# fetty31/fast_LIMO

Hardware: AMD Instinct MI355X
Metric: scans/sec (64k-pt scan, 1M-pt map) + kNN HBM GB/s vs roofline; ATE vs CPU ref (higher is better)
Workload: dtype f32; 1 GPU; BASELINE.json configs[1]: 65536-pt Velodyne-like scan (64 rings x 1024 azimuths), 1000000-pt box-world map, k=5, MAX_NUM_ITERS=3, GPU deskew + iterated ESKF update per step; parallelism=replicas x1 (independent scan streams, no collective), steps_bit_reproducible=True, chains_run=0, chains_handed_back_early=0, chains_declined=2597

## Files before the change

fast_limo_amd/_abi.py:

```python
from __future__ import annotations

import ctypes as C
import numpy as np

f32p = np.ctypeslib.ndpointer(dtype=np.float32, flags="C_CONTIGUOUS")
f64p = np.ctypeslib.ndpointer(dtype=np.float64, flags="C_CONTIGUOUS")
i32p = np.ctypeslib.ndpointer(dtype=np.int32, flags="C_CONTIGUOUS")

CHAIN_MAX_PASSES = 12


class MapCfg(C.Structure):
    _fields_ = [("min_extent", C.c_float), ("bucket_size", C.c_int), ("downsample", C.c_int),
                ("cell_size", C.c_float)]


class MatchCfg(C.Structure):
    _fields_ = [("NUM_MATCH_POINTS", C.c_int), ("MAX_NUM_MATCHES", C.c_int), ("MAX_NUM_PC2MATCH", C.c_int),
                ("MAX_DIST_PLANE", C.c_double), ("PLANE_THRESHOLD", C.c_double), ("estimate_extrinsics", C.c_int)]


class Frame(C.Structure):
    _fields_ = [("p", C.c_float * 3), ("q", C.c_float * 4), ("v", C.c_float * 3), ("g", C.c_float * 3),
                ("w", C.c_float * 3), ("a", C.c_float * 3), ("bg", C.c_float * 3), ("ba", C.c_float * 3),
# ... 148 lines not shown
    ("flimo_corr_graph", "flimo_loc_corr_graph", [vp, vp, sz, P(CorrGraphCfg), vp, vp, vp, vp]),
    ("flimo_desc_ref_set", "flimo_loc_desc_ref_set", [vp, sz, i]),
    ("flimo_desc_match", "flimo_loc_desc_match", [vp, sz, i, i, vp, vp, vp]),
)
LOC_OF = {hip: loc for hip, loc, _ in PAIRED}

HIP_ONLY = (
    (i, "flimo_ctx_create", [i, P(vp)]),
    (None, "flimo_ctx_destroy", [vp]),
    (C.c_char_p, "flimo_last_error", [vp]),
    (C.c_char_p, "flimo_version", []),
    (i, "flimo_map_config", [vp, P(MapCfg)]),
    (i, "flimo_map_add", [vp, f32p, sz, sz, d]),
    (i, "flimo_map_clear", [vp]),
    (i, "flimo_map_crop_box", [vp, vp, vp, P(sz)]),
    (i, "flimo_map_crop_stats", [vp, P(u64)]),
    (i, "flimo_map_carve_stats", [vp, P(u64)]),
    (sz, "flimo_map_size", [vp]),
    (d, "flimo_map_last_time", [vp]),
    (i, "flimo_map_points", [vp, vp, sz, P(sz)]),
    (i, "flimo_map_add_scan", [vp, f64p, d]),
    (i, "flimo_knn", [vp, f32p, sz, i, i32p, f32p, i32p]),
    (i, "flimo_radius_candidates", [vp, f32p, sz, f, vp]),
    (i, "flimo_knn_k_candidates", [vp, vp, sz, i, f, vp]),
    (i, "flimo_set_outlier_chunk", [vp, sz]),
    (i, "flimo_set_fpfh_chunk", [vp, sz]),
    (i, "flimo_set_keypoints_chunk", [vp, sz]),
    (i, "flimo_set_cluster_chunk", [vp, sz]),
    (i, "flimo_set_plane_chunk", [vp, sz]),
    (i, "flimo_set_voxel_plan", [vp, i]),
    (i, "flimo_set_region_chunk", [vp, sz]),
    (i, "flimo_set_normals_chunk", [vp, sz]),
    (i, "flimo_set_fitness_chunk", [vp, sz]),
    (i, "flimo_set_linearize_chunk", [vp, sz]),
    (i, "flimo_set_corr_chunk", [vp, sz]),
    (i, "flimo_set_desc_chunk", [vp, sz, sz]),
    (sz, "flimo_desc_ref_size", [vp]),
    (i, "flimo_desc_ref_dim", [vp]),
    (f, "flimo_desc_last_ms", [vp]),
    (i, "flimo_plane_solve_host", [vp, P(PlaneCfg), vp, vp]),
    (i, "flimo_voxel_key_host", [vp, f, vp, P(u64)]),
    (i, "flimo_region_joined_host", [vp, vp, vp, vp, P(RegionCfg), P(i), P(i), P(i)]),
    (i, "flimo_corr_pose_host", [vp, vp, P(CorrCfg), vp, vp]),
    (i, "flimo_corr_compatible_host", [vp, vp, vp, vp, P(CorrGraphCfg)]),
    (i, "flimo_desc_dist_host", [vp, vp, i, vp]),
    (None, "flimo_plane_fit5_host", [f32p, f32p]),
    (i, "flimo_plane_eval5_host", [f32p, f32p, f]),
    (i, "flimo_calculate_H_host", [f64p, f32p, f32p, f32p, sz, i, f64p, f64p]),
    (i, "flimo_insert_rule_replay", [f, i, f32p, vp, sz, vp, P(sz)]),
    (i, "flimo_scan_set", [vp, f32p, sz, sz]),
    (sz, "flimo_scan_size", [vp]),
    (i, "flimo_scan_get", [vp, vp, sz, P(sz)]),
    (i, "flimo_scan_voxel_filter", [vp, f, P(sz)]),
    (i, "flimo_raw_scan_set", [vp, f32p, sz, sz, f64p]),
    (i, "flimo_raw_scan_filter_set", [vp, vp, sz, P(FilterCfg), P(sz), P(d), P(i)]),
    (i, "flimo_raw_scan_filter_order_set", [vp, vp, sz, P(FilterCfg), i, P(sz), P(d), P(i), P(i)]),
    (i, "flimo_raw_scan_order", [vp, vp, sz, P(sz)]),
    (i, "flimo_upload_stage", [vp, sz, P(vp)]),
    (i, "flimo_scan_adopt", [vp, vp]),
    (i, "flimo_deskew_resident", [vp, vp, sz, f32p, f64p]),
    (i, "flimo_deskew_resident_offset", [vp, vp, sz, f32p, f64p, d]),
    (i, "flimo_deskew", [vp, f32p, sz, sz, f64p, vp, sz, f32p, f64p]),
    (i, "flimo_scan_to_world", [vp, f64p, vp, sz]),
    (i, "flimo_scan_clouds", [vp, f64p, P(vp), P(vp), P(sz)]),
    (i, "flimo_scan_debug_clouds", [vp, f64p, P(vp), P(vp), P(sz)]),
    (i, "flimo_match_reduce", [vp, f64p, P(MatchCfg), f64p, f64p, P(i)]),
    (i, "flimo_match_reduce_overlap", [vp, f64p, P(MatchCfg), f64p, f64p, P(i), vp, vp]),
    (i, "flimo_match_fetch", [vp, vp, sz, P(sz)]),
    (i, "flimo_match_fetch_H", [vp, vp, vp, sz, P(sz)]),
    (i, "flimo_update_chain", [vp, P(MatchCfg), P(ChainIO)]),
    (i, "flimo_chain_stats", [vp, f64p, i]),
    (i, "flimo_set_update_mode", [vp, i]),
    (i, "flimo_update_mode", [vp, P(i), P(d)]),
    (i, "flimo_set_pass_pipeline", [vp, i]),
    (i, "flimo_pass_pipeline_end", [vp]),
    (i, "flimo_pass_pipeline_last", [vp]),
    (i, "flimo_pass_pipeline_stats", [vp, P(ull)]),
    (i, "flimo_device_large_bar", [i, P(i)]),
    (i, "flimo_set_timing", [vp, i]),
    (i, "flimo_set_timing_stride", [vp, i]),
    (i, "flimo_set_timing_deferred", [vp, i]),
    (i, "flimo_set_wait_timeout_ms", [vp, i]),
    (i, "flimo_set_debug_records", [vp, i]),
    (i, "flimo_set_path_switches", [vp, i, i]),
    (ull, "flimo_pass_count", [vp]),
    (ull, "flimo_fused_pass_count", [vp]),
    (i, "flimo_tie_stats", [vp, P(ull)]),
    (i, "flimo_fine_stats", [vp, P(ull)]),
    (i, "flimo_map_index_bytes", [vp, P(u64)]),
    (i, "flimo_map_index_layout", [vp, i, P(d)]),
    (i, "flimo_map_grid_selfcheck", [vp, P(u64), P(u64)]),
    (i, "flimo_last_kernel_ms", [vp, P(f), P(f), P(f)]),
    (d, "flimo_last_candidates_per_query", [vp]),
    (i, "flimo_last_widen_count", [vp]),
    (i, "flimo_last_stragglers", [vp]),
    (i, "flimo_stragglers_by_pass", [vp, P(i)]),
    (i, "flimo_timing_totals", [vp, P(d), P(d), P(d), P(C.c_longlong), P(C.c_longlong), i]),
    (i, "flimo_timing_split", [vp, f64p, i]),
    (i, "flimo_ieskf_op_shape", [i, P(i), P(i)]),
    (i, "flimo_ieskf_eval", [vp, i, f64p, sz, f64p]),
    (i, "flimo_ieskf_eval_host", [i, f64p, sz, f64p, vp]),
    (i, "flimo_ieskf_run_fixed", [vp, f64p, f64p, f64p, d, d, i, i, f64p, f64p, vp, f64p, f64p, P(i)]),
)

HOST_ONLY = (
    (i, "flimo_loc_create", [P(LocCfg), P(vp)]),
    (None, "flimo_loc_destroy", [vp]),
    (vp, "flimo_loc_ctx", [vp]),
    (None, "flimo_loc_sync", [vp]),
    (None, "flimo_loc_set_async_insert", [vp, i]),
    (None, "flimo_loc_set_lazy_time_order", [vp, i]),
    (None, "flimo_loc_set_gpu_filters", [vp, i]),
    (None, "flimo_loc_set_exact_tied_order", [vp, i]),
    (None, "flimo_loc_set_local_map", [vp, f32p, f]),
    (i, "flimo_local_map_rule", [f64p, f32p, f, f64p, P(i), f32p, f32p]),
    (None, "flimo_loc_set_map_carving", [vp, i, P(CarveCfg)]),
    (i, "flimo_carve_rule", [i, P(i)]),
    (None, "flimo_carve_sensor", [f64p, f32p]),
    (sz, "flimo_loc_last_carve_removed", [vp]),
    (i, "flimo_loc_last_sweep_tied", [vp]),
    (None, "flimo_loc_set_propagation_wait", [vp, d]),
    (d, "flimo_loc_last_insert_seconds", [vp]),
    (i, "flimo_loc_update_imu", [vp, d, f32p, f32p]),
    (i, "flimo_loc_update_imu_n", [vp, sz, f64p, f32p, f32p]),
    (i, "flimo_loc_replay", [vp, sz, P(vp), uintpp, f64p, f64p, sz, f64p, f32p, f32p, i32p, f64p]),
    (i, "flimo_loc_update_pointcloud", [vp, f32p, sz, d]),
    (i, "flimo_loc_update_pointcloud_points", [vp, vp, sz, d]),
    (i, "flimo_loc_map_add", [vp, f32p, sz, d]),
    (sz, "flimo_loc_map_size", [vp]),
    (None, "flimo_loc_get_x", [vp, f64p]),
    (None, "flimo_loc_set_x", [vp, f64p]),
    (None, "flimo_loc_get_P", [vp, f64p]),
    (None, "flimo_loc_set_P", [vp, f64p]),
    (None, "flimo_loc_set_flags", [vp, i, i, i]),
    (i, "flimo_loc_num_passes", [vp]),
    (None, "flimo_loc_get_pass", [vp, i, P(i), f64p, f64p, f64p, f64p]),
    (sz, "flimo_loc_get_pc2match", [vp, vp, sz]),
    (sz, "flimo_loc_get_final_scan", [vp, vp, sz]),
    (sz, "flimo_loc_get_debug_cloud", [vp, i, vp, sz]),
    (None, "flimo_loc_get_stage_times", [vp, f64p]),
    (None, "flimo_loc_get_pose_cov", [vp, f64p]),
    (None, "flimo_loc_host_profile", [vp, f64p, i]),
    (i, "flimo_loc_register_resident", [vp, f64p, f64p]),
    (None, "flimo_host_state_update", [f32p, d, d]),
    (i, "flimo_host_time_order", [vp, i, sz, i, i, vp]),
    (i, "flimo_host_plane", [f32p, f32p, i, i, d, d, f32p, f32p, P(f)]),
    (i, "flimo_eskf_update_fixed", [f64p, f64p, f64p, f64p, i, i, f64p, d, d, P(i)]),
    (i, "flimo_eskf_predict", [f64p, f64p, d, f64p, f64p, f64p]),
    (i, "flimo_ieskf_gj12_host", [i, f64p, sz, f64p]),
    (i, "flimo_ieskf_run_fixed_host", [f64p, f64p, f64p, d, d, i, i, f64p, f64p, P(i), f64p, f64p, P(i)]),
    (None, "flimo_host_eigen_solver6", [f64p, f64p, f64p, f64p]),
)

HIP_SYMBOLS = [hip for hip, _, _ in PAIRED] + [name for _, name, _ in HIP_ONLY]
HOST_SYMBOLS = [loc for _, loc, _ in PAIRED] + [name for _, name, _ in HOST_ONLY]


def declare(lib, side):
    for row in PAIRED:
        fn = getattr(lib, row[side])
        fn.restype, fn.argtypes = C.c_int, [vp] + row[2]
    for restype, name, args in (HIP_ONLY, HOST_ONLY)[side]:
        fn = getattr(lib, name)
        fn.restype, fn.argtypes = restype, args
```

fast_limo_amd/_lib.py:

```python
from __future__ import annotations

import ctypes as C
import os
import numpy as np

from . import _abi
from ._abi import (CHAIN_MAX_PASSES, CarveCfg, ChainIO, ChainPass, ClusterCfg, ClusterStats, CorrCfg, CorrGraphCfg, FilterCfg, FpfhCfg, Frame,
                   KeypointCfg, MapCfg, MatchCfg, OutlierCfg, OutlierStats, PlaneCfg, PlaneSel, RegionCfg, RegionStats, VoxelCfg, VoxelStats,
                   f32p, f64p, i32p)

_PKG = os.path.dirname(os.path.abspath(__file__))
ROOT = os.path.dirname(_PKG)


class FlimoError(RuntimeError):
    pass


RADIUS_SORTED = 1


def carve_cfg(res=256, win=1, margin=0.2, rel_margin=0.02, max_depth=float("inf")) -> CarveCfg:
    return CarveCfg(int(res), int(win), float(margin), float(rel_margin), float(max_depth))

# ... 663 lines not shown
    def scan_clouds(self, x26):
        b, w, n = C.c_void_p(), C.c_void_p(), C.c_size_t(0)
        self._chk(self._L.flimo_scan_clouds(self._h, np.ascontiguousarray(x26, dtype=np.float64), C.byref(b), C.byref(w), C.byref(n)))
        if n.value == 0:
            return np.zeros((0, 3), np.float32), np.zeros((0, 3), np.float32)
        rec = lambda p: np.ctypeslib.as_array(C.cast(p, C.POINTER(C.c_float)), shape=(n.value, 4))[:, :3].copy()
        return rec(b), rec(w)

    def scan_debug_clouds(self, x26):
        d, f, n = C.c_void_p(), C.c_void_p(), C.c_size_t(0)
        self._chk(self._L.flimo_scan_debug_clouds(self._h, np.ascontiguousarray(x26, dtype=np.float64), C.byref(d), C.byref(f), C.byref(n)))
        if n.value == 0:
            return np.zeros((0, 4), np.float32), np.zeros((0, 4), np.float32)
        rec = lambda p: np.ctypeslib.as_array(C.cast(p, C.POINTER(C.c_float)), shape=(n.value, 4)).copy()
        return rec(d), rec(f)

    def map_add_scan(self, x26, stamp=0.0):
        self._chk(self._L.flimo_map_add_scan(self._h, np.ascontiguousarray(x26, dtype=np.float64), float(stamp)))

    def set_timing(self, level=2):
        self._chk(self._L.flimo_set_timing(self._h, 2 if level is True else int(level)))

    def set_timing_stride(self, every=1):
        self._chk(self._L.flimo_set_timing_stride(self._h, int(every)))

    def set_timing_deferred(self, on=True):
        self._chk(self._L.flimo_set_timing_deferred(self._h, 1 if on else 0))

    def pass_count(self) -> int:
        return int(self._L.flimo_pass_count(self._h))

    def fine_stats(self):
        o = (C.c_ulonglong * 4)()
        self._chk(self._L.flimo_fine_stats(self._h, o))
        return dict(active=bool(o[0]), points=int(o[1]), builds=int(o[2]), passes=int(o[3]))

    def tie_stats(self):
        o = (C.c_ulonglong * 2)()
        self._chk(self._L.flimo_tie_stats(self._h, o))
        return dict(passes_redone=int(o[0]), queries_settled=int(o[1]))

    def map_index_bytes(self):
        o = (C.c_uint64 * 6)()
        self._chk(self._L.flimo_map_index_bytes(self._h, o))
        return dict(points=int(o[0]), index=int(o[1]), second_level=int(o[2]), tiles=int(o[3]), tile_pool_relayouts=int(o[4]),
                    sorted_array_allocated=int(o[5]))

    def map_index_layout(self, level=0):
        o = (C.c_double * 28)()
        self._chk(self._L.flimo_map_index_layout(self._h, int(level), o))
        if not o[19]:
            return dict(valid=False)
        ints = ("xs", "six", "siy", "siz", "nx", "ny", "nz", "ts", "ty", "tz", "ntx", "nty", "ntz", "escape_slots", "escape_slots_taken")
        d = dict(valid=True, ox=np.float32(o[0]), oy=np.float32(o[1]), oz=np.float32(o[2]), cell=np.float32(o[3]), points=int(o[20]))
        d.update((name, int(o[4 + i])) for i, name in enumerate(ints))
        if level == 1:
            d.update(qlo=tuple(int(o[21 + a]) for a in range(3)), qhi=tuple(int(o[24 + a]) for a in range(3)))
        return d

    def fused_pass_count(self) -> int:
        return int(self._L.flimo_fused_pass_count(self._h))

    def grid_selfcheck(self):
        mm = C.c_uint64(0)
        st = (C.c_uint64 * 2)()
        self._chk(self._L.flimo_map_grid_selfcheck(self._h, C.byref(mm), st))
        return int(mm.value), int(st[0]), int(st[1])

    def set_debug_records(self, on=True):
        self._chk(self._L.flimo_set_debug_records(self._h, int(on)))

    def last_kernel_ms(self):
        a = C.c_float(0)
        b = C.c_float(0)
        d = C.c_float(0)
        self._chk(self._L.flimo_last_kernel_ms(self._h, C.byref(a), C.byref(b), C.byref(d)))
        return a.value, b.value, d.value

    def timing_totals(self, reset=False):
        a = C.c_double(0); b = C.c_double(0); d = C.c_double(0); n = C.c_longlong(0); q = C.c_longlong(0)
        self._chk(self._L.flimo_timing_totals(self._h, C.byref(a), C.byref(b), C.byref(d), C.byref(n), C.byref(q), int(reset)))
        return dict(knn_ms=a.value, widen_ms=b.value, fit_ms=d.value, passes=n.value, queries=q.value)

    def set_path_switches(self, tail=-1, fuse=-1):
        self._chk(self._L.flimo_set_path_switches(self._h, int(tail), int(fuse)))

    def timing_split(self, reset=False):
        o = np.zeros(6)
        self._chk(self._L.flimo_timing_split(self._h, o, int(reset)))
        return dict(fused_ms=o[0], fused_n=int(o[1]), knn_ms=o[2], widen_ms=o[3], fit_ms=o[4], separate_n=int(o[5]))

    def update_chain(self, cfg: "MatchCfg", x26, P, limits, R=0.001, D=5.0, max_iter=3, want_log=True):
        io = ChainIO()
        io.x26[:] = list(np.asarray(x26, dtype=np.float64))
        io.P[:] = list(np.asarray(P, dtype=np.float64).reshape(-1))
        io.limits[:] = list(np.asarray(limits, dtype=np.float64))
        io.R, io.D, io.max_iter, io.want_log = float(R), float(D), int(max_iter), int(bool(want_log))
        self._chk(self._L.flimo_update_chain(self._h, C.byref(cfg), C.byref(io)))
        n_log = min(CHAIN_MAX_PASSES, io.passes + (1 if io.status == 2 else 0))
        log = [dict(M=io.log[i].M, stragglers=io.log[i].stragglers, ties=io.log[i].ties,
                    HTH=np.array(io.log[i].HTH).reshape(12, 12), HTh=np.array(io.log[i].HTh), dx=np.array(io.log[i].dx),
                    x_after=np.array(io.log[i].x_after)) for i in range(n_log)]
        meas = dict(M=io.meas_M, HTH=np.array(io.meas_HTH).reshape(12, 12), HTh=np.array(io.meas_HTh)) if io.meas_valid else None
        return dict(status=io.status, reason=io.reason, passes=io.passes, it_next=io.it_next, t=io.t, x=np.array(io.x26_out),
                    meas=meas, log=log)

    def set_update_mode(self, mode: int):
        self._chk(self._L.flimo_set_update_mode(self._h, int(mode)))

    def update_mode(self):
        ch = C.c_int(0); rtt = C.c_double(0)
        self._chk(self._L.flimo_update_mode(self._h, C.byref(ch), C.byref(rtt)))
        return dict(chained=bool(ch.value), launch_rtt_us=rtt.value)

    def set_pass_pipeline(self, on: bool):
        self._chk(self._L.flimo_set_pass_pipeline(self._h, int(on)))

    def pass_pipeline_end(self):
        self._chk(self._L.flimo_pass_pipeline_end(self._h))

    def pass_pipeline_last(self):
        self._chk(self._L.flimo_pass_pipeline_last(self._h))

    def pass_pipeline_stats(self):
        o = (C.c_ulonglong * 4)()
        self._chk(self._L.flimo_pass_pipeline_stats(self._h, o))
        return dict(published=int(o[0]), cancelled=int(o[1]), aged=int(o[2]), left=int(o[3]))

    def chain_stats(self, reset=False):
        o = np.zeros(5)
        self._chk(self._L.flimo_chain_stats(self._h, o, int(reset)))
        return dict(algebra_ms=o[0], algebra_n=int(o[1]), chains=int(o[2]), handed_back=int(o[3]), declined=int(o[4]))

    def ieskf_eval(self, op, items):
        a, no = ik_items(op, items)
        out = np.zeros((a.shape[0], no))
        if a.shape[0]:
            self._chk(self._L.flimo_ieskf_eval(self._h, int(op), a.reshape(-1), a.shape[0], out.reshape(-1)))
        return out

    def ieskf_run_fixed(self, x26, P, limits, partials, extras=None, tag_ok=None, R=0.001, D=5.0, max_iter=3):
        x, Pm, lim, part = ik_fixed_args(x26, P, limits, partials)
        ns = part.shape[0]
        ex = np.zeros((ns, 2)) if extras is None else np.ascontiguousarray(extras, dtype=np.float64).reshape(ns, 2)
        tg = None if tag_ok is None else np.ascontiguousarray(tag_ok, dtype=np.int32).reshape(ns)
        it_out = np.zeros((int(max_iter) + 1, IK_ITER_N))
        fin = np.zeros(IK_FINAL_N)
        n = C.c_int(0)
        self._chk(self._L.flimo_ieskf_run_fixed(self._h, x, Pm, lim, float(R), float(D), int(max_iter), ns, part.reshape(-1), ex.reshape(-1),
                                                None if tg is None else tg.ctypes.data, it_out.reshape(-1), fin, C.byref(n)))
        its = []
        for r in it_out[:n.value]:
            on = bool(r[590])
            its.append(dict(pre_dxn=r[0:23].copy(), pre_AG=r[23:299].copy(), HTH=r[299:443].reshape(12, 12).copy() if on else None,
                            HTh=r[443:455].copy() if on else None, dx=r[455:478].copy() if on else None,
                            x_after=r[478:504].copy() if on else None, pose=r[504:570].astype(np.float32), prev_RT=r[570:586].astype(np.float32),
                            status=int(r[586]), it=int(r[587]), t=int(r[588]), passes=int(r[589]), went_on=on))
        final = dict(status=int(fin[0]), reason=int(fin[1]), passes=int(fin[2]), it=int(fin[3]), t=int(fin[4]), x=fin[5:31].copy(),
                     passinfo=fin[31:67].reshape(12, 3).copy(), sums=fin[67:158].copy())
        return its, final

    def last_widen_count(self) -> int:
        return int(self._L.flimo_last_widen_count(self._h))

    def set_wait_timeout_ms(self, ms: int):
        self._chk(self._L.flimo_set_wait_timeout_ms(self._h, int(ms)))

    def last_stragglers(self) -> int:
# ... 76 lines not shown
```

fast_limo_amd/csrc/hip/flimo_capi.hip:

```cpp
#include <hip/hip_runtime.h>
#include <stdarg.h>
#include <stdio.h>
#include <string.h>
#include <math.h>
#include <string>
#include <chrono>
#include <thread>
#include <array>
#include <vector>
#include <algorithm>
#include <limits>
#include <immintrin.h>
#include "../../../include/flimo_c.h"
#include "../../../include/flimo_dev.h"
#include "flimo_types.h"
#include "flimo_kernels.h"
#include "flimo_math.h"
#include "flimo_pose.h"
#include "flimo_corr.h"
#include "flimo_plane.h"
#include "flimo_voxel.h"
#include "flimo_region.h"
#include "flimo_desc.h"
#include "flimo_chain.h"
// ... 146 lines not shown
  bool recs_valid = false, dbg_valid = false;
  PrevPass prev{};
  bool prune = true;
  unsigned probe_min = 96;
  int stragglers_hist[4] = {1 << 30, 0, 0, 0};
  int pass_in_scan = 0;
  int last_stragglers = -1;
  bool fine_on = true;
  unsigned fine_threshold = 64;
  int fine_div = 4;
  unsigned fine_min_points = 32768;
  bool fine_valid = false;
  bool crowd_box_valid = false;
  GridView fine{};
  int fine_qlo[3] = {0, 0, 0}, fine_qhi[3] = {-1, -1, -1};
  float4 *d_fine_tmp = nullptr, *d_fine_pts = nullptr;
  size_t fine_pts_cap = 0;
  IndexTables fine_idx;
  uint32_t* d_fine_count = nullptr;
  void* d_crowd_list = nullptr;
  uint32_t* d_crowd_count = nullptr;
  uint32_t* d_crowd_bits = nullptr;
  size_t crowd_bits_cap = 0;
  uint32_t crowd_listed = 0;
  std::vector<std::array<int, 3>> crowd_cells;
  float fine_center[3] = {0.f, 0.f, 0.f};
  bool have_fine_center = false;
  float fine_radius = 24.f;
  uint64_t fine_builds = 0, fine_passes = 0;
  int xslabs = 2;
  int* d_tie_list = nullptr;
  unsigned int* d_tie_count = nullptr;
  size_t tie_cap = 0;
  bool ties = true;
  unsigned long long tie_redos = 0, tie_queries = 0;
  unsigned long long* d_tie_settled = nullptr;
  void* d_nbrk = nullptr;
  size_t nbrk_cap = 0;
  int wait_timeout_ms = 2000;
  hipEvent_t adopt_ev = nullptr;
  hipEvent_t timeout_ev = nullptr;
  bool timeout_pending = false;
  ChainState* d_chain = nullptr;
  void* d_chain_gran = nullptr;
  ChainPrior* h_chain_prior = nullptr;
  ChainPrior* d_chain_prior = nullptr;
  double* h_chain_res = nullptr;
  void* d_chain_res = nullptr;
  double* h_chain_log = nullptr;
  void* d_chain_log = nullptr;
  unsigned long long chain_tag = 0x4000000000000000ull;
  struct Prelaunch {
    bool active = false;
    unsigned long long seq = 0;
    size_t nq = 0;
    int n_all = 0, pos = 0;
    flimo_match_cfg cfg{};
    uint64_t grid_version = 0;
    unsigned int end_code = 0;
    double t_launch = 0.0;
    float prev_RT[16] = {0};
  } pre;
  bool pipeline = false;
  bool pipeline_env = false;
  PipeHead* d_pipe_head = nullptr;
  unsigned int pipe_tag = 0;
  bool pipe_last_hint = false;
  unsigned long long pipe_published = 0, pipe_cancelled = 0;
  unsigned long long pipe_aged = 0, pipe_left = 0;
  bool row_slack = true;
  bool test_tight_array = false;
  int test_publish_delay_ms = 0;
  int test_publish_split_ms = 0;
  PrevPass prev_before{};
  int update_mode = 0;
  double launch_rtt_us = 0.0;
  bool host_update = false;
  hipEvent_t chain_ev[CH_MAX_PASSES][8];
  bool chain_ev_made = false;
  double chain_alg_ms = 0;
  long long chain_alg_n = 0, chains_run = 0, chains_back = 0, chains_declined = 0;
  int fov_check = 0, fov_check_bad = 0;
  bool tail = true;
};

constexpr size_t FRAMES_FG_SLOT = 8192;
static int timing_drain(flimo_ctx* c);
static inline void ctx_enter(flimo_ctx* c);
static int fail(flimo_ctx* c, int code, const char* fmt, ...) {
  char buf[512];
  va_list ap;
  va_start(ap, fmt);
  vsnprintf(buf, sizeof(buf), fmt, ap);
  va_end(ap);
  if (c) c->err = buf;
  return code;
}
#define HIPCHK(c, call)                                                                          \
  do {                                                                                           \
    hipError_t e_ = (call);                                                                      \
    if (e_ != hipSuccess) return fail(c, FLIMO_ERR_HIP, "%s failed: %s", #call, hipGetErrorString(e_)); \
  } while (0)

static int ensure_pinned(flimo_ctx* c, void*& buf, size_t& cap, size_t bytes) {
  if (bytes <= cap) return FLIMO_OK;
  if (buf) (void)hipHostFree(buf);
  buf = nullptr;
  cap = 0;
  const size_t ncap = bytes + bytes / 4 + 4096;
  HIPCHK(c, hipHostMalloc(&buf, ncap, hipHostMallocDefault));
  cap = ncap;
  return FLIMO_OK;
}
static int ensure_stage(flimo_ctx* c, size_t bytes) { return ensure_pinned(c, c->h_stage, c->stage_cap, bytes); }

template <typename T>
static int ensure_dev(flimo_ctx* c, T*& p, size_t& cap, size_t need, bool keep, size_t keep_n) {
  if (need <= cap) return FLIMO_OK;
  size_t ncap = need + need / 4 + 1024;
  T* np = nullptr;
  HIPCHK(c, hipMalloc(&np, ncap * sizeof(T)));
  if (keep && p && keep_n) {
    HIPCHK(c, hipMemcpyAsync(np, p, keep_n * sizeof(T), hipMemcpyDeviceToDevice, c->stream));
    HIPCHK(c, hipStreamSynchronize(c->stream));
  }
  if (p) (void)hipFree(p);
  p = np;
  cap = ncap;
  return FLIMO_OK;
}

struct DevScratch {
  std::vector<void*> got;
  hipError_t err = hipSuccess;
  DevScratch() = default;
  DevScratch(const DevScratch&) = delete;
  DevScratch& operator=(const DevScratch&) = delete;
  ~DevScratch() { for (void* p : got) (void)hipFree(p); }
  template <typename T>
  T* get(size_t count) {
    void* p = nullptr;
    if (err == hipSuccess) err = hipMalloc(&p, count * sizeof(T));
    if (err != hipSuccess) return nullptr;
    got.push_back(p);
    return static_cast<T*>(p);
  }
  void drop(void* p) {
    got.erase(std::remove(got.begin(), got.end(), p), got.end());
    (void)hipFree(p);
  }
  int ok(flimo_ctx* c) const { return err == hipSuccess ? FLIMO_OK : fail(c, FLIMO_ERR_HIP, "hipMalloc failed: %s", hipGetErrorString(err)); }
};


static void load_dev_switches(flimo_ctx* c) {
  auto env_int = [](const char* name, int& out) { const char* e = getenv(name); if (!e) return false; out = atoi(e); return true; };
  int v = 0;
  if (env_int("FLIMO_FUSE", v)) c->fuse = v != 0;
  if (env_int("FLIMO_TAIL", v)) c->tail = v != 0;
  if (env_int("FLIMO_PRUNE", v)) c->prune = v != 0;
  if (env_int("FLIMO_PROBE", v) && v >= 0) c->probe_min = (unsigned)v;
  if (env_int("FLIMO_TIES", v)) c->ties = v != 0;
  if (env_int("FLIMO_FINE", v)) c->fine_on = v != 0;
  if (env_int("FLIMO_FINE_THRESHOLD", v) && v > 0) c->fine_threshold = (unsigned)v;
  if (env_int("FLIMO_FINE_MIN_POINTS", v) && v >= 0) c->fine_min_points = (unsigned)v;
  if (env_int("FLIMO_FULL_REBUILD", v)) c->full_rebuild = v != 0;
  if (env_int("FLIMO_HOST_UPDATE", v)) c->update_mode = v != 0 ? 1 : 2;
  if (env_int("FLIMO_PIPELINE", v)) { c->pipeline = v != 0; c->pipeline_env = true; }
  if (env_int("FLIMO_TEST_PUBLISH_DELAY_MS", v) && v > 0) c->test_publish_delay_ms = v;
  if (env_int("FLIMO_TEST_PUBLISH_SPLIT_MS", v) && v > 0) c->test_publish_split_ms = v;
  if (env_int("FLIMO_TEST_TIGHT_ARRAY", v)) c->test_tight_array = v != 0;
  if (env_int("FLIMO_ROW_SLACK", v)) c->row_slack = v != 0;
  if (env_int("FLIMO_TAIL_MAX", v) && v > 0) c->tail_max_env = v;
}

static bool host_store_probe(flimo_ctx* c, PipeHead* head) {
  volatile unsigned long long* tagp = reinterpret_cast<volatile unsigned long long*>(c->h_chain_res) + 1;
  for (unsigned int round = 0; round < 2; round++) {
    const unsigned int pattern = 0x5a17c0deu ^ (round * 0x01010101u);
    volatile unsigned long long* g = &head->gran[round == 0 ? 0 : PH_GRANULES - 1];
    *g = ((unsigned long long)pattern << 32) | (unsigned long long)round;
    _mm_sfence();
    const unsigned long long tag = 0x7200000000000000ull + round;
    launch_word_probe(c->stream, reinterpret_cast<unsigned int*>(const_cast<unsigned long long*>(g)) + 1, c->d_chain_res, tag);
    if (hipStreamSynchronize(c->stream) != hipSuccess) { (void)hipGetLastError(); return false; }
    if (*tagp != tag) return false;
    const double seen = c->h_chain_res[0];
    if ((unsigned int)llround(seen) != pattern) return false;
    *g = 0ull;
  }
  _mm_sfence();
  memset(c->h_chain_res, 0, 2 * sizeof(double));
  return true;
}

extern "C" const char* flimo_version(void) { return "fast_limo_amd 0.1.0 (gfx950)"; }

extern "C" const char* flimo_last_error(const flimo_ctx* ctx) { return ctx ? ctx->err.c_str() : "null context"; }

extern "C" int flimo_ctx_create(int device, flimo_ctx** out) {
  if (!out) return FLIMO_ERR_INVALID;
  *out = nullptr;
  int ndev = 0;
  if (hipGetDeviceCount(&ndev) != hipSuccess || ndev <= 0) return FLIMO_ERR_NO_DEVICE;
  if (device < 0 || device >= ndev) return FLIMO_ERR_INVALID;
  if (hipSetDevice(device) != hipSuccess) return FLIMO_ERR_NO_DEVICE;
  hipDeviceProp_t prop;
  if (hipGetDeviceProperties(&prop, device) != hipSuccess) return FLIMO_ERR_NO_DEVICE;
  if (strncmp(prop.gcnArchName, "gfx950", 6) != 0) return FLIMO_ERR_NO_DEVICE;
  flimo_ctx* c = new flimo_ctx();
  c->device = device;
  if (hipStreamCreateWithFlags(&c->stream, hipStreamNonBlocking) != hipSuccess) { delete c; return FLIMO_ERR_HIP; }
  for (int i = 0; i < 6; i++) (void)hipEventCreate(&c->ev[i]);
  bool ok = hipMalloc(&c->d_partials, (size_t)c->reduce_waves * 256 * sizeof(double)) == hipSuccess &&
            hipMalloc(&c->d_out256, FIT_GROUPS * FIT_SLOT * sizeof(double)) == hipSuccess &&
            hipHostMalloc((void**)&c->h_out256, FIT_GROUPS * FIT_SLOT * sizeof(double), hipHostMallocMapped) == hipSuccess &&
            hipHostGetDevicePointer((void**)&c->d_out256_host, c->h_out256, 0) == hipSuccess &&
            hipHostMalloc((void**)&c->h_granules, FIT_GROUPS * FIT_LIVE_PAD * 2 * sizeof(double), hipHostMallocMapped) == hipSuccess &&
            hipHostGetDevicePointer((void**)&c->d_granules_host, c->h_granules, 0) == hipSuccess &&
            hipMalloc(&c->d_ticket, (FIT_GROUPS + 2) * sizeof(unsigned int)) == hipSuccess &&
            hipMemset(c->d_ticket, 0, (FIT_GROUPS + 2) * sizeof(unsigned int)) == hipSuccess &&
            hipMalloc(&c->d_cand, sizeof(unsigned long long)) == hipSuccess &&
            hipMalloc(&c->d_tie_count, 2 * sizeof(unsigned int)) == hipSuccess &&
            hipMemset(c->d_tie_count, 0, 2 * sizeof(unsigned int)) == hipSuccess &&
            hipMalloc((void**)&c->d_chain, chain_state_size()) == hipSuccess &&
            hipMemset(c->d_chain, 0, chain_state_size()) == hipSuccess &&
            hipMalloc(&c->d_chain_gran, FIT_GROUPS * FIT_LIVE_PAD * 2 * sizeof(double)) == hipSuccess &&
            hipMemset(c->d_chain_gran, 0, FIT_GROUPS * FIT_LIVE_PAD * 2 * sizeof(double)) == hipSuccess &&
            hipHostMalloc((void**)&c->h_chain_prior, sizeof(ChainPrior), hipHostMallocMapped) == hipSuccess &&
            hipHostGetDevicePointer((void**)&c->d_chain_prior, c->h_chain_prior, 0) == hipSuccess &&
            hipHostMalloc((void**)&c->h_chain_res, (size_t)CH_RES * 2 * sizeof(double), hipHostMallocMapped) == hipSuccess &&
            hipHostGetDevicePointer(&c->d_chain_res, c->h_chain_res, 0) == hipSuccess &&
            hipHostMalloc((void**)&c->h_chain_log, (size_t)CH_MAX_PASSES * CH_LOGN * 2 * sizeof(double), hipHostMallocMapped) == hipSuccess &&
            hipHostGetDevicePointer(&c->d_chain_log, c->h_chain_log, 0) == hipSuccess &&
            hipMalloc((void**)&c->d_tie_settled, sizeof(unsigned long long)) == hipSuccess &&
            hipMemset(c->d_tie_settled, 0, sizeof(unsigned long long)) == hipSuccess &&
            hipMalloc(&c->d_wl_count, sizeof(int)) == hipSuccess &&
            hipMemset(c->d_wl_count, 0, sizeof(int)) == hipSuccess &&
            hipHostMalloc((void**)&c->h_wl_count, sizeof(int), hipHostMallocDefault) == hipSuccess &&
            hipHostMalloc((void**)&c->h_cand, sizeof(unsigned long long), hipHostMallocDefault) == hipSuccess;
  if (!ok) { flimo_ctx_destroy(c); return FLIMO_ERR_HIP; }
  memset(c->h_chain_res, 0, (size_t)CH_RES * 2 * sizeof(double));
  memset(c->h_chain_log, 0, (size_t)CH_MAX_PASSES * CH_LOGN * 2 * sizeof(double));
  memset(c->h_out256, 0, FIT_GROUPS * FIT_SLOT * sizeof(double));
  memset(c->h_granules, 0, FIT_GROUPS * FIT_LIVE_PAD * 2 * sizeof(double));
  launch_mfma_layout(c->stream, c->d_out256);
  if (hipMemcpyAsync(c->h_out256, c->d_out256, 256 * sizeof(double), hipMemcpyDeviceToHost, c->stream) != hipSuccess ||
      hipStreamSynchronize(c->stream) != hipSuccess) { flimo_ctx_destroy(c); return FLIMO_ERR_HIP; }
  bool seen[256] = {false};
  for (int r = 0; r < 256; r++) {
    const double v = c->h_out256[r];
    const int code = (int)llround(v);
    if (code < 0 || code > 255 || fabs(v - code) > 1e-9 || seen[code]) { flimo_ctx_destroy(c); return FLIMO_ERR_HIP; }
    seen[code] = true;
    c->mfma_idx[code / 16][code % 16] = r;
  }
  {
    int k = 0;
    for (int i = 0; i < 12; i++) for (int j = i; j < 12; j++) c->live_idx[k++] = (unsigned char)c->mfma_idx[i][j];
    for (int i = 0; i < 12; i++) c->live_idx[k++] = (unsigned char)c->mfma_idx[i][12];
    c->live_idx[k++] = (unsigned char)c->mfma_idx[13][13];
    for (; k < FIT_LIVE_PAD; k++) c->live_idx[k] = 0;
  }
  c->book = insert_book_create();
  load_dev_switches(c);
  {
    void* p = nullptr;
    int large_bar = 0;
    (void)hipDeviceGetAttribute(&large_bar, hipDeviceAttributeIsLargeBar, device);
    if (getenv("FLIMO_NO_BAR") != nullptr) large_bar = 0;
    if (large_bar && hipExtMallocWithFlags(&p, sizeof(PipeHead), hipDeviceMallocFinegrained) == hipSuccess && p &&
        hipMemset(p, 0, sizeof(PipeHead)) == hipSuccess && hipDeviceSynchronize() == hipSuccess && host_store_probe(c, static_cast<PipeHead*>(p))) {
      c->d_pipe_head = static_cast<PipeHead*>(p);
      void* q = nullptr;
      if (hipExtMallocWithFlags(&q, 2 * FRAMES_FG_SLOT, hipDeviceMallocFinegrained) == hipSuccess && q)
        c->d_frames_fg = static_cast<char*>(q);
      else (void)hipGetLastError();
    } else {
      if (p) (void)hipFree(p);
      (void)hipGetLastError();
      c->d_pipe_head = nullptr;
    }
  }
  {
    std::vector<double> rt;
    volatile unsigned long long* tagp = reinterpret_cast<volatile unsigned long long*>(c->h_chain_res) + 1;
    for (int i = 0; i < 40; i++) {
      const unsigned long long tag = 0x7100000000000000ull + (unsigned long long)i;
      const auto t0 = std::chrono::steady_clock::now();
      launch_rtt_probe(c->stream, c->d_chain_res, tag);
      unsigned long long spins = 0;
      while (*tagp != tag && ++spins < 200000000ull) _mm_pause();
      const double us = std::chrono::duration<double, std::micro>(std::chrono::steady_clock::now() - t0).count();
      if (i >= 8) rt.push_back(us);
    }
    (void)hipStreamSynchronize(c->stream);
    std::sort(rt.begin(), rt.end());
    c->launch_rtt_us = rt[rt.size() / 4];
    memset(c->h_chain_res, 0, 2 * sizeof(double));
    c->host_update = c->update_mode != 2;
  }
  *out = c;
  return FLIMO_OK;
}

extern "C" void flimo_ctx_destroy(flimo_ctx* c) {
  if (!c) return;
  ctx_enter(c);
  if (c->stream) (void)hipStreamSynchronize(c->stream);
  (void)hipFree(c->d_map_raw); (void)hipFree(c->d_map_sorted); index_free(c->idx); index_free(c->fine_idx);
  (void)hipFree(c->d_scan_sorted); (void)hipFree(c->d_nbr); (void)hipFree(c->d_wl); (void)hipFree(c->d_wl_count);
  (void)hipFree(c->d_fit_partials); (void)hipFree(c->d_raw_sorted); (void)hipFree(c->d_t_sorted);
  (void)hipFree(c->d_scan); (void)hipFree(c->d_scan_raw); (void)hipFree(c->d_scan_world); (void)hipFree(c->d_scan_t);
  (void)hipFree(c->d_frames); (void)hipFree(c->d_recs); (void)hipFree(c->d_dbg); (void)hipFree(c->d_dbg_clouds);
  (void)hipFree(c->d_fine_tmp); (void)hipFree(c->d_fine_pts); 
  (void)hipFree(c->d_fine_count); (void)hipFree(c->d_crowd_list); (void)hipFree(c->d_crowd_count); (void)hipFree(c->d_crowd_bits);
  (void)hipFree(c->d_tkey[0]); (void)hipFree(c->d_tkey[1]); (void)hipFree(c->d_tperm); (void)hipFree(c->d_t_tmp);
  (void)hipFree(c->d_raw32); (void)hipFree(c->d_filt_ext); (void)hipFree(c->d_nbrk); (void)hipFree(c->d_tie_list); (void)hipFree(c->d_tie_count);
  if (c->h_filt_ext) (void)hipHostFree(c->h_filt_ext);
  (void)hipFree(c->d_partials); (void)hipFree(c->d_out256); (void)hipFree(c->d_cand); (void)hipFree(c->d_ticket);
  if (c->h_out256) (void)hipHostFree(c->h_out256);
  if (c->h_granules) (void)hipHostFree(c->h_granules);
  (void)hipFree(c->d_fit2_partials);
  if (c->h_cand) (void)hipHostFree(c->h_cand);
  (void)hipFree(c->d_chain); (void)hipFree(c->d_chain_gran); (void)hipFree(c->d_tie_settled);
  if (c->h_chain_prior) (void)hipHostFree(c->h_chain_prior);
  if (c->h_chain_res) (void)hipHostFree(c->h_chain_res);
  if (c->h_chain_log) (void)hipHostFree(c->h_chain_log);
  if (c->chain_ev_made) for (int i = 0; i < CH_MAX_PASSES; i++) for (int k = 0; k < 8; k++) (void)hipEventDestroy(c->chain_ev[i][k]);
  if (c->h_stage) (void)hipHostFree(c->h_stage);
  if (c->h_dbg_clouds) (void)hipHostFree(c->h_dbg_clouds);
  if (c->h_clouds) (void)hipHostFree(c->h_clouds);
  for (int k = 0; k < 2; k++) if (c->h_frames[k]) (void)hipHostFree(c->h_frames[k]);
  map_scratch_free(c->scratch);
  for (int i = 0; i < 6; i++) if (c->ev[i]) (void)hipEventDestroy(c->ev[i]);
  if (c->ev_ring_made) for (int r = 0; r < flimo_ctx::EV_RING; r++) for (int i = 0; i < 6; i++) (void)hipEventDestroy(c->ev_ring[r][i]);
  if (c->timeout_ev) (void)hipEventDestroy(c->timeout_ev);
  if (c->adopt_ev) (void)hipEventDestroy(c->adopt_ev);
  if (c->h_wl_count) (void)hipHostFree(c->h_wl_count);
  if (c->d_pipe_head) (void)hipFree(c->d_pipe_head);
  if (c->d_frames_fg) (void)hipFree(c->d_frames_fg);
  if (c->stream) (void)hipStreamDestroy(c->stream);
  if (c->book) insert_book_destroy(c->book);
  c->gbook.release();
  (void)hipFree(c->d_batch);
  (void)hipFree(c->d_desc_rt); (void)hipFree(c->d_desc_norm);
  delete c;
}

extern "C" int flimo_map_config(flimo_ctx* c, const flimo_map_cfg* cfg) {
  if (!c || !cfg) return FLIMO_ERR_INVALID;
  if (!(cfg->min_extent > 0.f)) return fail(c, FLIMO_ERR_INVALID, "min_extent must be > 0");
  const float cell_before = c->map_cfg.cell_size;
  c->map_cfg = *cfg;
  if (!(c->map_cfg.cell_size > 0.f)) c->map_cfg.cell_size = 0.5f;
  if (c->map_cfg.cell_size != cell_before) { c->force_full = true; c->have_gbox = false; c->have_origin = false; }
  insert_book_config(c->book, cfg->min_extent, cfg->downsample != 0);
  return FLIMO_OK;
}

extern "C" int flimo_map_clear(flimo_ctx* c) {
  if (!c) return FLIMO_ERR_INVALID;
  c->map_n = 0;
  c->grid_valid = false;
  c->fine_valid = false;
  c->have_gbox = false;
  c->have_origin = false;
  c->map_last_time = -1.0;
  c->bb[0] = c->bb[1] = c->bb[2] = 3.4e38f; c->bb[3] = c->bb[4] = c->bb[5] = -3.4e38f;
  c->crowd_box_valid = false;
  c->have_fine_center = false;
  insert_book_clear(c->book);
  c->gbook.active = false;
  c->prev.valid = 0;
  return FLIMO_OK;
}

extern "C" size_t flimo_map_size(const flimo_ctx* c) { return c ? c->map_n : 0; }
extern "C" double flimo_map_last_time(const flimo_ctx* c) { return c ? c->map_last_time : -1.0; }

static inline int grid_low_x_cells(int xs) { return (8 + xs - 1) / xs; }
static bool grid_side_low_ok(const GridView& g, const float* bb, int a) {
  const float o[3] = {g.ox, g.oy, g.oz};
  const int si[3] = {g.six, g.siy, g.siz};
  const int low = a == 0 ? grid_low_x_cells(g.xs) : 0;
  if ((int)floorf((bb[a] - 0.5f * g.cell - o[a]) * g.inv_cell) - si[a] < low) return false;
  if ((int)floorf((bb[a] - o[a]) * g.inv_cell) - si[a] < low) return false;
  return true;
}
static bool grid_covers(const GridView& g, const float* bb) {
  const float o[3] = {g.ox, g.oy, g.oz};
  const int n[3] = {g.nx, g.ny, g.nz}, si[3] = {g.six, g.siy, g.siz};
  for (int a = 0; a < 3; a++) {
    if (!grid_side_low_ok(g, bb, a)) return false;
    if ((int)floorf((bb[3 + a] - o[a]) * g.inv_cell) - si[a] > n[a] - 2) return false;
  }
  return true;
}
static int update_fine_grid(flimo_ctx* c, bool relayout, const float4* new_pts = nullptr, size_t n_new = 0) {
  c->fine_valid = false;
  if (!c->fine_on || !c->grid_valid || c->map_n == 0) return FLIMO_OK;
  const GridView& g = c->grid;
  if ((double)g.nx * (double)g.ny * (double)g.nz > 2.0e9) return FLIMO_OK;
  constexpr uint32_t CROWD_CAP = 1u << 20;
  if (!c->d_crowd_list) {
    HIPCHK(c, hipMalloc(&c->d_crowd_list, (size_t)CROWD_CAP * sizeof(int4)));
    HIPCHK(c, hipMalloc(&c->d_crowd_count, sizeof(uint32_t)));
    HIPCHK(c, hipMalloc(&c->d_fine_count, sizeof(uint32_t)));
  }
  static const bool prof = getenv("FLIMO_PROF_INSERT") != nullptr;
  auto now = [] { return std::chrono::duration<double>(std::chrono::steady_clock::now().time_since_epoch()).count(); };
  const double tp0 = prof ? now() : 0.0;
  uint32_t listed = 0;
  const size_t ncells_main = (size_t)g.nx * g.ny * g.nz;
  if (relayout || !c->crowd_box_valid || !new_pts) {
    const size_t words = (ncells_main + 31) / 32;
    if (words > c->crowd_bits_cap) {
      (void)hipFree(c->d_crowd_bits);
      c->d_crowd_bits = nullptr; c->crowd_bits_cap = 0;
      HIPCHK(c, hipMalloc(&c->d_crowd_bits, (words + words / 4 + 64) * sizeof(uint32_t)));
      c->crowd_bits_cap = words + words / 4 + 64;
    }
// ... 1542 lines not shown
    struct Part { void* dst; const void* src; size_t bytes; char* at; } parts[5] = {
        {centroid, d_centroid, 24 * m, nullptr}, {cov, d_cov, 48 * m, nullptr}, {label, d_label, 4 * m, nullptr},
        {count, d_cnt, 4 * m, nullptr},          {first, d_first, 4 * m, nullptr}};
    for (Part& p : parts) {
      if (!p.dst) continue;
      p.at = h;
      h += p.bytes;
      HIPCHK(c, hipMemcpyAsync(p.at, p.src, p.bytes, hipMemcpyDeviceToHost, c->stream));
    }
    HIPCHK(c, hipStreamSynchronize(c->stream));
    for (const Part& p : parts)
      if (p.dst) memcpy(p.dst, p.at, p.bytes);
  }
  if (stats) *stats = st;
  return FLIMO_OK;
}
extern "C" int flimo_map_remove_regions(flimo_ctx* c, size_t first, size_t n, const flimo_region_cfg* cfg, size_t* removed,
                                        flimo_region_stats* stats) {
  if (!c) return FLIMO_ERR_INVALID;
  { const int rc = region_check(c, first, n, cfg, "remove regions"); if (rc) return rc; }
  if (c->map_n == 0) { if (removed) *removed = 0; region_stats_none(stats); return FLIMO_OK; }
  if (n == 0 && !stats) { if (removed) *removed = 0; return FLIMO_OK; }
  RegionDev d;
  flimo_region_stats st;
  { const int rc = regions_device(c, first, n, *cfg, false, false, true, false, d, &st); if (rc) return rc; }
  if (removed) *removed = 0;
  if (stats) *stats = st;
  if (st.sel_points == 0) return FLIMO_OK;
  return map_remove_masked(c, d.mask, first, n, (size_t)st.sel_points, &c->region_removals, &c->region_removed, removed, "remove regions");
}
extern "C" int flimo_set_region_chunk(flimo_ctx* c, size_t n) { return set_chunk(c, &flimo_ctx::region_chunk, n, (size_t)1 << 20); }
extern "C" int flimo_region_joined_host(const float pi[3], const float ni[4], const float pj[3], const float nj[4], const flimo_region_cfg* cfg,
                                        int* smooth_i, int* smooth_j, int* joined) {
  if (!pi || !ni || !pj || !nj || !cfg || !region_cfg_ok(cfg)) return FLIMO_ERR_INVALID;
  const float r2 = cfg->tol * cfg->tol;
  if (smooth_i) *smooth_i = region_smooth(ni[0], ni[1], ni[2], ni[3], cfg->max_curv) ? 1 : 0;
  if (smooth_j) *smooth_j = region_smooth(nj[0], nj[1], nj[2], nj[3], cfg->max_curv) ? 1 : 0;
  if (joined)
    *joined = region_has_normal(ni[0], ni[1], ni[2], ni[3]) && region_has_normal(nj[0], nj[1], nj[2], nj[3]) &&
                      region_joined(pi, ni, pj, nj, r2, cfg->min_cos) ? 1 : 0;
  return FLIMO_OK;
}
extern "C" int flimo_set_voxel_plan(flimo_ctx* c, int plan) {
  if (!c) return FLIMO_ERR_INVALID;
  if (plan < 0 || (plan & ~VOXEL_PLAN_SORTED) > VOXEL_PLAN_RUNS) return fail(c, FLIMO_ERR_INVALID, "voxel plan: %d is none of 0..4, + 8", plan);
  c->voxel_plan = plan;
  return FLIMO_OK;
}

static int ensure_raw_sorted(flimo_ctx* c, size_t n) {
  if (n <= c->raw_sorted_cap) return FLIMO_OK;
  const size_t cap = n + n / 4 + 1024;
  float4* rs = nullptr;
  double* ts = nullptr;
  HIPCHK(c, hipMalloc(&rs, cap * sizeof(float4)));
  HIPCHK(c, hipMalloc(&ts, cap * sizeof(double)));
  (void)hipFree(c->d_raw_sorted); (void)hipFree(c->d_t_sorted);
  c->d_raw_sorted = rs; c->d_t_sorted = ts; c->raw_sorted_cap = cap;
  return FLIMO_OK;
}
static int ensure_scan(flimo_ctx* c, size_t n) {
  { const int rc = ensure_raw_sorted(c, n); if (rc) return rc; }
  if (n <= c->scan_cap) return FLIMO_OK;
  const size_t cap = n + n / 4 + 1024;
  float4 *a = nullptr, *b = nullptr, *w = nullptr, *so = nullptr;
  double* t = nullptr;
  void* nb = nullptr;
  int* wl = nullptr;
  double* fp = nullptr;
  const size_t fpn = (size_t)fit_blocks((int)cap) * 256;
  {
    int* tlst = nullptr;
    HIPCHK(c, hipMalloc(&tlst, cap * sizeof(int)));
    (void)hipFree(c->d_tie_list);
    c->d_tie_list = tlst; c->tie_cap = cap;
  }
  {
    const size_t f2n = (size_t)std::max(std::max(fit2_blocks((int)cap), fused_blocks((int)cap)), FUSED_SPREAD_SLOTS / 128 + 8) * FIT_LIVE_PAD;
    double* f2 = nullptr;
    HIPCHK(c, hipMalloc(&f2, f2n * sizeof(double)));
    (void)hipFree(c->d_fit2_partials);
    c->d_fit2_partials = f2; c->fit2_partials_cap = f2n;
  }
  HIPCHK(c, hipMalloc(&so, cap * sizeof(float4)));
  HIPCHK(c, hipMalloc(&nb, cap * nbr_rec_size()));
  HIPCHK(c, hipMemsetAsync(nb, 0, cap * nbr_rec_size(), c->stream));
  HIPCHK(c, hipMalloc(&wl, (cap + 8192) * wl_entry_size()));
  HIPCHK(c, hipMalloc(&fp, fpn * sizeof(double)));
  (void)hipFree(c->d_scan_sorted); (void)hipFree(c->d_nbr); (void)hipFree(c->d_wl); (void)hipFree(c->d_fit_partials);
  c->d_scan_sorted = so; c->d_nbr = nb; c->d_wl = wl; c->d_fit_partials = fp; c->fit_partials_cap = fpn;
  HIPCHK(c, hipMalloc(&a, cap * sizeof(float4)));
  HIPCHK(c, hipMalloc(&b, cap * sizeof(float4)));
  HIPCHK(c, hipMalloc(&w, cap * sizeof(float4)));
  HIPCHK(c, hipMalloc(&t, cap * sizeof(double)));
  (void)hipFree(c->d_scan); (void)hipFree(c->d_scan_raw); (void)hipFree(c->d_scan_world); (void)hipFree(c->d_scan_t);
  c->d_scan = a; c->d_scan_raw = b; c->d_scan_world = w; c->d_scan_t = t;
  c->scan_cap = cap;
  c->scan_n = 0; c->sorted_n = 0; c->raw_n = 0; c->prev.valid = 0;
  c->deskew_kept = false;
  return FLIMO_OK;
}

static int ensure_recs(flimo_ctx* c, size_t n) {
  if (n <= c->rec_cap) return FLIMO_OK;
  const size_t cap = n + n / 4 + 1024;
  (void)hipFree(c->d_recs); (void)hipFree(c->d_dbg);
  c->d_recs = nullptr; c->d_dbg = nullptr; c->rec_cap = 0;
  HIPCHK(c, hipMalloc(&c->d_recs, cap * sizeof(Rec16)));
  HIPCHK(c, hipMalloc(&c->d_dbg, cap * sizeof(RecDbg)));
  c->rec_cap = cap;
  return FLIMO_OK;
}

static int upload_points(flimo_ctx* c, const float* xyz, size_t n, size_t stride_bytes, float4* dst) {
  int rc = ensure_stage(c, n * sizeof(float4));
  if (rc) return rc;
  float4* st = (float4*)c->h_stage;
  const unsigned char* b = (const unsigned char*)xyz;
  for (size_t i = 0; i < n; i++) {
    const float* p = (const float*)(b + i * stride_bytes);
    st[i].x = p[0]; st[i].y = p[1]; st[i].z = p[2]; st[i].w = (stride_bytes >= 16) ? p[3] : 0.f;
  }
  HIPCHK(c, hipMemcpyAsync(dst, st, n * sizeof(float4), hipMemcpyHostToDevice, c->stream));
  HIPCHK(c, hipStreamSynchronize(c->stream));
  return FLIMO_OK;
}

static int flush_deskew(flimo_ctx* c) {
  if (!c->deskew_pending) return FLIMO_OK;
  c->deskew_pending = false;
  const DeskewArgs& a = c->deskew_args;
  launch_deskew(c->stream, a.raw, a.t, (int)c->deskew_n, a.frames, a.nf, a.mats, a.out_sorted, a.out_orig, a.t_offset);
  HIPCHK(c, hipGetLastError());
  return FLIMO_OK;
}

extern "C" int flimo_scan_set(flimo_ctx* c, const float* xyz, size_t n, size_t stride_bytes) {
  if (!c) return FLIMO_ERR_INVALID;
  if (n > 0 && (!xyz || stride_bytes < 12)) return fail(c, FLIMO_ERR_INVALID, "bad xyz/stride");
  if (n > 0x7fff0000ull) return fail(c, FLIMO_ERR_TOO_LARGE, "scan too large");
  ctx_enter(c);
  c->deskew_pending = false;
  c->deskew_kept = false;
  int rc = ensure_scan(c, n);
  if (rc) return rc;
  if (n) {
    rc = upload_points(c, xyz, n, stride_bytes, c->d_scan);
    if (rc) return rc;
    HIPCHK(c, sort_scan(c->stream, c->d_scan, n, c->d_scan_sorted, c->scratch));
    HIPCHK(c, hipStreamSynchronize(c->stream));
  }
  c->scan_n = n; c->sorted_n = n; c->prev.valid = 0;
  return FLIMO_OK;
}

extern "C" size_t flimo_scan_size(const flimo_ctx* c) { return c ? c->scan_n : 0; }

static int download_xyz(flimo_ctx* c, const float4* src, size_t m, float* out) {
  int rc = ensure_stage(c, m * sizeof(float4));
  if (rc) return rc;
  HIPCHK(c, hipMemcpyAsync(c->h_stage, src, m * sizeof(float4), hipMemcpyDeviceToHost, c->stream));
  HIPCHK(c, hipStreamSynchronize(c->stream));
  const float4* s = (const float4*)c->h_stage;
  for (size_t i = 0; i < m; i++) { out[3 * i] = s[i].x; out[3 * i + 1] = s[i].y; out[3 * i + 2] = s[i].z; }
  return FLIMO_OK;
}
// ... 340 lines not shown
  if (!on && c->ev_pending) { const int rc = timing_drain(c); if (rc) return rc; }
  c->timing_deferred = on != 0;
  return FLIMO_OK;
}
extern "C" unsigned long long flimo_pass_count(const flimo_ctx* c) { return c ? c->pass_seq : 0ull; }
extern "C" unsigned long long flimo_fused_pass_count(const flimo_ctx* c) { return c ? c->fused_passes : 0ull; }
extern "C" int flimo_fine_stats(const flimo_ctx* c, unsigned long long out[4]) {
  if (!c || !out) return FLIMO_ERR_INVALID;
  out[0] = c->fine_valid ? 1 : 0; out[1] = c->fine_valid ? c->fine.n_pts : 0; out[2] = c->fine_builds; out[3] = c->fine_passes;
  return FLIMO_OK;
}
extern "C" int flimo_map_index_bytes(const flimo_ctx* c, uint64_t out[6]) {
  if (!c || !out) return FLIMO_ERR_INVALID;
  out[0] = (uint64_t)c->map_n * sizeof(float4);
  auto tables = [](const GridView& g, const IndexTables& T) {
    const uint64_t rows = ((uint64_t)g.ny + 2 * GRID_PAD) * ((uint64_t)g.nz + 2 * GRID_PAD);
    return (uint64_t)T.tiles_used * grid_tile_entries(g.ts, g.ty, g.tz) * 8ull + (uint64_t)GRID_DIR_MAX * 2ull +
           (uint64_t)(grid_xstart_size(g.ny, g.nz, g.ntx) + T.ovf_cap) * 4ull + rows * 4ull + (uint64_t)g.ny * g.nz * 4ull;
  };
  out[5] = c->d_map_sorted ? (uint64_t)c->sorted_cap * sizeof(float4) : 0ull;
  out[1] = c->grid_valid ? tables(c->grid, c->idx) : 0ull;
  out[2] = c->fine_valid ? (uint64_t)c->fine.n_pts * sizeof(float4) + tables(c->fine, c->fine_idx) : 0ull;
  out[3] = c->grid_valid ? c->idx.tiles_used : 0ull;
  out[4] = c->index_overflows;
  return FLIMO_OK;
}
extern "C" int flimo_map_index_layout(flimo_ctx* c, int level, double out[28]) {
  if (!c || !out || level < 0 || level > 1) return FLIMO_ERR_INVALID;
  for (int i = 0; i < 28; i++) out[i] = 0.0;
  const bool valid = level == 0 ? c->grid_valid : c->fine_valid;
  out[19] = valid ? 1.0 : 0.0;
  if (!valid) return FLIMO_OK;
  const GridView& g = level == 0 ? c->grid : c->fine;
  const IndexTables& T = level == 0 ? c->idx : c->fine_idx;
  out[0] = g.ox; out[1] = g.oy; out[2] = g.oz; out[3] = g.cell; out[4] = g.xs;
  out[5] = g.six; out[6] = g.siy; out[7] = g.siz; out[8] = g.nx; out[9] = g.ny; out[10] = g.nz;
  out[11] = g.ts; out[12] = g.ty; out[13] = g.tz; out[14] = g.ntx; out[15] = g.nty; out[16] = g.ntz;
  out[17] = (double)(T.ovf_cap / 8);
  uint32_t taken = 0;
  ctx_enter(c);
  HIPCHK(c, hipStreamSynchronize(c->stream));
  if (T.counters) HIPCHK(c, hipMemcpy(&taken, T.counters + 2, sizeof(taken), hipMemcpyDeviceToHost));
  out[18] = taken;
  out[20] = g.n_pts;
  if (level == 1) for (int a = 0; a < 3; a++) { out[21 + a] = c->fine_qlo[a]; out[24 + a] = c->fine_qhi[a]; }
  return FLIMO_OK;
}
extern "C" int flimo_tie_stats(flimo_ctx* c, unsigned long long out[2]) {
  if (!c || !out) return FLIMO_ERR_INVALID;
  out[0] = c->tie_redos; out[1] = c->tie_queries;
  unsigned long long dev = 0;
  ctx_enter(c);
  if (c->d_tie_settled && hipMemcpy(&dev, c->d_tie_settled, sizeof(dev), hipMemcpyDeviceToHost) == hipSuccess) out[1] += dev;
  return FLIMO_OK;
}
extern "C" int flimo_set_timing_stride(flimo_ctx* c, int every) { if (!c || every < 1) return FLIMO_ERR_INVALID; c->timing_stride = every; return FLIMO_OK; }
extern "C" int flimo_set_debug_records(flimo_ctx* c, int on) { if (!c) return FLIMO_ERR_INVALID; c->debug_recs = on != 0; return FLIMO_OK; }
extern "C" int flimo_last_kernel_ms(const flimo_ctx* c, float* knn_ms, float* widen_ms, float* fit_ms) {
  if (!c) return FLIMO_ERR_INVALID;
  if (knn_ms) *knn_ms = c->last_knn_ms;
  if (widen_ms) *widen_ms = c->last_widen_ms;
  if (fit_ms) *fit_ms = c->last_fit_ms;
  return FLIMO_OK;
}
extern "C" int flimo_last_widen_count(const flimo_ctx* c) { return c ? c->last_widen_count : 0; }
extern "C" int flimo_last_stragglers(const flimo_ctx* c) { return c ? c->last_stragglers : -1; }
extern "C" int flimo_stragglers_by_pass(const flimo_ctx* c, int out[4]) {
  if (!c || !out) return FLIMO_ERR_INVALID;
  for (int i = 0; i < 4; i++) out[i] = c->stragglers_hist[i];
  return FLIMO_OK;
}
extern "C" int flimo_timing_totals(flimo_ctx* c, double* knn_ms, double* widen_ms, double* fit_ms, long long* passes,
                                   long long* queries, int reset) {
  if (!c) return FLIMO_ERR_INVALID;
  if (c->ev_pending) { ctx_enter(c); const int rc = timing_drain(c); if (rc) return rc; }
  if (knn_ms) *knn_ms = c->tot_knn_ms;
  if (widen_ms) *widen_ms = c->tot_widen_ms;
  if (fit_ms) *fit_ms = c->tot_fit_ms;
  if (passes) *passes = c->tot_passes;
  if (queries) *queries = c->tot_queries;
  if (reset) { c->tot_knn_ms = c->tot_widen_ms = c->tot_fit_ms = 0.0; c->tot_passes = 0; c->tot_queries = 0; }
  return FLIMO_OK;
}
extern "C" int flimo_set_path_switches(flimo_ctx* c, int tail, int fuse) {
  if (!c) return FLIMO_ERR_INVALID;
  if (tail >= 0) c->tail = tail != 0;
  if (fuse >= 0) c->fuse = fuse != 0;
  return FLIMO_OK;
}
extern "C" int flimo_timing_split(flimo_ctx* c, double out[6], int reset) {
  if (!c || !out) return FLIMO_ERR_INVALID;
  if (c->ev_pending) { ctx_enter(c); const int rc = timing_drain(c); if (rc) return rc; }
  out[0] = c->split_fused_ms; out[1] = (double)c->split_fused_n;
  out[2] = c->split_knn_ms; out[3] = c->split_widen_ms; out[4] = c->split_fit_ms; out[5] = (double)c->split_sep_n;
  if (reset) { c->split_fused_ms = c->split_knn_ms = c->split_widen_ms = c->split_fit_ms = 0.0; c->split_fused_n = c->split_sep_n = 0; }
  return FLIMO_OK;
}
extern "C" double flimo_last_candidates_per_query(const flimo_ctx* c) { return c ? c->last_cand_per_query : 0.0; }

static int gate_rings(const flimo_ctx* c, double max_dist_plane) {
  const double cell = c->grid.cell;
  const int maxdim = std::max(c->grid.nx, std::max(c->grid.ny, c->grid.nz));
  const double margin = 1.0e-3 + 4.0e-7 * maxdim;
  const double need = sqrt(std::max(max_dist_plane, 0.0)) * (1.0 + 1e-5) / cell + margin;
  int r = (int)ceil(need);
  return std::max(r, 1);
}

static int abandon_wait(flimo_ctx* c, const char* what, unsigned long long id) {
  if (!c->timeout_ev) (void)hipEventCreateWithFlags(&c->timeout_ev, hipEventDisableTiming);
  if (c->timeout_ev && hipEventRecord(c->timeout_ev, c->stream) == hipSuccess) c->timeout_pending = true;
  c->prev.valid = 0;
  return fail(c, FLIMO_ERR_TIMEOUT, "%s %llu did not publish its result within %d ms (kernels still running)", what, id, c->wait_timeout_ms);
}
static inline bool same_match_cfg(const flimo_match_cfg& a, const flimo_match_cfg& b) {
  return a.NUM_MATCH_POINTS == b.NUM_MATCH_POINTS && a.MAX_NUM_MATCHES == b.MAX_NUM_MATCHES && a.MAX_NUM_PC2MATCH == b.MAX_NUM_PC2MATCH &&
         a.MAX_DIST_PLANE == b.MAX_DIST_PLANE && a.PLANE_THRESHOLD == b.PLANE_THRESHOLD && a.estimate_extrinsics == b.estimate_extrinsics;
}
static inline double wall_s() { return std::chrono::duration<double>(std::chrono::steady_clock::now().time_since_epoch()).count(); }
static inline void cancel_prelaunch(flimo_ctx* c) {
  if (!c->pre.active) return;
  c->pre.active = false;
  c->pipe_cancelled++;
  *reinterpret_cast<volatile unsigned long long*>(&c->d_pipe_head->gran[0]) = (unsigned long long)c->pre.end_code << 32;
  _mm_sfence();
}
static inline void ctx_enter(flimo_ctx* c) {
  (void)hipSetDevice(c->device);
  cancel_prelaunch(c);
}
static inline void publish_prelaunch(flimo_ctx* c, const PoseMats& P, unsigned long long seq) {
  unsigned int w[PH_GRANULES] = {0u};
  const unsigned int* src = reinterpret_cast<const unsigned int*>(&P);
  for (int i = 0; i < PH_WORDS; i++) w[i] = src[i < 36 ? (i / 12) * 16 + i % 12 : i + 12];
  const unsigned long long tag = (unsigned long long)ch_epoch_of(seq) << 32;
  volatile unsigned long long* dst = c->d_pipe_head->gran;
  for (int i = 0; i < PH_GRANULES; i++) {
    if (i == PH_GRANULES / 2 && c->test_publish_split_ms > 0) {
      _mm_sfence();
      std::this_thread::sleep_for(std::chrono::milliseconds(c->test_publish_split_ms));
    }
    dst[i] = tag | (unsigned long long)w[i];
  }
  _mm_sfence();
  c->pre.active = false;
  c->pipe_published++;
}

static inline bool auto_host_update(const flimo_ctx*) { return true; }

static int check_abandoned(flimo_ctx* c) {
  if (!c->timeout_pending) return FLIMO_OK;
  hipError_t q = hipEventQuery(c->timeout_ev);
  if (q == hipErrorNotReady) return fail(c, FLIMO_ERR_TIMEOUT, "the launches of an earlier pass whose wait ran out are still running");
  c->timeout_pending = false;
  if (q != hipSuccess) return fail(c, FLIMO_ERR_HIP, "an abandoned pass failed: %s", hipGetErrorString(q));
  return FLIMO_OK;
}
static bool tags_complete(const flimo_ctx* c, unsigned long long want) {
  const volatile unsigned long long* t0 = reinterpret_cast<const volatile unsigned long long*>(c->h_granules);
  if (t0[2 * FIT_LIVE + 1] != want || t0[2 * (FIT_LIVE + 1) + 1] != want) return false;
  for (int g = 0; g < FIT_GROUPS; g++) {
    const volatile unsigned long long* tags = reinterpret_cast<const volatile unsigned long long*>(c->h_granules + (size_t)g * FIT_LIVE_PAD * 2);
    for (int k = 0; k < FIT_LIVE; k++)
      if (tags[2 * k + 1] != want) return false;
  }
  return true;
}
constexpr int FLIMO_PASS_LEFT = 1000;
static int wait_tags(flimo_ctx* c, unsigned long long want, int left_ms = -1) {
  const volatile unsigned long long* t0 = reinterpret_cast<const volatile unsigned long long*>(c->h_granules);
  unsigned long long spins = 0;
  double deadline = 0.0;
  auto now_s = [] { return std::chrono::duration<double>(std::chrono::steady_clock::now().time_since_epoch()).count(); };
  if (c->wait_timeout_ms == 0) return abandon_wait(c, "pass", want);
  const int bound_ms = left_ms >= 0 ? std::min(left_ms, c->wait_timeout_ms) : c->wait_timeout_ms;
  for (;;) {
    if (t0[2 * (FIT_LIVE + 1) + 1] == want && tags_complete(c, want)) return FLIMO_OK;
    _mm_pause();
    if ((++spins & 0x3fffull) != 0) continue;
    if (left_ms >= 0 && c->d_pipe_head &&
        __atomic_load_n(&c->d_pipe_head->decision, __ATOMIC_ACQUIRE) == ((ch_epoch_of(want) & 0x3fffffffu) | 0x80000000u)) return FLIMO_PASS_LEFT;
    const double t = now_s();
    if (deadline == 0.0) { deadline = t + 1e-3 * (double)bound_ms; continue; }
    if (t < deadline) continue;
    const hipError_t q = hipStreamQuery(c->stream);
    if (q == hipErrorNotReady && left_ms >= 0 && bound_ms < c->wait_timeout_ms) { left_ms = -1; deadline = t + 1e-3 * (double)(c->wait_timeout_ms - bound_ms); continue; }
    if (q == hipErrorNotReady) return abandon_wait(c, "pass", want);
    if (q != hipSuccess) return fail(c, FLIMO_ERR_HIP, "pass %llu failed: %s", want, hipGetErrorString(q));
    if (tags_complete(c, want)) return FLIMO_OK;
    if (left_ms >= 0) return FLIMO_PASS_LEFT;
    (void)hipMemsetAsync(c->d_ticket, 0, (FIT_GROUPS + 2) * sizeof(unsigned int), c->stream);
    (void)hipMemsetAsync(c->d_wl_count, 0, sizeof(int), c->stream);
    (void)hipMemsetAsync(c->d_tie_count, 0, 2 * sizeof(unsigned int), c->stream);
    (void)hipStreamSynchronize(c->stream);
    c->prev.valid = 0;
    return fail(c, FLIMO_ERR_HIP, "pass %llu completed without publishing its result (reduction tickets re-armed)", want);
  }
}

extern "C" int flimo_set_wait_timeout_ms(flimo_ctx* c, int ms) {
  if (!c || ms < 0) return FLIMO_ERR_INVALID;
  c->wait_timeout_ms = ms;
  return FLIMO_OK;
}

extern "C" int flimo_match_reduce(flimo_ctx* c, const double x26[26], const flimo_match_cfg* cfg, double HTH[144], double HTh[12], int* M);
extern "C" int flimo_match_reduce_overlap(flimo_ctx* c, const double x26[26], const flimo_match_cfg* cfg, double HTH[144], double HTh[12],
                                          int* M, void (*while_in_flight)(void*), void* arg) {
  if (!c) return FLIMO_ERR_INVALID;
  c->overlap_fn = while_in_flight;
  c->overlap_arg = arg;
  const int rc = flimo_match_reduce(c, x26, cfg, HTH, HTh, M);
  c->overlap_fn = nullptr;
  return rc;
}

static inline void run_overlap(flimo_ctx* c) {
  if (!c->overlap_fn) return;
  void (*fn)(void*) = c->overlap_fn;
  c->overlap_fn = nullptr;
  fn(c->overlap_arg);
}

struct PassPlan {
  const flimo_match_cfg* cfg = nullptr;
  PoseMats P;
  MatchParams mp;
  size_t nq = 0;
  int n_all = 0;
  bool general_k = false;
  bool use_pre = false, was_pre = false;
  bool last_of_update = false;
  uint64_t grid_version = 0;
  const DeskewArgs* dkp = nullptr;
  bool cap_binds = false, want_recs = false, want_count = false, fused_cap = false, use_fit2 = false;
  int tlev = 0;
  hipEvent_t* ev = nullptr;
  int tail_max = 0;
  bool tail = false, fused = false, after_fine = false, widen_timed = false;
  unsigned long long seq = 0;
  bool ties_on = false, inline_ties = false;
  TieList tl{};
  BookView book{};
  const BookView* bookp = nullptr;
  double tp0 = 0, tpa = 0, tpb = 0, tpc = 0, tp1 = 0;
};
static const bool g_prof_pass = getenv("FLIMO_PROF_PASS") != nullptr;
static inline double now_us() { return std::chrono::duration<double, std::micro>(std::chrono::steady_clock::now().time_since_epoch()).count(); }

constexpr int PASS_NOTHING = 2000;
static int pass_plan(flimo_ctx* c, const double x26[26], const flimo_match_cfg* cfg, PassPlan& pl) {
  pl.cfg = cfg;
  pl.general_k = cfg->NUM_MATCH_POINTS != 5;
  pl.last_of_update = c->pipe_last_hint;
  c->pipe_last_hint = false;
  struct PreGuard { flimo_ctx* c; bool decided = false; ~PreGuard() { if (!decided) cancel_prelaunch(c); } } pre_guard{c};
  { const int rca = check_abandoned(c); if (rca) return rca; }
  c->last_nq = 0;
  c->last_cfg = *cfg;
  c->recs_valid = c->dbg_valid = false;
  if (!c->grid_valid && c->map_n > 0) { int rc0 = rebuild_grid(c); if (rc0) return rc0; }
  if (!c->grid_valid || c->map_n == 0) return PASS_NOTHING;
  size_t nq = c->scan_n;
  if (cfg->MAX_NUM_PC2MATCH >= 0 && nq > (size_t)cfg->MAX_NUM_PC2MATCH) nq = (size_t)cfg->MAX_NUM_PC2MATCH;
  if (nq == 0) return PASS_NOTHING;
  pl.nq = nq;
  (void)hipSetDevice(c->device);
  pl.grid_version = c->grid_builds * 0x100000000ull + c->grid_merges;
  bool use_pre = c->pre.active && !pl.general_k && c->prev.valid && c->pre.nq == nq && c->pre.seq == c->pass_seq + 1 &&
                 same_match_cfg(c->pre.cfg, *cfg) && c->pre.grid_version == pl.grid_version && !c->deskew_pending &&
                 !(nq < c->sorted_n || (c->sorted_n < c->scan_n && nq > c->sorted_n)) && c->pre.n_all == (int)c->sorted_n &&
                 !c->debug_recs && !(cfg->MAX_NUM_MATCHES >= 0 && (size_t)cfg->MAX_NUM_MATCHES < nq) &&
                 memcmp(c->pre.prev_RT, c->prev.RT, sizeof(c->pre.prev_RT)) == 0;
  if (use_pre && !(wall_s() - c->pre.t_launch < 0.25e-3 * (double)CH_POLL_MS)) { use_pre = false; c->pipe_aged++; }
  if (!use_pre) cancel_prelaunch(c);
  pre_guard.decided = true;
  int rc = ensure_recs(c, nq);
  if (rc) { cancel_prelaunch(c); return rc; }

  pl.tp0 = g_prof_pass ? now_us() : 0.0;
  pose_from_x26(x26, pl.P);
  MatchParams& mp = pl.mp;
  mp.max_dist_plane_d = cfg->MAX_DIST_PLANE;
  mp.plane_threshold = (float)cfg->PLANE_THRESHOLD;
  mp.estimate_extrinsics = cfg->estimate_extrinsics ? 1 : 0;
  mp.n_queries = (int)nq;
  mp.max_ring = gate_rings(c, cfg->MAX_DIST_PLANE);

  if (nq < c->sorted_n || (c->sorted_n < c->scan_n && nq > c->sorted_n)) {
    const size_t want = nq;
    { const int rcf = flush_deskew(c); if (rcf) return rcf; }
    HIPCHK(c, sort_scan(c->stream, c->d_scan, want, c->d_scan_sorted, c->scratch));
    c->sorted_n = want;
    c->prev.valid = 0;
  }
  pl.n_all = (int)c->sorted_n;
  const bool ride = c->deskew_pending && !pl.general_k && c->deskew_n == (size_t)pl.n_all &&
                    !(c->fine_valid && mp.max_ring >= 1);
  if (!ride) { const int rcf = flush_deskew(c); if (rcf) return rcf; }
  pl.dkp = ride ? &c->deskew_args : nullptr;
  c->deskew_pending = false;
  pl.cap_binds = cfg->MAX_NUM_MATCHES >= 0 && (size_t)cfg->MAX_NUM_MATCHES < nq;
  if (pl.general_k) return FLIMO_OK;
  pl.want_recs = c->debug_recs || pl.cap_binds;
  if (c->debug_recs) HIPCHK(c, hipMemsetAsync(c->d_cand, 0, sizeof(unsigned long long), c->stream));
  pl.want_count = c->debug_recs;
  pl.tpa = g_prof_pass ? now_us() : 0.0;
  pl.tlev = (c->timing == 1 && c->timing_stride > 1 && ((c->pass_seq + 1) % (unsigned long long)c->timing_stride) != 0) ? 0 : c->timing;
  pl.ev = (c->timing_deferred && c->ev_ring_made) ? c->ev_ring[c->ev_pending] : c->ev;
  const bool first_pass = !c->prev.valid;
  c->pass_in_scan = first_pass ? 0 : std::min(c->pass_in_scan + 1, 3);
  pl.tail_max = c->tail_max_env > 0 ? c->tail_max_env : std::max(1024, pl.n_all / 64);
  const bool tail_here = first_pass ? (c->stragglers_hist[0] <= pl.tail_max)
                                    : (c->stragglers_hist[c->pass_in_scan] <= pl.tail_max);
  pl.tail = c->tail && tail_here && mp.max_ring >= 2 && mp.max_ring <= 3;
  c->prev.probe_min = c->probe_min;
  pl.fused = pl.tail && c->fuse && !pl.want_recs;
  pl.seq = ++c->pass_seq;
  pl.ties_on = c->ties && c->gbook.active;
  pl.tl = TieList{};
  pl.tl.count_next = c->d_tie_count + ((pl.seq + 1) & 1);
  pl.inline_ties = pl.ties_on && !pl.want_recs;
  if (pl.ties_on && !pl.inline_ties) { pl.tl.list = c->d_tie_list; pl.tl.count = c->d_tie_count + (pl.seq & 1); pl.tl.cap = (unsigned)c->tie_cap; }
  pl.book = BookView{c->gbook.node_c, c->gbook.node_child, c->gbook.node_cnt, c->gbook.root, c->d_tie_settled};
  pl.bookp = pl.inline_ties ? &pl.book : nullptr;
  pl.after_fine = c->fine_valid && mp.max_ring >= 1;
  if (use_pre && !(pl.fused && !pl.after_fine && pl.tlev == 0)) {
    cancel_prelaunch(c);
    use_pre = false;
  }
  if (use_pre) {
    const int test_delay_ms = c->test_publish_delay_ms;
    if (wall_s() - c->pre.t_launch >= 0.25e-3 * (double)CH_POLL_MS) { cancel_prelaunch(c); use_pre = false; c->pipe_aged++; }
    else if (test_delay_ms > 0) std::this_thread::sleep_for(std::chrono::milliseconds(test_delay_ms));
  }
  pl.use_pre = pl.was_pre = use_pre;
  pl.widen_timed = !pl.tail && pl.tlev == 1 && mp.max_ring >= 2;
  pl.fused_cap = pl.cap_binds && !c->debug_recs;
  pl.use_fit2 = !pl.want_recs;
  return FLIMO_OK;
}

static int pass_general_k(flimo_ctx* c, const PassPlan& pl, double HTH[144], double HTh[12], int* M) {
  const flimo_match_cfg* cfg = pl.cfg;
  const int n_all = pl.n_all;
  const size_t nq = pl.nq;
  if ((size_t)n_all > c->nbrk_cap) {
    (void)hipFree(c->d_nbrk);
    c->d_nbrk = nullptr; c->nbrk_cap = 0;
    const size_t cap = (size_t)n_all + (size_t)n_all / 4 + 1024;
    HIPCHK(c, hipMalloc(&c->d_nbrk, cap * nbrk_rec_size()));
    c->nbrk_cap = cap;
  }
  c->prev.valid = 0;
  const BookView bookk{c->gbook.node_c, c->gbook.node_child, c->gbook.node_cnt, c->gbook.root, nullptr};
  if (!launch_match_k(c->stream, cfg->NUM_MATCH_POINTS, c->grid, c->d_scan_sorted, n_all, pl.P, pl.mp, c->d_nbrk, c->d_recs, c->d_dbg,
                      (c->ties && c->gbook.active) ? &bookk : nullptr))
    return fail(c, FLIMO_ERR_UNSUPPORTED, "NUM_MATCH_POINTS out of range");
  if (pl.cap_binds) launch_cap(c->stream, c->d_recs, (int)nq, cfg->MAX_NUM_MATCHES);
  launch_reduce(c->stream, c->d_recs, (int)nq, c->reduce_waves, c->d_partials, c->d_out256_host);
  HIPCHK(c, hipMemsetAsync(c->d_tie_count, 0, 2 * sizeof(unsigned int), c->stream));
  HIPCHK(c, hipGetLastError());
  run_overlap(c);
  HIPCHK(c, hipStreamSynchronize(c->stream));
  ++c->pass_seq;
  for (int i = 0; i < 12; i++) {
    for (int j = 0; j < 12; j++) HTH[i * 12 + j] = c->h_out256[c->mfma_idx[i][j]];
    HTh[i] = c->h_out256[c->mfma_idx[i][12]];
  }
  *M = (int)llround(c->h_out256[c->mfma_idx[13][13]]);
  c->last_nq = (int)nq;
  c->last_P = pl.P; c->last_mp = pl.mp; c->last_n_all = n_all;
  c->recs_valid = true; c->dbg_valid = true;
  c->last_stragglers = -1;
  c->async_deskews = 0;
  return FLIMO_OK;
}

static int pass_launch(flimo_ctx* c, PassPlan& pl) {
  const flimo_match_cfg* cfg = pl.cfg;
  const PoseMats& P = pl.P;
  const MatchParams& mp = pl.mp;
  const int n_all = pl.n_all;
  const size_t nq = pl.nq;
  const unsigned long long seq = pl.seq;
  const int tlev = pl.tlev;
  if (pl.use_pre) {
    publish_prelaunch(c, P, seq);
    c->fused_passes++;
  } else if (pl.after_fine) {
    launch_knn5_fine(c->stream, c->fine, c->d_scan_sorted, n_all, P, c->d_nbr, c->prev, c->fine_qlo, c->fine_qhi, &pl.tl, seq);
    c->fine_passes++;
  }
  if (pl.use_pre) {
  } else if (pl.fused) {
    launch_match_fused(c->stream, c->grid, c->d_scan_sorted, n_all, P, mp, c->d_nbr, c->d_wl, c->d_wl_count, nullptr, c->prev,
                       c->live_idx, c->d_fit2_partials, c->d_granules_host, c->d_ticket, seq, tlev == 1 ? pl.ev[0] : nullptr,
                       tlev == 1 ? pl.ev[1] : nullptr, &pl.tl, pl.after_fine ? 1 : 0, pl.dkp, nullptr, nullptr, pl.bookp);
    c->fused_passes++;
  } else
  launch_knn5(c->stream, 2, c->grid, c->d_scan_sorted, n_all, P, mp.max_ring, c->d_nbr, c->d_wl,
              c->d_wl_count, c->debug_recs ? c->d_cand : nullptr, c->prev, pl.tail ? 1 : 0, tlev == 1 ? pl.ev[0] : nullptr,
              tlev == 1 ? pl.ev[1] : nullptr, nullptr, &pl.tl, pl.after_fine ? 1 : 0, seq, pl.dkp);
  c->prev_before = c->prev;
  if (c->prune) { memcpy(c->prev.RT, P.RT, sizeof(c->prev.RT)); c->prev.valid = 1; }
  pl.tpb = g_prof_pass ? now_us() : 0.0;
  if (!pl.tail)
    launch_widen(c->stream, c->grid, c->d_scan_sorted, P, mp.max_ring, c->d_nbr, c->d_wl, c->d_wl_count,
                 c->debug_recs ? c->d_cand : nullptr, pl.widen_timed ? pl.ev[4] : nullptr, pl.widen_timed ? pl.ev[5] : nullptr, &pl.tl);
  pl.tpc = g_prof_pass ? now_us() : 0.0;
  if (pl.want_count) HIPCHK(c, hipMemcpyAsync(c->h_wl_count, c->d_wl_count, sizeof(int), hipMemcpyDeviceToHost, c->stream));
  if (pl.fused) {
  } else if (pl.use_fit2)
    launch_fit2(c->stream, c->grid, c->d_scan_sorted, n_all, c->d_nbr, P, mp, c->live_idx, c->d_fit2_partials, c->d_granules_host,
                c->d_ticket, c->d_wl_count, seq, tlev == 1 ? pl.ev[2] : nullptr, tlev == 1 ? pl.ev[3] : nullptr, &pl.tl, nullptr, nullptr, pl.bookp);
  else {
    HIPCHK(c, hipGetLastError());
    if (pl.ties_on) { launch_tie(c->stream, c->grid, pl.book, c->d_scan_sorted, P, c->d_nbr, pl.tl); HIPCHK(c, hipGetLastError()); }
    launch_fit(c->stream, c->grid, c->d_scan_sorted, n_all, c->d_nbr, P, mp, pl.fused_cap ? nullptr : c->d_fit_partials,
               pl.want_recs ? c->d_recs : nullptr, c->debug_recs ? c->d_dbg : nullptr, pl.cap_binds ? c->d_out256 : c->d_out256_host,
               c->d_ticket, c->d_wl_count, seq);
    HIPCHK(c, hipGetLastError());
    HIPCHK(c, hipMemsetAsync(c->d_tie_count, 0, 2 * sizeof(unsigned int), c->stream));
  }
  if (pl.fused_cap) {
    launch_capreduce(c->stream, c->d_recs, (int)nq, cfg->MAX_NUM_MATCHES, c->d_out256_host, c->d_wl_count, seq);
  } else if (pl.cap_binds) {
    launch_cap(c->stream, c->d_recs, (int)nq, cfg->MAX_NUM_MATCHES);
    launch_reduce(c->stream, c->d_recs, (int)nq, c->reduce_waves, c->d_partials, c->d_out256_host);
  }
  HIPCHK(c, hipGetLastError());
  pl.tp1 = g_prof_pass ? now_us() : 0.0;
  if (c->debug_recs) HIPCHK(c, hipMemcpyAsync(c->h_cand, c->d_cand, sizeof(unsigned long long), hipMemcpyDeviceToHost, c->stream));
  if (c->pipeline && !pl.last_of_update && c->d_pipe_head && c->prune && pl.use_fit2 && !pl.want_count && c->tail && c->fuse &&
      mp.max_ring >= 2 && mp.max_ring <= 3 && !c->fine_valid && pl.inline_ties == pl.ties_on) {
    const unsigned long long nseq = seq + 1;
    const int ntlev = (c->timing == 1 && c->timing_stride > 1 && (nseq % (unsigned long long)c->timing_stride) != 0) ? 0 : c->timing;
    const int npos = std::min(c->pass_in_scan + 1, 3);
    if (ntlev == 0 && c->stragglers_hist[npos] <= pl.tail_max) {
      TieList tln{};
      tln.count_next = c->d_tie_count + ((nseq + 1) & 1);
      ChainCtl pc{};
      pc.end_code = 0x80000000u | (++c->pipe_tag & 0x7fffffffu);
      PrevPass pv = c->prev;
      pv.valid = 1;
      launch_match_fused(c->stream, c->grid, c->d_scan_sorted, n_all, P, mp, c->d_nbr, c->d_wl, c->d_wl_count, nullptr, pv,
                         c->live_idx, c->d_fit2_partials, c->d_granules_host, c->d_ticket, nseq, nullptr, nullptr, &tln, 0, nullptr,
                         nullptr, &pc, pl.bookp, ch_epoch_of(nseq), c->d_pipe_head);
      HIPCHK(c, hipGetLastError());
      c->pre.active = true; c->pre.seq = nseq; c->pre.nq = nq; c->pre.n_all = n_all; c->pre.pos = npos; c->pre.cfg = *cfg;
      c->pre.grid_version = pl.grid_version; c->pre.end_code = pc.end_code; c->pre.t_launch = wall_s();
      memcpy(c->pre.prev_RT, pv.RT, sizeof(c->pre.prev_RT));
    }
  }
  return FLIMO_OK;
}

static int timing_read(flimo_ctx* c, hipEvent_t* ev, int kind) {
  const bool fused = kind & 1, use_fit2 = kind & 2, widen_timed = kind & 4;
  if (hipEventElapsedTime(&c->last_knn_ms, ev[0], ev[1]) != hipSuccess) {
    HIPCHK(c, hipEventSynchronize(ev[1]));
    (void)hipEventElapsedTime(&c->last_knn_ms, ev[0], ev[1]);
  }
  c->tot_knn_ms += c->last_knn_ms;
  if (fused) {
    c->last_fit_ms = 0.f; c->last_widen_ms = 0.f;
    c->split_fused_ms += c->last_knn_ms; c->split_fused_n++;
  } else if (use_fit2) {
    c->last_widen_ms = 0.f;
    if (widen_timed) {
      if (hipEventElapsedTime(&c->last_widen_ms, ev[4], ev[5]) != hipSuccess) c->last_widen_ms = 0.f;
      c->tot_widen_ms += c->last_widen_ms;
    }
    if (hipEventElapsedTime(&c->last_fit_ms, ev[2], ev[3]) != hipSuccess) {
      HIPCHK(c, hipEventSynchronize(ev[3]));
      (void)hipEventElapsedTime(&c->last_fit_ms, ev[2], ev[3]);
    }
    c->tot_fit_ms += c->last_fit_ms;
    c->split_knn_ms += c->last_knn_ms; c->split_widen_ms += c->last_widen_ms; c->split_fit_ms += c->last_fit_ms; c->split_sep_n++;
  }
  return FLIMO_OK;
}
static int timing_drain(flimo_ctx* c) {
  const int n = c->ev_pending;
  c->ev_pending = 0;
  for (int i = 0; i < n; i++) { const int rc = timing_read(c, c->ev_ring[i], c->ev_kind[i]); if (rc) return rc; }
  return FLIMO_OK;
}

static int pass_collect(flimo_ctx* c, PassPlan& pl, double HTH[144], double HTh[12], int* M) {
  const PoseMats& P = pl.P;
  const MatchParams& mp = pl.mp;
  const int n_all = pl.n_all;
  const size_t nq = pl.nq;
  const unsigned long long seq = pl.seq;
  const int tlev = pl.tlev;
  double acc[256];
  if (pl.use_fit2) {
    auto wait_granules = [&](unsigned long long want, int left_ms = -1) -> int {
      const int rcw = wait_tags(c, want, left_ms);
      if (rcw) return rcw;
      __atomic_thread_fence(__ATOMIC_ACQUIRE);
      return FLIMO_OK;
    };
    run_overlap(c);
    {
      int rcw = wait_granules(seq, pl.was_pre ? CH_POLL_MS + 25 : -1);
      if (rcw == FLIMO_PASS_LEFT) {
        cancel_prelaunch(c);
        c->pipe_left++;
        launch_match_fused(c->stream, c->grid, c->d_scan_sorted, n_all, P, mp, c->d_nbr, c->d_wl, c->d_wl_count, nullptr, c->prev_before,
                           c->live_idx, c->d_fit2_partials, c->d_granules_host, c->d_ticket, seq, nullptr, nullptr, &pl.tl, 0, nullptr, nullptr,
                           nullptr, pl.bookp);
        HIPCHK(c, hipGetLastError());
        rcw = wait_granules(seq);
      }
      if (rcw) return rcw;
    }
    c->last_stragglers = (int)llround(c->h_granules[2 * FIT_LIVE]);
    c->stragglers_hist[c->pass_in_scan] = c->last_stragglers;
    const long n_ties = (long)llround(c->h_granules[2 * (FIT_LIVE + 1)]);
    if (n_ties > 0 && pl.ties_on) {
      c->tie_redos++; c->tie_queries += (unsigned long long)n_ties;
      launch_tie(c->stream, c->grid, pl.book, c->d_scan_sorted, P, c->d_nbr, pl.tl);
      const unsigned long long seq2 = ++c->pass_seq;
      TieList tl2{};
      tl2.count_next = c->d_tie_count + ((seq2 + 1) & 1);
      launch_fit2(c->stream, c->grid, c->d_scan_sorted, n_all, c->d_nbr, P, mp, c->live_idx, c->d_fit2_partials, c->d_granules_host,
                  c->d_ticket, c->d_wl_count, seq2, nullptr, nullptr, &tl2);
      HIPCHK(c, hipGetLastError());
      const int rcw = wait_granules(seq2);
      if (rcw) return rcw;
    }
    double live[FIT_LIVE];
    for (int k = 0; k < FIT_LIVE; k++) {
      double r = c->h_granules[2 * k];
      for (int g = 1; g < FIT_GROUPS; g++) r += c->h_granules[((size_t)g * FIT_LIVE_PAD + k) * 2];
      live[k] = r;
    }
    for (int t = 0; t < 256; t++) acc[t] = 0.0;
    {
      int k = 0;
      for (int i = 0; i < 12; i++) for (int j = i; j < 12; j++) { acc[c->mfma_idx[i][j]] = live[k]; acc[c->mfma_idx[j][i]] = live[k]; k++; }
      for (int i = 0; i < 12; i++) acc[c->mfma_idx[i][12]] = live[k++];
      acc[c->mfma_idx[13][13]] = live[k++];
    }
  } else if (!c->debug_recs) {
    unsigned long long spins = 0;
    for (int g = 0; g < (pl.cap_binds ? 1 : FIT_GROUPS); g++) {
      volatile unsigned long long* flag = reinterpret_cast<volatile unsigned long long*>(c->h_out256 + (size_t)g * FIT_SLOT + 256);
      while (*flag != seq) {
        _mm_pause();
        if (++spins > 40000000ull) {
          HIPCHK(c, hipStreamSynchronize(c->stream));
          if (*flag != seq) return fail(c, FLIMO_ERR_HIP, "pass %llu completed without publishing its result", seq);
          break;
        }
      }
    }
    __atomic_thread_fence(__ATOMIC_ACQUIRE);
  } else {
    HIPCHK(c, hipStreamSynchronize(c->stream));
  }
  if (tlev) {
    const int kind = (pl.fused ? 1 : 0) | (pl.use_fit2 ? 2 : 0) | (pl.widen_timed ? 4 : 0);
    if (pl.ev != c->ev) {
      c->ev_kind[c->ev_pending++] = (unsigned char)kind;
      if (c->ev_pending == flimo_ctx::EV_RING) { const int rc = timing_drain(c); if (rc) return rc; }
    } else {
      const int rc = timing_read(c, c->ev, kind);
      if (rc) return rc;
    }
    c->tot_passes++; c->tot_queries += n_all;
  }
  if (g_prof_pass) {
    static double acc_launch = 0, acc_wait = 0, a0 = 0, a1 = 0, a2 = 0, a3 = 0; static long cnt = 0;
    const double tp2 = now_us();
    acc_launch += pl.tp1 - pl.tp0; acc_wait += tp2 - pl.tp1;
    a0 += pl.tpa - pl.tp0; a1 += pl.tpb - pl.tpa; a2 += pl.tpc - pl.tpb; a3 += pl.tp1 - pl.tpc;
    if (++cnt % 200 == 0) {
      fprintf(stderr, "[flimo pass] host: pose+launches %.2f us (prep %.2f, knn launch %.2f, widen launch %.2f, fit launch %.2f), wait for result %.2f us (mean of 200)\n",
              acc_launch / 200, a0 / 200, a1 / 200, a2 / 200, a3 / 200, acc_wait / 200);
      acc_launch = acc_wait = a0 = a1 = a2 = a3 = 0;
    }
  }
  c->async_deskews = 0;
  if (pl.want_count) c->last_widen_count = *c->h_wl_count;
  if (c->debug_recs) c->last_cand_per_query = (double)(*c->h_cand) / (double)nq;
  if (!pl.use_fit2) {
    c->last_stragglers = -1;
    const int slots = pl.cap_binds ? 1 : FIT_GROUPS;
    for (int t = 0; t < 256; t++) {
      double r = c->h_out256[t];
      for (int g = 1; g < slots; g++) r += c->h_out256[(size_t)g * FIT_SLOT + t];
      acc[t] = r;
    }
  }
  for (int i = 0; i < 12; i++) {
    for (int j = 0; j < 12; j++) HTH[i * 12 + j] = acc[c->mfma_idx[i][j]];
    HTh[i] = acc[c->mfma_idx[i][12]];
  }
  *M = (int)llround(acc[c->mfma_idx[13][13]]);
  c->last_nq = (int)nq;
  c->last_P = P; c->last_mp = mp; c->last_n_all = n_all;
  c->recs_valid = pl.want_recs && !pl.fused_cap;
  c->dbg_valid = c->debug_recs;
  return FLIMO_OK;
}

extern "C" int flimo_match_reduce(flimo_ctx* c, const double x26[26], const flimo_match_cfg* cfg, double HTH[144],
                                  double HTh[12], int* M) {
  if (!c || !x26 || !cfg || !HTH || !HTh || !M) return FLIMO_ERR_INVALID;
  if (cfg->NUM_MATCH_POINTS < 3 || cfg->NUM_MATCH_POINTS > 8)
    return fail(c, FLIMO_ERR_UNSUPPORTED, "NUM_MATCH_POINTS must be in 3..8 (a plane needs 3 points; the neighbour records hold 8)");
  for (int i = 0; i < 144; i++) HTH[i] = 0.0;
  for (int i = 0; i < 12; i++) HTh[i] = 0.0;
  *M = 0;
  PassPlan pl;
  int rc = pass_plan(c, x26, cfg, pl);
  if (rc == PASS_NOTHING) return FLIMO_OK;
  if (rc) return rc;
  if (pl.general_k) return pass_general_k(c, pl, HTH, HTh, M);
  if ((rc = pass_launch(c, pl)) != FLIMO_OK) return rc;
  return pass_collect(c, pl, HTH, HTh, M);
}

extern "C" int flimo_set_update_mode(flimo_ctx* c, int mode) {
  if (!c || mode < 0 || mode > 2) return FLIMO_ERR_INVALID;
  c->update_mode = mode;
  c->host_update = mode == 1 || (mode == 0 && auto_host_update(c));
  return FLIMO_OK;
}
extern "C" int flimo_set_pass_pipeline(flimo_ctx* c, int on) {
  if (!c) return FLIMO_ERR_INVALID;
  cancel_prelaunch(c);
  if (!c->pipeline_env) c->pipeline = on != 0;
  if (c->update_mode == 0) c->host_update = auto_host_update(c);
  return FLIMO_OK;
}
extern "C" int flimo_pass_pipeline_end(flimo_ctx* c) {
  if (!c) return FLIMO_ERR_INVALID;
  cancel_prelaunch(c);
  return FLIMO_OK;
}
extern "C" int flimo_pass_pipeline_last(flimo_ctx* c) {
  if (!c) return FLIMO_ERR_INVALID;
  c->pipe_last_hint = true;
  return FLIMO_OK;
// ... 865 lines not shown
```

fast_limo_amd/csrc/hip/flimo_kernels.h:

```cpp
#pragma once
#include <hip/hip_runtime.h>
#include "flimo_types.h"

namespace flimo {
struct FuseArgs;
struct TieList;
struct BookView;
struct ChainCtl;
struct PipeHead;
struct ChainHead;
struct DeskewArgs {
  const float4* raw; const double* t; const void* frames; int nf; const float* mats; double t_offset;
  float4* out_sorted; float4* out_orig; int on;
  int stage_words;
};

void launch_knn5(hipStream_t st, int lanes_per_query, const GridView& G, const float4* scan_sorted, int n,
                 const PoseMats& P, int max_ring, void* nbr, int* wl, int* wl_count, unsigned long long* cand,
                 const PrevPass& prev, int tail, hipEvent_t e0 = nullptr, hipEvent_t e1 = nullptr, const struct FuseArgs* fuse = nullptr,
                 const TieList* ties = nullptr, int after_fine = 0, unsigned long long seq = 0ull, const DeskewArgs* deskew = nullptr,
                 const ChainHead* chain = nullptr);
void launch_knn5_fine(hipStream_t st, const GridView& Gf, const float4* scan_sorted, int n, const PoseMats& P, void* nbr,
                      const PrevPass& prev, const int qlo[3], const int qhi[3], const TieList* ties, unsigned long long seq,
                      const ChainHead* chain = nullptr);
void launch_widen(hipStream_t st, const GridView& G, const float4* scan_sorted, const PoseMats& P, int max_ring, void* nbr,
                  int* wl, int* wl_count, unsigned long long* cand, hipEvent_t e0 = nullptr, hipEvent_t e1 = nullptr,
                  const TieList* ties = nullptr, const ChainHead* chain = nullptr);
int fit_blocks(int n);
void set_xcd_stripe(int stripe);
constexpr int FIT_GROUPS = 8;
constexpr int FIT_SLOT = 264;
void launch_fit(hipStream_t st, const GridView& G, const float4* scan_sorted, int n, const void* nbr, const PoseMats& P,
                const MatchParams& mp, double* partials, Rec16* recs, RecDbg* dbg, double* out256, unsigned int* ticket,
                int* wl_count, unsigned long long seq);
constexpr int FIT_LIVE = 91;
constexpr int FIT_LIVE_PAD = 96;
int fit2_blocks(int n);
void launch_fit2(hipStream_t st, const GridView& G, const float4* scan_sorted, int n, const void* nbr, const PoseMats& P,
                 const MatchParams& mp, const unsigned char* live_idx, double* partials, void* out_granules, unsigned int* ticket,
                 int* wl_count, unsigned long long seq, hipEvent_t e0 = nullptr, hipEvent_t e1 = nullptr, const TieList* ties = nullptr,
                 const ChainHead* chain = nullptr, const ChainCtl* ctl = nullptr, const BookView* book = nullptr);
constexpr int FUSED_SPREAD_SLOTS = 32768;
int fused_spread(int n);
int fused_blocks(int n);
void launch_match_fused(hipStream_t st, const GridView& G, const float4* scan_sorted, int n, const PoseMats& P, const MatchParams& mp,
                        void* nbr, int* wl, int* wl_count, unsigned long long* cand, const PrevPass& prev,
                        const unsigned char* live_idx, double* partials, void* out_granules, unsigned int* ticket,
                        unsigned long long seq, hipEvent_t e0 = nullptr, hipEvent_t e1 = nullptr, const TieList* ties = nullptr,
                        int after_fine = 0, const DeskewArgs* deskew = nullptr, const ChainHead* chain = nullptr,
                        const ChainCtl* ctl = nullptr, const BookView* book = nullptr, unsigned int wait_epoch = 0u,
                        const PipeHead* pipe = nullptr);
struct BookView { const float4* node_c; const int* node_child; const int* node_cnt; int root; unsigned long long* settled; };
struct TieList { int* list; unsigned int* count; unsigned int cap; unsigned int* count_next; };
void launch_tie(hipStream_t st, const GridView& G, const BookView& B, const float4* scan_sorted, const PoseMats& P, void* nbr,
                const TieList& tl);
void launch_knn_tie(hipStream_t st, const GridView& G, const BookView& B, const float* qxyz, int nq, int k, int32_t* idx, float* sqd,
                    const int32_t* cnt);
size_t nbrk_rec_size();
bool launch_match_k(hipStream_t st, int k, const GridView& G, const float4* scan_sorted, int n, const PoseMats& P,
                    const MatchParams& mp, void* nbrk, Rec16* recs, RecDbg* dbg, const BookView* book = nullptr);
size_t nbr_rec_size();
size_t wl_entry_size();
void launch_knn(hipStream_t st, const GridView& G, const float* qxyz, int nq, int k, int max_ring, int32_t* idx,
                float* sqd, int32_t* cnt);
void launch_cap(hipStream_t st, Rec16* recs, int n, int cap);
void launch_capreduce(hipStream_t st, const Rec16* recs, int n, int cap, double* out256, int* wl_count, unsigned long long seq);
void launch_reduce(hipStream_t st, const Rec16* recs, int n, int nwaves, double* partials, double* out256);
void launch_mfma_layout(hipStream_t st, double* raw256);
void launch_word_probe(hipStream_t st, const unsigned int* src, void* out_granule, unsigned long long tag);
void launch_rtt_probe(hipStream_t st, void* out_granule, unsigned long long tag);
void launch_deskew(hipStream_t st, const float4* in, const double* t, int n, const void* frames, int nf,
                   const float* mats32, float4* out_sorted, float4* out_orig, double t_offset = 0.0);
void launch_transform(hipStream_t st, const float4* in, int n, const PoseMats& P, float4* out);
bool launch_deskew_debug(hipStream_t st, const DeskewArgs& dk, int n, const PoseMats& P, float4* out_world, float4* out_final);
size_t dev_frame_size();

struct MapBuildScratch {
  void* cub_tmp = nullptr;
  size_t cub_tmp_bytes = 0;
  uint32_t* keys_in = nullptr;
  uint32_t* keys_out = nullptr;
  uint32_t* vals_in = nullptr;
  uint32_t* vals_out = nullptr;
  size_t cap_pts = 0;
  unsigned long long *ck_in = nullptr, *ck_out = nullptr;
  size_t ck_cap = 0;
  float* bbox = nullptr;
  uint32_t* mail_host = nullptr;
  uint32_t* mail_dev = nullptr;
  uint32_t mail_seq = 0;
  unsigned long long* filt_desc = nullptr;
  size_t filt_tiles_cap = 0;
  unsigned int filt_epoch = 0, filt_ticket_base = 0;
  unsigned long long* filt_mail_host = nullptr;
  unsigned long long* filt_mail_dev = nullptr;
  unsigned long long* crop_desc = nullptr;
  size_t crop_tiles_cap = 0;
  unsigned int* carve_img = nullptr;
  size_t carve_img_words = 0;
};
enum MailSlot { MAIL_BOOK = 0 , MAIL_BOOK_END = 8 , MAIL_CROWD = 12, MAIL_BOXCOUNT = 13, MAIL_BBOX = 16 , MAIL_VOXEL = 24 , MAIL_TILES = 28 , MAIL_ROWS = 32 , MAIL_ESCAPES = 33 , MAIL_CROP = 36 , MAIL_CARVE = 37 ,
                MAIL_TAG = 62 , MAIL_WORDS = 64 };
struct MailPart { const void* src; int n; int dst; };
hipError_t mail_words(hipStream_t st, MapBuildScratch& S, const MailPart* parts, int nparts, bool rearm_bbox = false, void* zero = nullptr,
                      int zero_n = 0);
hipError_t ensure_mail(MapBuildScratch& S);
hipError_t mail_wait(hipStream_t st, MapBuildScratch& S);
hipError_t map_crop_compact(hipStream_t st, const float4* in, size_t n, const float lo[3], const float hi[3], float4* out, int blocks,
                            MapBuildScratch& S, size_t* kept, float bb[6]);

struct CarveCfg { float s[3]; int res, win; float margin, rel_margin, max_depth; };
hipError_t carve_image(hipStream_t st, const float4* scan, size_t n, const PoseMats& P, const CarveCfg& cfg, MapBuildScratch& S);
hipError_t carve_mask(hipStream_t st, const float4* in, size_t n, const CarveCfg& cfg, MapBuildScratch& S, unsigned char* d_mask, size_t* count);
hipError_t map_carve_compact(hipStream_t st, const float4* in, size_t n, const CarveCfg& cfg, const float* lo, const float* hi, float4* out,
                             int blocks, MapBuildScratch& S, size_t* kept, float bb[6]);

hipError_t map_mask_compact(hipStream_t st, const float4* in, size_t n, const unsigned char* d_mask, size_t first, size_t n_mask, float4* out,
                            int blocks, MapBuildScratch& S, size_t* kept, float bb[6]);

hipError_t map_bbox(hipStream_t st, const float4* pts, size_t n, MapBuildScratch& S, float bbox_host[6]);
hipError_t sort_scan(hipStream_t st, const float4* in, size_t n, float4* out, MapBuildScratch& S,
                     const double* t_in = nullptr, double* t_out = nullptr);
hipError_t index_scan(hipStream_t st, const float4* in, size_t n, float4* out, const double* t_in, double* t_out);
constexpr size_t index_escape_words(size_t pts_cap) { return (pts_cap / 16 + 64) * 8; }
// ... 144 lines not shown
```

fast_limo_amd/csrc/hip/flimo_kernels.hip:

```cpp
#include <hip/hip_runtime.h>
#include <hip/hip_ext.h>
#include <float.h>
#include <limits.h>
#include <stdlib.h>
#include <algorithm>
#include "flimo_types.h"
#include "flimo_math.h"
#include "flimo_kernels.h"
#include "flimo_chain.h"
#include "flimo_ieskf.h"

#pragma clang fp contract(off)

namespace flimo {

FLIMO_DEV bool pair_less(float d0, int i0, float d1, int i1) { return (d0 < d1) || (d0 == d1 && i0 < i1); }

template <int K>
FLIMO_DEV void topk_insert(float (&bd)[K], int (&bi)[K], float d, int id) {
  if (!pair_less(d, id, bd[K - 1], bi[K - 1])) return;
  bd[K - 1] = d;
  bi[K - 1] = id;
#pragma unroll
  for (int s = K - 1; s > 0; s--) {
// ... 625 lines not shown
        float tq = fl_sqrt(Rm[4] - Rm[8] - Rm[0] + 1.0f);
        uy_ = 0.5f * tq;
        tq = fl_div(0.5f, tq);
        uw_ = (Rm[2] - Rm[6]) * tq;
        uz_ = (Rm[7] + Rm[5]) * tq;
        ux_ = (Rm[1] + Rm[3]) * tq;
      } else {
        float tq = fl_sqrt(Rm[8] - Rm[0] - Rm[4] + 1.0f);
        uz_ = 0.5f * tq;
        tq = fl_div(0.5f, tq);
        uw_ = (Rm[3] - Rm[1]) * tq;
        ux_ = (Rm[2] + Rm[6]) * tq;
        uy_ = (Rm[5] + Rm[7]) * tq;
      }
    }
  }
  const float nqw = qw * uw_ - qx * ux_ - qy * uy_ - qz * uz_;
  const float nqx = qw * ux_ + qx * uw_ + qy * uz_ - qz * uy_;
  const float nqy = qw * uy_ + qy * uw_ + qz * ux_ - qx * uz_;
  const float nqz = qw * uz_ + qz * uw_ + qx * uy_ - qy * ux_;
  const float fdt = (float)dt;
  const float px = F.p[0] + (fdt * F.v[0] + fdt * (fdt * (0.5f * a0x)));
  const float py = F.p[1] + (fdt * F.v[1] + fdt * (fdt * (0.5f * a0y)));
  const float pz = F.p[2] + (fdt * F.v[2] + fdt * (fdt * (0.5f * a0z)));
  float R0[9];
  quat_to_rot(nqx, nqy, nqz, nqw, R0);
  const float X[16] = {R0[0], R0[1], R0[2], px, R0[3], R0[4], R0[5], py, R0[6], R0[7], R0[8], pz, 0.f, 0.f, 0.f, 1.f};
  float T[16];
#pragma unroll
  for (int i = 0; i < 4; i++)
#pragma unroll
    for (int j = 0; j < 4; j++) {
      float acc = X[i * 4 + 0] * mats[0 * 4 + j];
      acc = acc + X[i * 4 + 1] * mats[1 * 4 + j];
      acc = acc + X[i * 4 + 2] * mats[2 * 4 + j];
      acc = acc + X[i * 4 + 3] * mats[3 * 4 + j];
      T[i * 4 + j] = acc;
    }
  float wx_ = ((T[0] * p.x + T[1] * p.y) + T[2] * p.z) + T[3] * 1.f;
  float wy_ = ((T[4] * p.x + T[5] * p.y) + T[6] * p.z) + T[7] * 1.f;
  float wz_ = ((T[8] * p.x + T[9] * p.y) + T[10] * p.z) + T[11] * 1.f;
  float ww_ = ((T[12] * p.x + T[13] * p.y) + T[14] * p.z) + T[15] * 1.f;
  return make_float4(wx_, wy_, wz_, ww_);
}

__device__ __forceinline__ float4 deskew_body(const float4 wp, const float* __restrict__ mats, float w) {
  const float* Li = mats + 16;
  const float ox_ = ((Li[0] * wp.x + Li[1] * wp.y) + Li[2] * wp.z) + Li[3] * wp.w;
  const float oy_ = ((Li[4] * wp.x + Li[5] * wp.y) + Li[6] * wp.z) + Li[7] * wp.w;
  const float oz_ = ((Li[8] * wp.x + Li[9] * wp.y) + Li[10] * wp.z) + Li[11] * wp.w;
  return make_float4(ox_, oy_, oz_, w);
}

__device__ __forceinline__ float4 deskew_point(const float4 p, const double tk, const DevFrame* __restrict__ frames, int nf,
                                               const float* __restrict__ mats) {
  return deskew_body(deskew_world(p, tk, frames, nf, mats), mats, p.w);
}

__global__ __launch_bounds__(256) void deskew_kernel(const float4* __restrict__ in, const double* __restrict__ t,
                                                     int n, const DevFrame* __restrict__ frames, int nf,
                                                     const float* __restrict__ mats, float4* __restrict__ out_sorted,
                                                     float4* __restrict__ out_orig, double t_offset) {
  const int k = blockIdx.x * blockDim.x + threadIdx.x;
  if (k >= n) return;
  const float4 o = deskew_point(in[k], t[k] + t_offset, frames, nf, mats);
  out_sorted[k] = o;
  out_orig[__float_as_uint(o.w)] = make_float4(o.x, o.y, o.z, 1.0f);
}

struct FuseArgs {
  int fine_mode;
  int qlo[3], qhi[3];
  TieList tl;
  MatchParams mp;
  FitIdx idx;
  double* partials;
  double2* granules;
  unsigned int* ticket;
  unsigned long long seq;
  DeskewArgs dk;
  BookView book;
  ChainCtl ch;
  int spread;
};
template <int ROWS>
__device__ __forceinline__ void fit_reduce_publish(const float (&v)[16], bool owns_row, int row, float* sr, double* sa0, double* sa1,
                                                   double* sa2, double* sa3, unsigned int* s_last, const FitIdx& idx,
                                                   double* __restrict__ partials, double2* __restrict__ out_granules,
                                                   unsigned int* __restrict__ ticket, int* __restrict__ wl_count,
                                                   unsigned long long seq, const TieList& tl, int blk = -1, int nblk = -1);
FLIMO_DEV void fit_row(const GridView& G, const PoseMats& P, const MatchParams& mp, const int (&ids)[5], float gx, float gy, float gz,
                       float (&v)[16]);

struct TieLds;
__device__ bool tie_select_wave(const GridView& G, const BookView& B, float qx, float qy, float qz, float dk, int k, TieLds& S,
                                uint32_t (&out_pos)[8], float (&out_d)[8]);
__device__ __forceinline__ void tie_repair_wave(const GridView& G, const BookView& B, NbrRec* __restrict__ nbr, bool mine_tied, int p,
                                                float gx, float gy, float gz, uint32_t d5bits, int (&ids)[5], TieLds& TS) {
  const int lane = threadIdx.x & 63;
  unsigned long long tm = __ballot(mine_tied);
  while (tm) {
    const int tlane = __ffsll((long long)tm) - 1;
    tm &= tm - 1ull;
    const float qx = __int_as_float(__builtin_amdgcn_readlane(__float_as_int(gx), tlane));
    const float qy = __int_as_float(__builtin_amdgcn_readlane(__float_as_int(gy), tlane));
    const float qz = __int_as_float(__builtin_amdgcn_readlane(__float_as_int(gz), tlane));
    const float dk = __int_as_float(__builtin_amdgcn_readlane((int)d5bits, tlane));
    uint32_t pos[8];
    float d[8];
#pragma unroll
    for (int s_ = 0; s_ < 8; s_++) { pos[s_] = 0u; d[s_] = 0.f; }
    wave_lds_sync();
    const bool ok = tie_select_wave(G, B, qx, qy, qz, dk, 5, TS, pos, d);
    int got[5];
#pragma unroll
    for (int s_ = 0; s_ < 5; s_++) got[s_] = __builtin_amdgcn_readlane((int)pos[s_], 0);
    if (ok && lane == tlane) {
#pragma unroll
      for (int s_ = 0; s_ < 5; s_++) ids[s_] = got[s_];
      int4* rec = reinterpret_cast<int4*>(&nbr[p]);
      rec[0] = make_int4(got[0], got[1], got[2], got[3]);
      rec[1] = make_int4(got[4], 1, (int)d5bits, 1);
      if (B.settled) atomicAdd(B.settled, 1ull);
    }
    wave_lds_sync();
  }
}

#ifdef FLIMO_WPE
#define KNN_WPE __attribute__((amdgpu_waves_per_eu(FLIMO_WPE, FLIMO_WPE)))
#else
#define KNN_WPE
#endif
struct DirRegs { uint4 v[GRID_DIR_MAX / 8 / 256]; };
__device__ __forceinline__ DirRegs grid_dir_fetch(const GridView& G) {
  const int n16 = (G.ntx * G.nty * G.ntz + 7) >> 3;
  const uint4* src = reinterpret_cast<const uint4*>(G.dir);
  DirRegs r;
#pragma unroll
  for (int k = 0; k < GRID_DIR_MAX / 8 / 256; k++)
    r.v[k] = (int)threadIdx.x + 256 * k < n16 ? src[threadIdx.x + 256 * k] : make_uint4(0u, 0u, 0u, 0u);
  return r;
}
__device__ __forceinline__ void grid_dir_store(uint16_t* s_dir, const DirRegs& r) {
  uint4* dst = reinterpret_cast<uint4*>(s_dir);
#pragma unroll
  for (int k = 0; k < GRID_DIR_MAX / 8 / 256; k++) dst[threadIdx.x + 256 * k] = r.v[k];
  __syncthreads();
}
template <int L, int SLOTS, bool FUSE, bool FINE = false>
__device__ __forceinline__ void knn5_pass(const GridView& G, uint16_t* dir, const DirRegs* dir_pending, const float4* __restrict__ scan_sorted, int n,
                                          const PoseMats& P, int max_ring, NbrRec* __restrict__ nbr,
                                          int* __restrict__ wl, int* __restrict__ wl_count,
                                          unsigned long long* __restrict__ cand_total, const float* __restrict__ prev_RT, int prev_valid,
                                          unsigned prev_probe_min, int tail, const FuseArgs& fa) {
  constexpr int QPB = 256 / L;
  const TieList tl = fa.tl;
  __shared__ WaveLds s_w[4];
  __shared__ unsigned int s_last;
  static_assert(sizeof(WaveLds) * 4 >= (size_t)IESKF_LDS_BYTES, "the filter's algebra runs in this workgroup's shared memory");
  int nb = (int)gridDim.x;
  if constexpr (FUSE) {
    if (fa.ch.S) {
      nb -= 1;
      if ((int)blockIdx.x == nb) {
        double* big = reinterpret_cast<double*>(s_w);
// ... 289 lines not shown
            uint32_t s0 = (uint32_t)sub;
            for (; s0 + (SLOTS / 2) * L < total2; s0 += SLOTS * L)
              knn5_body<L, SLOTS, FINE>(G.pts, s0, total2, last, off2, dl2, gx, gy, gz, kb);
            if (s0 < total2) knn5_body<L, (SLOTS >= 2 ? SLOTS / 2 : 1), FINE>(G.pts, s0, total2, last, off2, dl2, gx, gy, gz, kb);
          }
          cand += total2 > (uint32_t)sub ? (int)((total2 - (uint32_t)sub + L - 1) / L) : 0;
          double cb[6], cc[6];
          key_pair_merge6(kb, cb);
          key_merge6(c, cb, cc);
          if (two || split_walk) {
#pragma unroll
            for (int i = 0; i < 6; i++) c[i] = cc[i];
          }
        }
#pragma unroll
        for (int i = 0; i < 5; i++) best[i] = (u64)__double_as_longlong(c[i]);
        sixth = (u64)__double_as_longlong(c[5]);
      } else if (L > 1) {
        u64 mine[6];
#pragma unroll
        for (int i = 0; i < 5; i++) mine[i] = best[i];
        mine[5] = sixth;
#pragma unroll
        for (int r = 0; r < 6; r++) {
          double md = __longlong_as_double((long long)mine[0]);
#pragma unroll
          for (int o = 1; o < L; o <<= 1) md = key_min(md, __shfl_xor(md, o, 64));
          const u64 m = (u64)__double_as_longlong(md);
          if (r < 5) best[r] = m; else sixth = m;
          if (mine[0] == m) { mine[0] = mine[1]; mine[1] = mine[2]; mine[2] = mine[3]; mine[3] = mine[4]; mine[4] = mine[5]; mine[5] = KEY_NONE; }
        }
      }
      const float edge = fminf(fminf(fminf(rx, 1.f - rx), fminf(ry, 1.f - ry)), fminf(rz, 1.f - rz));
      const float rg = (1.f + edge - margin) * G.cell;
      const float d5 = __uint_as_float((uint32_t)(best[4] >> 32));
      const bool have5 = d5 < INFINITY;
      const bool covers = (cx - 1 <= 0) && (cx + 1 >= G.nx - 1) && (cy - 1 <= 0) && (cy + 1 >= G.ny - 1) &&
                          (cz - 1 <= 0) && (cz + 1 >= G.nz - 1);
      if (have5 && (covers || d5 <= rg * rg * (1.f - 1.0e-6f))) {
        flag = 1;
        tie = key_has_tie(best, sixth);
      }
      else if (covers) flag = 0;
      else flag = (max_ring > 1) ? 2 : 0;
    }
  }
  if (cand_total) {
    int c = cand;
#pragma unroll
    for (int o = 1; o < L; o <<= 1) c += __shfl_xor(c, o, 64);
    if (sub == 0 && in_range) atomicAdd(cand_total, (unsigned long long)c);
  }
  if constexpr (FINE) {
    const bool inside = qcx >= fa.qlo[0] && qcx <= fa.qhi[0] && qcy >= fa.qlo[1] && qcy <= fa.qhi[1] && qcz >= fa.qlo[2] && qcz <= fa.qhi[2];
    if (in_range && sub == 0 && flag == 1 && inside) {
      int4 a, b;
      a.x = (int)(uint32_t)best[0]; a.y = (int)(uint32_t)best[1]; a.z = (int)(uint32_t)best[2]; a.w = (int)(uint32_t)best[3];
      b.x = (int)(uint32_t)best[4]; b.y = 4; b.z = (int)(uint32_t)(best[4] >> 32);
      b.w = (int)(1u | (tie ? 2u : 0u) | ((uint32_t)(fa.seq & 0xffffffull) << 8));
      int4* o = reinterpret_cast<int4*>(&nbr[p]);
      o[0] = a;
      o[1] = b;
      if (tie && tl.list) { const unsigned slot = atomicAdd(tl.count, 1u); if (slot < tl.cap) tl.list[slot] = p; }
    }
    return;
  }
  TRACE(0, 4);
  const bool pend_tail = tail && in_range && flag == 2;
  if (in_range && sub == 0 && !pend_tail) {
    int4 a, b;
    a.x = (int)(uint32_t)best[0]; a.y = (int)(uint32_t)best[1]; a.z = (int)(uint32_t)best[2]; a.w = (int)(uint32_t)best[3];
    b.x = (int)(uint32_t)best[4]; b.y = min(flag, 2); b.z = (int)(uint32_t)(best[4] >> 32); b.w = ((flag == 1) ? 1 : 0) | (tie ? 2 : 0);
    if (tie && !tie_listed && tl.list) { const unsigned slot = atomicAdd(tl.count, 1u); if (slot < tl.cap) tl.list[slot] = p; }
    int4* o = reinterpret_cast<int4*>(&nbr[p]);
    o[0] = a;
    o[1] = b;
    if (flag >= 2) {
      const int slot = atomicAdd(wl_count, 1);
      int4* e = reinterpret_cast<int4*>(wl) + 2 * (size_t)slot;
      e[0] = make_int4(p, __float_as_int(gx), __float_as_int(gy), __float_as_int(gz));
      e[1] = make_int4((int)(uint32_t)(best[4] >> 32), 2, __float_as_int(b2), 0);
    }
  }
  WaveLds& W = s_w[threadIdx.x >> 6];
  if (tail) knn5_tail(G, dir, max_ring, nbr, pend_tail && sub == 0, p, gx, gy, gz, (uint32_t)(best[4] >> 32), b2, W, wl_count, cand_total, FUSE, tl);
  TRACE(0, 5);
  if constexpr (FUSE) {
    const int lane = threadIdx.x & 63;
    float v[16];
#pragma unroll
    for (int i = 0; i < 16; i++) v[i] = 0.f;
    wave_lds_sync();
    int ids[5] = {(int)(uint32_t)best[0], (int)(uint32_t)best[1], (int)(uint32_t)best[2], (int)(uint32_t)best[3], (int)(uint32_t)best[4]};
    int fl = flag;
    bool tied = tie;
    uint32_t d5b = (uint32_t)(best[4] >> 32);
    if (sub == 0 && in_range && pend_tail) {
      const int4* rr = reinterpret_cast<const int4*>(W.res[lane]);
      const int4 a = rr[0], b = rr[1];
      ids[0] = a.x; ids[1] = a.y; ids[2] = a.z; ids[3] = a.w; ids[4] = b.x;
      fl = b.y;
      tied = (b.w & 2) != 0;
      d5b = (uint32_t)b.z;
    }
    if (fa.book.node_c)
      tie_repair_wave(G, fa.book, nbr, sub == 0 && in_range && fl == 1 && tied, p, gx, gy, gz, d5b, ids, *reinterpret_cast<TieLds*>(W.tile));
    TRACE(1, 1);
    if (sub == 0 && in_range) {
      if (fl == 1 && __float_as_uint(sp.w) < (uint32_t)fa.mp.n_queries) fit_row(G, P, fa.mp, ids, gx, gy, gz, v);
    }
    TRACE(1, 3);
    wave_lds_sync();
    fit_reduce_publish<64 / L>(v, sub == 0, lane / L, W.tile, s_w[0].acc, s_w[1].acc, s_w[2].acc, s_w[3].acc, &s_last, fa.idx,
                               fa.partials, fa.granules, fa.ticket, wl_count, fa.seq, tl, (int)blockIdx.x, nb);
  }
  TRACE_FLUSH();
}

template <int L, int SLOTS, bool FUSE, bool FINE = false>
__global__ __launch_bounds__(256) KNN_WPE void knn5_kernel(GridView G, const float4* __restrict__ scan_sorted, int n,
                                                   PoseMats P, int max_ring, NbrRec* __restrict__ nbr,
                                                   int* __restrict__ wl, int* __restrict__ wl_count,
                                                   unsigned long long* __restrict__ cand_total, PrevPass prev, int tail,
                                                   FuseArgs fa) {
  __shared__ __align__(16) uint16_t s_dir[GRID_DIR_MAX];
  const DirRegs dr = grid_dir_fetch(G);
  __shared__ PoseMats s_pose;
  static_assert(sizeof(PoseMats) % 4 == 0 && sizeof(PoseMats) / 4 <= 256, "one word per thread");
  if (threadIdx.x < sizeof(PoseMats) / 4)
    reinterpret_cast<uint32_t*>(&s_pose)[threadIdx.x] = reinterpret_cast<const uint32_t*>(&P)[threadIdx.x];
  knn5_pass<L, SLOTS, FUSE, FINE>(G, s_dir, &dr, scan_sorted, n, s_pose, max_ring, nbr, wl, wl_count, cand_total, prev.RT, prev.valid, prev.probe_min, tail, fa);
}
__device__ __forceinline__ const ChainHead* chain_enter(const ChainHead* __restrict__ H, const PipeHead* __restrict__ pipe, const PrevRT& prt,
                                                        unsigned int wait_epoch, unsigned int end_code) {
  constexpr int NW = (int)(sizeof(ChainHead) / 4);
  __shared__ unsigned int s_head[NW];
  __shared__ int s_go;
  if (pipe != nullptr) {
    const int tid = (int)threadIdx.x;
    if (tid < 64) {
      const unsigned long long t0 = wall_clock64();
      int go = 0;
      unsigned long long gv = 0ull;
      unsigned int* dec = const_cast<unsigned int*>(&pipe->decision);
      const unsigned int v_go = wait_epoch, v_pend = wait_epoch | 0x80000000u, v_no = (wait_epoch & 0x3fffffffu) | 0x80000000u;
      for (int look = 0;; look++) {
        const unsigned int d = __hip_atomic_load(dec, __ATOMIC_RELAXED, __HIP_MEMORY_SCOPE_SYSTEM);
        gv = __hip_atomic_load(&pipe->gran[tid], __ATOMIC_RELAXED, __HIP_MEMORY_SCOPE_SYSTEM);
        const unsigned int e = (unsigned int)(gv >> 32);
        const bool all = __ballot(e == wait_epoch) == ~0ull;
        const unsigned int e0 = (unsigned int)__builtin_amdgcn_readfirstlane((int)e);
        if (d == v_no) break;
        if (d == v_pend) { __builtin_amdgcn_s_sleep(8); continue; }
        if (all) { go = 1; break; }
        if (e0 == end_code) break;
        const unsigned long long waited = wall_clock64() - t0;
        if (blockIdx.x == 0 && d != v_go && waited > (unsigned long long)CH_POLL_MS * 100000ull) {
          if (tid == 0) __hip_atomic_store(dec, v_pend, __ATOMIC_RELAXED, __HIP_MEMORY_SCOPE_SYSTEM);
          asm volatile("s_waitcnt vmcnt(0)" ::: "memory");
          for (int nap = 0; nap < 4; nap++) __builtin_amdgcn_s_sleep(127);
          gv = __hip_atomic_load(&pipe->gran[tid], __ATOMIC_RELAXED, __HIP_MEMORY_SCOPE_SYSTEM);
          go = __ballot((unsigned int)(gv >> 32) == wait_epoch) == ~0ull ? 1 : 0;
          if (tid == 0) __hip_atomic_store(dec, go ? v_go : v_no, __ATOMIC_RELAXED, __HIP_MEMORY_SCOPE_SYSTEM);
          break;
        }
        if (waited > 4ull * (unsigned long long)CH_POLL_MS * 100000ull) break;
        if (look == 0) __builtin_amdgcn_s_sleep(48);
        else __builtin_amdgcn_s_sleep(8);
      }
      if (go && tid < PH_WORDS) s_head[tid < 36 ? (tid / 12) * 16 + tid % 12 : tid + 12] = (unsigned int)gv;
      if (tid == 0) s_go = go;
    } else if (tid < 64 + 12) {
      const int k = tid - 64;
      s_head[(k / 4) * 16 + 12 + k % 4] = __float_as_uint(k % 4 == 3 ? 1.f : 0.f);
    } else if (tid >= 128 && tid < 128 + 16) {
      s_head[offsetof(ChainHead, prev_RT) / 4 + (tid - 128)] = __float_as_uint(prt.v[tid - 128]);
    } else if (tid >= 192 && tid < 192 + NW - (int)(offsetof(ChainHead, status) / 4)) {
      s_head[offsetof(ChainHead, status) / 4 + (tid - 192)] = 0u;
    }
    __syncthreads();
    if (!s_go) return nullptr;
  } else {
    if ((int)threadIdx.x < NW) s_head[threadIdx.x] = reinterpret_cast<const unsigned int*>(H)[threadIdx.x];
    __syncthreads();
  }
  const ChainHead* Lh = reinterpret_cast<const ChainHead*>(s_head);
  return Lh->status != 0 ? nullptr : Lh;
}
template <int L, int SLOTS, bool FUSE, bool FINE = false>
__global__ __launch_bounds__(256) KNN_WPE void knn5_chain_kernel(GridView G, const float4* __restrict__ scan_sorted, int n,
                                                   const ChainHead* __restrict__ H, int max_ring, NbrRec* __restrict__ nbr,
                                                   int* __restrict__ wl, int* __restrict__ wl_count,
                                                   unsigned long long* __restrict__ cand_total, int prev_valid, unsigned probe_min, int tail,
                                                   FuseArgs fa, unsigned int wait_epoch, const PipeHead* __restrict__ pipe, PrevRT prt) {
  __shared__ __align__(16) uint16_t s_dir[GRID_DIR_MAX];
  {
    const DirRegs dr = grid_dir_fetch(G);
    grid_dir_store(s_dir, dr);
  }
  const ChainHead* Lh = chain_enter(H, pipe, prt, wait_epoch, fa.ch.end_code);
  if (!Lh) return;
  knn5_pass<L, SLOTS, FUSE, FINE>(G, s_dir, nullptr, scan_sorted, n, Lh->pose, max_ring, nbr, wl, wl_count, cand_total, Lh->prev_RT, prev_valid, probe_min, tail, fa);
}

__device__ __forceinline__ void widen_body(const GridView& G, int max_ring, NbrRec* __restrict__ nbr,
                                           const int* __restrict__ wl, const int* __restrict__ wl_count,
                                           unsigned long long* __restrict__ cand_total, int first_ring, const TieList& tl,
                                           int blk, int nblk, uint32_t (*s_off)[65], uint32_t (*s_lo)[64]) {
  const int lane = threadIdx.x & 63, wave = threadIdx.x >> 6;
  const int maxdim = grid_maxdim(G);
  const float margin = 1.0e-3f + 4.0e-7f * (float)maxdim;
  int w = blk * 4 + wave;
  const int4* entries = reinterpret_cast<const int4*>(wl);
  int4 e0 = entries[2 * (size_t)w], e1 = entries[2 * (size_t)w + 1];
  const int count = *wl_count;
  for (; w < count; w += nblk * 4) {
    if (w != blk * 4 + wave) { e0 = entries[2 * (size_t)w]; e1 = entries[2 * (size_t)w + 1]; }
    const int p = e0.x;
    const float gx = __int_as_float(e0.y), gy = __int_as_float(e0.z), gz = __int_as_float(e0.w);
    const int hint_bits = e1.x;
    const float fx = (gx - G.ox) * G.inv_cell, fy = (gy - G.oy) * G.inv_cell, fz = (gz - G.oz) * G.inv_cell;
    const float flx = floorf(fminf(fmaxf(fx, -1.0e9f), 1.0e9f)), fly = floorf(fminf(fmaxf(fy, -1.0e9f), 1.0e9f)),
                flz = floorf(fminf(fmaxf(fz, -1.0e9f), 1.0e9f));
    const int cx = (int)flx - G.six, cy = (int)fly - G.siy, cz = (int)flz - G.siz;
    const float rx = fminf(fmaxf(fx - flx, 0.f), 1.f), ry = fminf(fmaxf(fy - fly, 0.f), 1.f),
                rz = fminf(fmaxf(fz - flz, 0.f), 1.f);
    const float edge = fminf(fminf(fminf(rx, 1.f - rx), fminf(ry, 1.f - ry)), fminf(rz, 1.f - rz));
    u64 best[5] = {KEY_NONE, KEY_NONE, KEY_NONE, KEY_NONE, KEY_NONE};
    u64 sixth = KEY_NONE;
    int flag = 0;
    int cand = 0;
    int r = first_ring;
    float bnd2 = __int_as_float(e1.z);
    if (!(bnd2 >= 0.f)) bnd2 = INFINITY;
    {
      const float hint = __int_as_float(hint_bits);
      if (hint >= 0.f && hint < INFINITY) {
        const float need = fl_sqrt(hint) * G.inv_cell * (1.f + 4.0e-6f) - edge + margin;
        r = max(2, (int)ceilf(fminf(need, 1.0e9f)));
        const float rc = (fl_sqrt(hint) * (1.f + 1.0e-5f) + 1.0e-6f) * G.inv_cell;
        bnd2 = fminf(bnd2, rc * rc * (1.f + 1.0e-5f));
      }
      r = min(r, max_ring);
    }
    for (;;) {
      const int side = 2 * r + 1;
      uint32_t lo = 0, len = 0;
      if (lane < side * side) {
        const int dy = (lane % side) - r, dz = (lane / side) - r;
        const int yy = cy + dy, zz = cz + dz;
        const float a_ = fmaxf(slab_dist(dy, ry) - margin, 0.f), b_ = fmaxf(slab_dist(dz, rz) - margin, 0.f);
        const float dyz2 = a_ * a_ + b_ * b_;
        int x0 = max(cx - r, 0), x1 = min(cx + r, G.nx - 1);
        if (bnd2 < 1.0e18f) {
          const float xr = fl_sqrt(fmaxf(bnd2 - dyz2, 0.f)) * (1.f + 1.0e-6f) + margin + 1.0e-4f;
          const int dr = (int)fminf(floorf(fminf(xr + rx, 1.0e6f)), (float)r);
          const int dl = (int)fminf(floorf(fminf(xr + (1.f - rx), 1.0e6f)), (float)r);
          x0 = max(cx - dl, 0); x1 = min(cx + dr, G.nx - 1);
        }
        if (dyz2 <= bnd2 && yy >= 0 && yy < G.ny && zz >= 0 && zz < G.nz && x0 <= x1) {
          uint32_t hi_;
          grid_row_range(G, G.dir, yy, zz, x0 * G.xs, (x1 + 1) * G.xs, lo, hi_);
          len = hi_ - lo;
        }
      }
      uint32_t inc = len;
#pragma unroll
      for (int o = 1; o < 64; o <<= 1) {
        const uint32_t v = __shfl_up(inc, o, 64);
        if (lane >= o) inc += v;
      }
      const uint32_t total = __shfl(inc, 63, 64);
      s_off[wave][lane + 1] = inc;
      if (lane == 0) s_off[wave][0] = 0;
      s_lo[wave][lane] = lo;
      __builtin_amdgcn_wave_barrier();
      const double none = __longlong_as_double((long long)KEY_NONE);
      double k5[6] = {none, none, none, none, none, none};
      const uint32_t last = total - 1u;
      for (uint32_t s0 = (uint32_t)lane; s0 < total; s0 += 4 * 64) {
        float4 q[4];
        uint32_t id[4];
#pragma unroll
        for (int u = 0; u < 4; u++) {
          const uint32_t s = min(s0 + 64u * u, last);
          int a = 0;
#pragma unroll
          for (int step = 32; step >= 1; step >>= 1) a = (s_off[wave][a + step] <= s) ? a + step : a;
          id[u] = s_lo[wave][a] + (s - s_off[wave][a]);
          q[u] = G.pts[id[u]];
        }
        asm volatile("" : "+v"(q[0].x), "+v"(q[0].y), "+v"(q[0].z), "+v"(q[1].x), "+v"(q[1].y), "+v"(q[1].z),
                          "+v"(q[2].x), "+v"(q[2].y), "+v"(q[2].z), "+v"(q[3].x), "+v"(q[3].y), "+v"(q[3].z));
#pragma unroll
        for (int u = 0; u < 4; u++) {
          const bool live = s0 + 64u * u < total;
          const float d = sqdist3(gx, gy, gz, q[u].x, q[u].y, q[u].z);
          best6_insert(k5, key_make(live ? d : INFINITY, live ? id[u] : 0xffffffffu));
        }
      }
      cand += total > (uint32_t)lane ? (int)((total - (uint32_t)lane + 63u) / 64u) : 0;
      __builtin_amdgcn_wave_barrier();
      u64 mine[6];
#pragma unroll
      for (int i = 0; i < 6; i++) mine[i] = (u64)__double_as_longlong(k5[i]);
#pragma unroll
      for (int k = 0; k < 6; k++) {
        const double md = key_group_min(__longlong_as_double((long long)mine[0]), 64, lane);
        const u64 m = (u64)__double_as_longlong(md);
        if (k < 5) best[k] = m; else sixth = m;
        if (mine[0] == m) { mine[0] = mine[1]; mine[1] = mine[2]; mine[2] = mine[3]; mine[3] = mine[4]; mine[4] = mine[5]; mine[5] = KEY_NONE; }
      }
      const float rg = ((float)r + edge - margin) * G.cell;
      const float d5 = __uint_as_float((uint32_t)(best[4] >> 32));
      const bool have5 = d5 < INFINITY;
      const bool covers = (cx - r <= 0) && (cx + r >= G.nx - 1) && (cy - r <= 0) && (cy + r >= G.ny - 1) &&
                          (cz - r <= 0) && (cz + r >= G.nz - 1);
      if (have5 && (covers || d5 <= rg * rg * (1.f - 1.0e-6f))) { flag = 1; break; }
      if (covers || r >= max_ring) { flag = 0; break; }
      int rn = r + 1;
      if (have5) {
        const float need = fl_sqrt(d5) * G.inv_cell * (1.f + 4.0e-6f) - edge + margin;
        rn = max(r + 1, (int)ceilf(fminf(need, 1.0e9f)));
        const float rc = (fl_sqrt(d5) * (1.f + 1.0e-5f) + 1.0e-6f) * G.inv_cell;
        bnd2 = fminf(bnd2, rc * rc * (1.f + 1.0e-5f));
      }
      r = min(rn, max_ring);
    }
    if (cand_total) {
      int c = cand;
#pragma unroll
      for (int o = 1; o < 64; o <<= 1) c += __shfl_xor(c, o, 64);
      if (lane == 0) atomicAdd(cand_total, (unsigned long long)c);
    }
    if (lane == 0) {
      int4 a, b;
      a.x = (int)(uint32_t)best[0]; a.y = (int)(uint32_t)best[1]; a.z = (int)(uint32_t)best[2]; a.w = (int)(uint32_t)best[3];
      const bool tie = flag == 1 && key_has_tie(best, sixth);
      b.x = (int)(uint32_t)best[4]; b.y = flag; b.z = (int)(uint32_t)(best[4] >> 32); b.w = ((flag == 1) ? 1 : 0) | (tie ? 2 : 0);
      int4* o = reinterpret_cast<int4*>(&nbr[p]);
      o[0] = a;
      o[1] = b;
      if (tie && tl.list) { const unsigned slot = atomicAdd(tl.count, 1u); if (slot < tl.cap) tl.list[slot] = p; }
    }
  }
}
__global__ __launch_bounds__(256) void widen_kernel(GridView G, const float4* __restrict__ scan_sorted, PoseMats P,
                                                    int max_ring, NbrRec* __restrict__ nbr, const int* __restrict__ wl,
                                                    const int* __restrict__ wl_count,
                                                    unsigned long long* __restrict__ cand_total, int first_ring, TieList tl,
                                                    const ChainHead* __restrict__ H) {
  __shared__ uint32_t s_off[4][65];
  __shared__ uint32_t s_lo[4][64];
  if (H && H->status != 0) return;
  widen_body(G, max_ring, nbr, wl, wl_count, cand_total, first_ring, tl, (int)blockIdx.x, (int)gridDim.x, s_off, s_lo);
}

__global__ __launch_bounds__(256) void widen_general_kernel(GridView G, const float4* __restrict__ scan_sorted,
                                                            PoseMats P, int max_ring, NbrRec* __restrict__ nbr,
                                                            const int* __restrict__ wl, const int* __restrict__ wl_count, TieList tl) {
  constexpr int L = 16;
  const int count = *wl_count;
  const int sub = threadIdx.x % L;
  for (int w = blockIdx.x * (256 / L) + threadIdx.x / L; w < count; w += gridDim.x * (256 / L)) {
    const int p = reinterpret_cast<const int4*>(wl)[2 * (size_t)w].x;
    const float4 sp = scan_sorted[p];
    float gx, gy, gz;
    xform4(P.RT, sp.x, sp.y, sp.z, gx, gy, gz);
    KnnResult R;
    knn_search<L>(G, gx, gy, gz, sub, max_ring, R);
    if (sub == 0) {
      const bool ok = R.exact && (R.bi[4] != INT_MAX);
      int4 a, b;
      a.x = R.bi[0]; a.y = R.bi[1]; a.z = R.bi[2]; a.w = R.bi[3];
      b.x = R.bi[4]; b.y = ok ? 1 : 0; b.z = ok ? __float_as_int(R.bd[4]) : 0; b.w = ok ? 3 : 0;
      int4* o = reinterpret_cast<int4*>(&nbr[p]);
      o[0] = a;
      o[1] = b;
      if (ok && tl.list) { const unsigned slot = atomicAdd(tl.count, 1u); if (slot < tl.cap) tl.list[slot] = p; }
    }
  }
}

typedef double double4_t __attribute__((ext_vector_type(4)));


template <bool RECS, bool DBG, int FIT_THREADS>
__global__ __launch_bounds__(FIT_THREADS) void fit_kernel(GridView G, const float4* __restrict__ scan_sorted, int n,
                                                          const NbrRec* __restrict__ nbr, PoseMats P, MatchParams mp,
                                                          double* __restrict__ partials, Rec16* __restrict__ recs,
                                                          RecDbg* __restrict__ dbg, double* __restrict__ out256,
                                                          unsigned int* __restrict__ ticket, int* __restrict__ wl_count,
                                                          unsigned long long seq) {
  constexpr int FIT_WAVES = FIT_THREADS / 64;
  __shared__ float s_rec[FIT_WAVES][16 * 65];
  __shared__ double s_acc[FIT_WAVES][256];
  __shared__ unsigned int s_last;
  const int chunk = xcd_chunk(blockIdx.x, gridDim.x);
  const int p = chunk * FIT_THREADS + threadIdx.x;
  const int lane = threadIdx.x & 63, wave = threadIdx.x >> 6;

  float v[16];
#pragma unroll
  for (int i = 0; i < 16; i++) v[i] = 0.f;
  float n4[4] = {0.f, 0.f, 0.f, 0.f};
  float gx = 0.f, gy = 0.f, gz = 0.f;
  float sq[5] = {0.f, 0.f, 0.f, 0.f, 0.f};
  int ids[5] = {-1, -1, -1, -1, -1};
  int flag = 0;
  uint32_t orig = 0;
  bool valid = false;
  TRACE(1, 0);
  if (p < n) {
    const float4 sp = scan_sorted[p];
    orig = __float_as_uint(sp.w);
    xform4(P.RT, sp.x, sp.y, sp.z, gx, gy, gz);
    const int4* nb = reinterpret_cast<const int4*>(&nbr[p]);
    const int4 a = nb[0], b = nb[1];
    ids[0] = a.x; ids[1] = a.y; ids[2] = a.z; ids[3] = a.w; ids[4] = b.x;
    flag = b.y;
    valid = (flag == 1) && (orig < (uint32_t)mp.n_queries);
    TRACE(1, 1);
    if (valid) {
      float px[5], py[5], pz[5];
#pragma unroll
      for (int s = 0; s < 5; s++) {
// ... 192 lines not shown
    __hip_atomic_store(&partials[(size_t)fb * FIT_LIVE_PAD + threadIdx.x], r, __ATOMIC_RELAXED, __HIP_MEMORY_SCOPE_AGENT);
  }
  asm volatile("s_waitcnt vmcnt(0)" ::: "memory");
  __syncthreads();
  TRACE(1, 4);
  const int group = fb & (FIT_GROUPS - 1);
  const int nb_g = fnb / FIT_GROUPS;
  if (threadIdx.x == 0) {
    const unsigned int old = __hip_atomic_fetch_add(ticket + group, 1u, __ATOMIC_RELAXED, __HIP_MEMORY_SCOPE_AGENT);
    *s_last = (old == (unsigned int)nb_g - 1u) ? 1u : 0u;
  }
  __syncthreads();
  TRACE(1, 5);
  if (*s_last) {
    unsigned int launch_ticket = 0xffffffffu;
    unsigned int* launch_slot = ticket + FIT_GROUPS;
    asm volatile("" : "+v"(launch_slot));
    if (threadIdx.x == 255) launch_ticket = __hip_atomic_fetch_add(launch_slot, 1u, __ATOMIC_RELAXED, __HIP_MEMORY_SCOPE_AGENT);
    const int c2 = (int)threadIdx.x % (FIT_LIVE_PAD / 2), sl = (int)threadIdx.x / (FIT_LIVE_PAD / 2);
    const int per = (nb_g + 4) / 5;
    const int k0 = sl * per, k1 = sl < 5 ? min(nb_g, k0 + per) : 0;
    v2d_t a0 = {0.0, 0.0}, a1 = {0.0, 0.0};
    {
      const double* base = partials + (size_t)group * FIT_LIVE_PAD + 2 * c2;
      const size_t stride = (size_t)FIT_GROUPS * FIT_LIVE_PAD;
      for (int k = k0; k < k1; k += 16) {
        const double* q[16];
#pragma unroll
        for (int u = 0; u < 16; u++) q[u] = base + (size_t)min(k + u, k1 - 1) * stride;
        v2d_t w[16];
        asm volatile(
            "global_load_dwordx4 %0, %16, off sc1\n\tglobal_load_dwordx4 %1, %17, off sc1\n\t"
            "global_load_dwordx4 %2, %18, off sc1\n\tglobal_load_dwordx4 %3, %19, off sc1\n\t"
            "global_load_dwordx4 %4, %20, off sc1\n\tglobal_load_dwordx4 %5, %21, off sc1\n\t"
            "global_load_dwordx4 %6, %22, off sc1\n\tglobal_load_dwordx4 %7, %23, off sc1\n\t"
            "global_load_dwordx4 %8, %24, off sc1\n\tglobal_load_dwordx4 %9, %25, off sc1\n\t"
            "global_load_dwordx4 %10, %26, off sc1\n\tglobal_load_dwordx4 %11, %27, off sc1\n\t"
            "global_load_dwordx4 %12, %28, off sc1\n\tglobal_load_dwordx4 %13, %29, off sc1\n\t"
            "global_load_dwordx4 %14, %30, off sc1\n\tglobal_load_dwordx4 %15, %31, off sc1\n\t"
            "s_waitcnt vmcnt(0)"
            : "=&v"(w[0]), "=&v"(w[1]), "=&v"(w[2]), "=&v"(w[3]), "=&v"(w[4]), "=&v"(w[5]), "=&v"(w[6]), "=&v"(w[7]), "=&v"(w[8]),
              "=&v"(w[9]), "=&v"(w[10]), "=&v"(w[11]), "=&v"(w[12]), "=&v"(w[13]), "=&v"(w[14]), "=&v"(w[15])
            : "v"(q[0]), "v"(q[1]), "v"(q[2]), "v"(q[3]), "v"(q[4]), "v"(q[5]), "v"(q[6]), "v"(q[7]), "v"(q[8]), "v"(q[9]), "v"(q[10]),
              "v"(q[11]), "v"(q[12]), "v"(q[13]), "v"(q[14]), "v"(q[15])
            : "memory");
#pragma unroll
        for (int u = 0; u < 16; u += 2) {
          if (k + u < k1) a0 += w[u];
          if (k + u + 1 < k1) a1 += w[u + 1];
        }
      }
    }
    asm volatile("" : "+v"(launch_ticket));
    const bool launch_last = launch_ticket == (unsigned int)FIT_GROUPS - 1u;
    int n_wl = 0;
    unsigned int n_tie = 0u;
    if (launch_last) {
      n_wl = __hip_atomic_load(wl_count, __ATOMIC_RELAXED, __HIP_MEMORY_SCOPE_AGENT);
      if (tl.count) n_tie = __hip_atomic_load(tl.count, __ATOMIC_RELAXED, __HIP_MEMORY_SCOPE_AGENT);
    }
    __syncthreads();
    if (sl < 5) {
      double* dstb = sl < 2 ? sa0 + sl * FIT_LIVE_PAD : (sl < 4 ? sa1 + (sl - 2) * FIT_LIVE_PAD : sa2);
      dstb[2 * c2] = a0.x + a1.x;
      dstb[2 * c2 + 1] = a0.y + a1.y;
    }
    __syncthreads();
    TRACE(1, 6);
    if (threadIdx.x < FIT_LIVE) {
      v2d_t g;
      g.x = ((sa0[threadIdx.x] + sa0[FIT_LIVE_PAD + threadIdx.x]) + (sa1[threadIdx.x] + sa1[FIT_LIVE_PAD + threadIdx.x])) + sa2[threadIdx.x];
      g.y = __longlong_as_double((long long)seq);
      double2* o = out_granules + (size_t)group * FIT_LIVE_PAD + threadIdx.x;
      asm volatile("global_store_dwordx4 %0, %1, off sc0 sc1\n\ts_nop 1" :: "v"(o), "v"(g) : "memory");
    }
    if (threadIdx.x == 0) __hip_atomic_store(ticket + group, 0u, __ATOMIC_RELAXED, __HIP_MEMORY_SCOPE_AGENT);
    asm volatile("" : "+v"(n_wl), "+v"(n_tie));
    if (launch_last) publish_counters(n_wl, n_tie, out_granules, ticket, wl_count, seq, tl);
    if (launch_last) TRACE_LANE(1, 2, 255);
    TRACE(1, 7);
  }
}

template <int PPW>
__device__ __forceinline__ void fit2_pass(const GridView& G, const float4* __restrict__ scan_sorted, int n,
                                          const NbrRec* __restrict__ nbr, const PoseMats& P, const MatchParams& mp, const FitIdx& idx,
                                          double* __restrict__ partials, double2* __restrict__ out_granules,
                                          unsigned int* __restrict__ ticket, int* __restrict__ wl_count,
                                          unsigned long long seq, const TieList& tl, const ChainCtl& ch, const BookView& book) {
  __shared__ __align__(16) float s_rec[4][16 * 65];
  __shared__ double s_acc[4][256];
  __shared__ unsigned int s_last;
  static_assert(sizeof(float) * 4 * 16 * 65 >= (size_t)IESKF_LDS_BYTES, "the filter's algebra runs in this workgroup's shared memory");
  int nb = (int)gridDim.x;
  if (ch.S) {
    nb -= 1;
    if ((int)blockIdx.x == nb) {
      double* big = reinterpret_cast<double*>(&s_rec[0][0]);
      ik_extra_block(ch, big, (int)threadIdx.x);
      return;
    }
  }
  const int lane = threadIdx.x & 63, wave = threadIdx.x >> 6;
  const int chunk = xcd_chunk(blockIdx.x, nb);
  const int p = (chunk * 4 + wave) * PPW + lane;
  float v[16];
#pragma unroll
  for (int i = 0; i < 16; i++) v[i] = 0.f;
  TRACE(1, 0);
  {
    const bool mine = lane < PPW && p < n;
    const float4 sp = scan_sorted[mine ? p : 0];
    const int4* nb = reinterpret_cast<const int4*>(&nbr[mine ? p : 0]);
    const int4 a = nb[0], b = nb[1];
    float gx, gy, gz;
    xform4(P.RT, sp.x, sp.y, sp.z, gx, gy, gz);
    int ids[5] = {a.x, a.y, a.z, a.w, b.x};
    TRACE(1, 1);
    if (book.node_c)
      tie_repair_wave(G, book, const_cast<NbrRec*>(nbr), mine && b.y == 1 && (b.w & 2) != 0, p, gx, gy, gz, (uint32_t)b.z, ids,
                      *reinterpret_cast<TieLds*>(&s_rec[wave][0]));
    if (mine && b.y == 1 && __float_as_uint(sp.w) < (uint32_t)mp.n_queries) fit_row(G, P, mp, ids, gx, gy, gz, v);
  }
  TRACE(1, 3);
  fit_reduce_publish<PPW>(v, lane < PPW, lane, s_rec[wave], s_acc[0], s_acc[1], s_acc[2], s_acc[3], &s_last, idx, partials,
                          out_granules, ticket, wl_count, seq, tl, (int)blockIdx.x, nb);
}

template <int PPW>
__global__ __launch_bounds__(256) void fit2_kernel(GridView G, const float4* __restrict__ scan_sorted, int n,
                                                   const NbrRec* __restrict__ nbr, PoseMats P, MatchParams mp, FitIdx idx,
                                                   double* __restrict__ partials, double2* __restrict__ out_granules,
                                                   unsigned int* __restrict__ ticket, int* __restrict__ wl_count,
                                                   unsigned long long seq, TieList tl, ChainCtl ch, BookView book) {
  fit2_pass<PPW>(G, scan_sorted, n, nbr, P, mp, idx, partials, out_granules, ticket, wl_count, seq, tl, ch, book);
}
template <int PPW>
__global__ __launch_bounds__(256) void fit2_chain_kernel(GridView G, const float4* __restrict__ scan_sorted, int n,
                                                   const NbrRec* __restrict__ nbr, const ChainHead* __restrict__ H, MatchParams mp, FitIdx idx,
                                                   double* __restrict__ partials, double2* __restrict__ out_granules,
                                                   unsigned int* __restrict__ ticket, int* __restrict__ wl_count,
                                                   unsigned long long seq, TieList tl, ChainCtl ch, BookView book) {
  if (H->status != 0) return;
  fit2_pass<PPW>(G, scan_sorted, n, nbr, H->pose, mp, idx, partials, out_granules, ticket, wl_count, seq, tl, ch, book);
}

__constant__ unsigned char c_ordered_indices[8][7] = {
    {1, 2, 4, 3, 5, 6, 7}, {0, 3, 5, 2, 4, 7, 6}, {0, 3, 6, 1, 4, 7, 5}, {1, 2, 7, 0, 5, 6, 4},
    {0, 5, 6, 1, 2, 7, 3}, {1, 4, 7, 0, 3, 6, 2}, {2, 4, 7, 0, 3, 5, 1}, {3, 5, 6, 1, 2, 4, 0}};

__device__ __forceinline__ int book_morton(float x, float y, float z, const float4& c) {
  return (x > c.x ? 1 : 0) | (y > c.y ? 2 : 0) | (z > c.z ? 4 : 0);
}
__device__ __forceinline__ int visit_pos(int m, int c) {
  if (c == m) return 0;
  int pos = 8;
#pragma unroll
  for (int i = 0; i < 7; i++) pos = (c_ordered_indices[m][i] == c) ? 1 + i : pos;
  return pos;
}
__device__ bool visited_before(const BookView& B, float ax, float ay, float az, uint32_t ra, float bx, float by, float bz, uint32_t rb,
                               float qx, float qy, float qz) {
  int node = B.root;
  for (int depth = 0; depth < 64 && node >= 0; depth++) {
    if (B.node_cnt[node] >= 0) break;
    const float4 c = B.node_c[node];
    const int ca = book_morton(ax, ay, az, c), cb = book_morton(bx, by, bz, c);
    if (ca != cb) {
      const int m = book_morton(qx, qy, qz, c);
      return visit_pos(m, ca) < visit_pos(m, cb);
    }
    node = B.node_child[(size_t)node * 8 + ca];
  }
  return ra < rb;
}

struct TieLds { float4 pt[64]; float d[64]; uint32_t pos[64]; unsigned int cnt; };

__device__ bool tie_select_wave(const GridView& G, const BookView& B, float qx, float qy, float qz, float dk, int k, TieLds& S,
                                uint32_t (&out_pos)[8], float (&out_d)[8]) {
  const int lane = threadIdx.x & 63;
  const int maxdim = grid_maxdim(G);
  const float margin = 1.0e-3f + 4.0e-7f * (float)maxdim;
  const float fx = (qx - G.ox) * G.inv_cell, fy = (qy - G.oy) * G.inv_cell, fz = (qz - G.oz) * G.inv_cell;
  const float flx = floorf(fminf(fmaxf(fx, -1.0e9f), 1.0e9f)), fly = floorf(fminf(fmaxf(fy, -1.0e9f), 1.0e9f)),
              flz = floorf(fminf(fmaxf(fz, -1.0e9f), 1.0e9f));
  const int cx = (int)flx - G.six, cy = (int)fly - G.siy, cz = (int)flz - G.siz;
  const float rx = fminf(fmaxf(fx - flx, 0.f), 1.f), ry = fminf(fmaxf(fy - fly, 0.f), 1.f), rz = fminf(fmaxf(fz - flz, 0.f), 1.f);
  const float edge = fminf(fminf(fminf(rx, 1.f - rx), fminf(ry, 1.f - ry)), fminf(rz, 1.f - rz));
  const float need = fl_sqrt(dk) * G.inv_cell * (1.f + 4.0e-6f) - edge + margin;
  int r = max(1, (int)ceilf(fminf(need, 1.0e9f)));
  {
    const float rg = ((float)r + edge - margin) * G.cell;
    if (!(dk <= rg * rg * (1.f - 1.0e-6f))) r++;
  }
  if (r > 64) return false;
  if (lane == 0) S.cnt = 0u;
  wave_lds_sync();
  const int side = 2 * r + 1, rows = side * side;
  const float rc = (fl_sqrt(dk) * (1.f + 1.0e-5f) + 1.0e-6f) * G.inv_cell;
  const float bnd2 = rc * rc * (1.f + 1.0e-5f);
  for (int jb = 0; jb < rows; jb += 64) {
    const int j = jb + lane;
    if (j < rows) {
      const int jz = j / side, jy = j - jz * side;
      const int dy = jy - r, dz = jz - r;
      const int yy = cy + dy, zz = cz + dz;
      const float a = fmaxf(slab_dist(dy, ry) - margin, 0.f), b = fmaxf(slab_dist(dz, rz) - margin, 0.f);
      const float dyz2 = a * a + b * b;
      if (dyz2 <= bnd2 && yy >= 0 && yy < G.ny && zz >= 0 && zz < G.nz) {
        const float xr = fl_sqrt(fmaxf(bnd2 - dyz2, 0.f)) * (1.f + 1.0e-6f) + margin + 1.0e-4f;
        const int dr = (int)fminf(floorf(fminf(xr + rx, 1.0e6f)), (float)r);
        const int dl = (int)fminf(floorf(fminf(xr + (1.f - rx), 1.0e6f)), (float)r);
        const int x0 = max(cx - dl, 0), x1 = min(cx + dr, G.nx - 1);
        if (x0 <= x1) {
          uint32_t lo, hi;
          grid_row_range(G, G.dir, yy, zz, x0 * G.xs, (x1 + 1) * G.xs, lo, hi);
          for (uint32_t i = lo; i < hi; i++) {
            const float4 p = G.pts[i];
            const float d = sqdist3(qx, qy, qz, p.x, p.y, p.z);
            if (d <= dk) {
              const unsigned slot = atomicAdd(&S.cnt, 1u);
              if (slot < 64u) { S.pt[slot] = p; S.d[slot] = d; S.pos[slot] = i; }
            }
          }
        }
      }
// ... 492 lines not shown
    *wl_count = 0;
  }
}

__global__ void mfma_layout_kernel(double* __restrict__ raw) {
  const int lane = threadIdx.x;
  const int rc = lane & 15, k = lane >> 4;
  const double a = (k == 0) ? 1.0 : (k == 1 ? (double)rc : 0.0);
  const double b = (k == 0) ? (double)rc : (k == 1 ? 16.0 : 0.0);
  double4_t acc = {0.0, 0.0, 0.0, 0.0};
  acc = __builtin_amdgcn_mfma_f64_16x16x4f64(a, b, acc, 0, 0, 0);
  raw[lane * 4 + 0] = acc[0]; raw[lane * 4 + 1] = acc[1]; raw[lane * 4 + 2] = acc[2]; raw[lane * 4 + 3] = acc[3];
}

__global__ void word_probe_kernel(const unsigned int* __restrict__ src, double2* __restrict__ out, unsigned long long tag) {
  const unsigned int w = __hip_atomic_load(src, __ATOMIC_RELAXED, __HIP_MEMORY_SCOPE_SYSTEM);
  typedef double v2d_t __attribute__((ext_vector_type(2)));
  v2d_t g;
  g.x = (double)w;
  g.y = __longlong_as_double((long long)tag);
  asm volatile("global_store_dwordx4 %0, %1, off sc0 sc1\n\ts_nop 1" :: "v"(out), "v"(g) : "memory");
}
__global__ void rtt_probe_kernel(double2* __restrict__ out, unsigned long long tag) {
  typedef double v2d_t __attribute__((ext_vector_type(2)));
  v2d_t g;
  g.x = 1.0;
  g.y = __longlong_as_double((long long)tag);
  asm volatile("global_store_dwordx4 %0, %1, off sc0 sc1\n\ts_nop 1" :: "v"(out), "v"(g) : "memory");
}
void launch_rtt_probe(hipStream_t st, void* out_granule, unsigned long long tag) {
  hipLaunchKernelGGL(rtt_probe_kernel, dim3(1), dim3(1), 0, st, (double2*)out_granule, tag);
}

__global__ __launch_bounds__(256) void transform_kernel(const float4* __restrict__ in, int n, PoseMats P,
                                                        float4* __restrict__ out) {
  const int k = blockIdx.x * blockDim.x + threadIdx.x;
  if (k >= n) return;
  const float4 p = in[k];
  const float* M = P.RT;
  const float x = M[0] * p.x + (M[1] * p.y + (M[2] * p.z + M[3]));
  const float y = M[4] * p.x + (M[5] * p.y + (M[6] * p.z + M[7]));
  const float z = M[8] * p.x + (M[9] * p.y + (M[10] * p.z + M[11]));
  out[k] = make_float4(x, y, z, p.w);
}

constexpr int DEBUG_STAGE_WORDS = 2048;
__global__ __launch_bounds__(256) void deskew_debug_kernel(const DeskewArgs dk, int n, PoseMats P, float4* __restrict__ out_world,
                                                           float4* __restrict__ out_final) {
  __shared__ double s_frames[DEBUG_STAGE_WORDS / 2];
  const DevFrame* frames = static_cast<const DevFrame*>(dk.frames);
  const float* mats = dk.mats;
  if (dk.stage_words > 0) {
    unsigned int* dst = reinterpret_cast<unsigned int*>(s_frames);
    const unsigned int* src = reinterpret_cast<const unsigned int*>(dk.frames);
    for (int i = (int)threadIdx.x; i < dk.stage_words; i += 256)
      dst[i] = __hip_atomic_load(src + i, __ATOMIC_RELAXED, __HIP_MEMORY_SCOPE_SYSTEM);
    __syncthreads();
    frames = reinterpret_cast<const DevFrame*>(dst);
    mats = reinterpret_cast<const float*>(dst) + (dk.mats - static_cast<const float*>(dk.frames));
  }
  const int k = blockIdx.x * blockDim.x + threadIdx.x;
  if (k >= n) return;
  const float4 p = dk.raw[k];
  const unsigned int o = __float_as_uint(p.w);
  if (o >= (unsigned int)n) return;
  const float4 wp = deskew_world(p, dk.t[k] + dk.t_offset, frames, dk.nf, mats);
  const float4 b = deskew_body(wp, mats, 1.0f);
  const float* M = P.RT;
  const float x = M[0] * b.x + (M[1] * b.y + (M[2] * b.z + M[3]));
  const float y = M[4] * b.x + (M[5] * b.y + (M[6] * b.z + M[7]));
  const float z = M[8] * b.x + (M[9] * b.y + (M[10] * b.z + M[11]));
  const float w = M[12] * b.x + (M[13] * b.y + (M[14] * b.z + M[15]));
  out_world[o] = wp;
  out_final[o] = make_float4(x, y, z, w);
}

static inline int round_up8(int x) { return (x + 7) & ~7; }

template <int L>
static void launch_knn5_L(hipStream_t st, const GridView& G, const float4* scan_sorted, int n, const PoseMats& P,
                          int max_ring, void* nbr, int* wl, int* wl_count, unsigned long long* cand, const PrevPass& prev,
                          int tail, hipEvent_t e0, hipEvent_t e1, const FuseArgs* fuse, const TieList* tlp, int after_fine = 0,
                          unsigned long long seq = 0ull, const DeskewArgs* dk = nullptr, const ChainHead* chain = nullptr,
                          unsigned int wait_epoch = 0u, unsigned int end_code = 0u, const PipeHead* pipe = nullptr) {
  const int qpb = 256 / L;
  PrevRT prt;
  for (int i = 0; i < 16; i++) prt.v[i] = prev.RT[i];
  const int blocks = round_up8((n + qpb - 1) / qpb);
  constexpr int slots = 8;
  if constexpr (L == 2) {
    if (fuse) {
      const int grid = fused_blocks(n) + (fuse->ch.S ? 1 : 0);
      if (chain || pipe)
        hipExtLaunchKernelGGL((knn5_chain_kernel<2, 8, true>), dim3(grid), dim3(256), 0, st, e0, e1, 0, G, scan_sorted, n, chain, max_ring, (NbrRec*)nbr, wl, wl_count, cand, prev.valid, prev.probe_min, 1, *fuse, wait_epoch, pipe, prt);
      else
      hipExtLaunchKernelGGL((knn5_kernel<2, 8, true>), dim3(grid), dim3(256), 0, st, e0, e1, 0, G, scan_sorted, n, P, max_ring, (NbrRec*)nbr, wl, wl_count, cand, prev, 1, *fuse);
      return;
    }
  }
  FuseArgs nofuse{};
  if (tlp) nofuse.tl = *tlp;
  nofuse.fine_mode = after_fine ? 1 : 0;
  nofuse.seq = seq;
  if (dk) nofuse.dk = *dk;
  nofuse.ch.end_code = end_code;
  if constexpr (L == 2) {
    if (chain || pipe) {
      hipExtLaunchKernelGGL((knn5_chain_kernel<2, 8, false>), dim3(blocks), dim3(256), 0, st, e0, e1, 0, G, scan_sorted, n, chain, max_ring, (NbrRec*)nbr, wl, wl_count, cand, prev.valid, prev.probe_min, tail, nofuse, wait_epoch, pipe, prt);
      return;
    }
  }
  hipExtLaunchKernelGGL((knn5_kernel<L, slots, false>), dim3(blocks), dim3(256), 0, st, e0, e1, 0, G, scan_sorted, n, P, max_ring, (NbrRec*)nbr, wl, wl_count, cand, prev, tail, nofuse);
}

void launch_knn5(hipStream_t st, int lanes_per_query, const GridView& G, const float4* scan_sorted, int n,
                 const PoseMats& P, int max_ring, void* nbr, int* wl, int* wl_count, unsigned long long* cand,
                 const PrevPass& prev, int tail, hipEvent_t e0, hipEvent_t e1, const FuseArgs* fuse, const TieList* tlp, int after_fine,
                 unsigned long long seq, const DeskewArgs* dk, const ChainHead* chain) {
  if (n <= 0) return;
  if (max_ring < 2 || max_ring > TAIL_MAX_RING) tail = 0;
  if (chain) { launch_knn5_L<2>(st, G, scan_sorted, n, P, max_ring, nbr, wl, wl_count, cand, prev, tail, e0, e1, fuse, tlp, after_fine, seq, dk, chain); return; }
  (void)lanes_per_query;
  launch_knn5_L<2>(st, G, scan_sorted, n, P, max_ring, nbr, wl, wl_count, cand, prev, tail, e0, e1, fuse, tlp, after_fine, seq, dk);
}

void launch_widen(hipStream_t st, const GridView& G, const float4* scan_sorted, const PoseMats& P, int max_ring, void* nbr,
                  int* wl, int* wl_count, unsigned long long* cand, hipEvent_t e0, hipEvent_t e1, const TieList* tlp, const ChainHead* chain) {
  TieList tl{};
  if (tlp) tl = *tlp;
  if (max_ring <= 1) return;
  if (max_ring <= 3)
    hipExtLaunchKernelGGL(widen_kernel, dim3(2048), dim3(256), 0, st, e0, e1, 0, G, scan_sorted, P, max_ring, (NbrRec*)nbr, wl, wl_count, cand, max_ring, tl, chain);
  else
    hipLaunchKernelGGL(widen_general_kernel, dim3(256), dim3(256), 0, st, G, scan_sorted, P, max_ring, (NbrRec*)nbr, wl, wl_count, tl);
}

int fit_blocks(int n) { const int b = (n + 255) / 256; return (b + FIT_GROUPS - 1) / FIT_GROUPS * FIT_GROUPS; }

void launch_fit(hipStream_t st, const GridView& G, const float4* scan_sorted, int n, const void* nbr, const PoseMats& P,
                const MatchParams& mp, double* partials, Rec16* recs, RecDbg* dbg, double* out256, unsigned int* ticket,
                int* wl_count, unsigned long long seq) {
  if (n <= 0) return;
  const int blocks = fit_blocks(n);
  if (recs && dbg)
    hipLaunchKernelGGL((fit_kernel<true, true, 256>), dim3(blocks), dim3(256), 0, st, G, scan_sorted, n, (const NbrRec*)nbr, P, mp, partials, recs, dbg, out256, ticket, wl_count, seq);
  else if (recs)
    hipLaunchKernelGGL((fit_kernel<true, false, 256>), dim3(blocks), dim3(256), 0, st, G, scan_sorted, n, (const NbrRec*)nbr, P, mp, partials, recs, dbg, out256, ticket, wl_count, seq);
}

int fit2_blocks(int n) { const int b = (n + 255) / 256; return (b + FIT_GROUPS - 1) / FIT_GROUPS * FIT_GROUPS; }

void launch_fit2(hipStream_t st, const GridView& G, const float4* scan_sorted, int n, const void* nbr, const PoseMats& P,
                 const MatchParams& mp, const unsigned char* live_idx, double* partials, void* out_granules, unsigned int* ticket,
                 int* wl_count, unsigned long long seq, hipEvent_t e0, hipEvent_t e1, const TieList* tlp, const ChainHead* chain,
                 const ChainCtl* ctl, const BookView* bookp) {
  if (n <= 0) return;
  BookView book{};
  if (bookp) book = *bookp;
  TieList tl{};
  if (tlp) tl = *tlp;
  FitIdx idx;
  for (int i = 0; i < FIT_LIVE_PAD; i++) idx.raw[i] = i < FIT_LIVE ? live_idx[i] : 0;
  ChainCtl ch{};
  if (ctl) ch = *ctl;
  const int grid = fit2_blocks(n) + (ch.S ? 1 : 0);
  if (chain) {
    hipExtLaunchKernelGGL((fit2_chain_kernel<64>), dim3(grid), dim3(256), 0, st, e0, e1, 0, G, scan_sorted, n, (const NbrRec*)nbr, chain, mp, idx, partials, (double2*)out_granules, ticket, wl_count, seq, tl, ch, book);
    return;
  }
  hipExtLaunchKernelGGL((fit2_kernel<64>), dim3(grid), dim3(256), 0, st, e0, e1, 0, G, scan_sorted, n, (const NbrRec*)nbr, P, mp, idx, partials, (double2*)out_granules, ticket, wl_count, seq, tl, ch, book);
}

int fused_spread(int n) { int sh = 0; while (sh < 3 && ((long long)n << (sh + 1)) <= FUSED_SPREAD_SLOTS) sh++; return sh; }
int fused_blocks(int n) { return round_up8((int)((((long long)n << fused_spread(n)) + 127) / 128)); }
void launch_knn5_fine(hipStream_t st, const GridView& Gf, const float4* scan_sorted, int n, const PoseMats& P, void* nbr,
                      const PrevPass& prev, const int qlo[3], const int qhi[3], const TieList* tlp, unsigned long long seq, const ChainHead* chain) {
  if (n <= 0) return;
  FuseArgs fa{};
  fa.fine_mode = 2;
  fa.seq = seq;
  for (int a = 0; a < 3; a++) { fa.qlo[a] = qlo[a]; fa.qhi[a] = qhi[a]; }
  if (tlp) fa.tl = *tlp;
  PrevPass pv = prev;
  if (chain) {
    hipLaunchKernelGGL((knn5_chain_kernel<2, 8, false, true>), dim3(round_up8((n + 127) / 128)), dim3(256), 0, st, Gf, scan_sorted, n, chain, 1,
                       (NbrRec*)nbr, (int*)nullptr, (int*)nullptr, (unsigned long long*)nullptr, pv.valid, pv.probe_min, 0, fa, 0u, (const PipeHead*)nullptr, PrevRT{});
    return;
  }
  hipLaunchKernelGGL((knn5_kernel<2, 8, false, true>), dim3(round_up8((n + 127) / 128)), dim3(256), 0, st, Gf, scan_sorted, n, P, 1,
                     (NbrRec*)nbr, (int*)nullptr, (int*)nullptr, (unsigned long long*)nullptr, pv, 0, fa);
}
void launch_match_fused(hipStream_t st, const GridView& G, const float4* scan_sorted, int n, const PoseMats& P, const MatchParams& mp,
                        void* nbr, int* wl, int* wl_count, unsigned long long* cand, const PrevPass& prev,
                        const unsigned char* live_idx, double* partials, void* out_granules, unsigned int* ticket,
                        unsigned long long seq, hipEvent_t e0, hipEvent_t e1, const TieList* tlp, int after_fine, const DeskewArgs* dk,
                        const ChainHead* chain, const ChainCtl* ctl, const BookView* bookp, unsigned int wait_epoch, const PipeHead* pipe) {
  if (n <= 0) return;
  if ((pipe != nullptr) != (wait_epoch != 0u)) return;
  FuseArgs fa{};
  if (ctl) fa.ch = *ctl;
  if (bookp) fa.book = *bookp;
  if (dk) fa.dk = *dk;
  fa.fine_mode = after_fine ? 1 : 0;
  fa.tl = TieList{};
  if (tlp) fa.tl = *tlp;
  fa.mp = mp;
  for (int i = 0; i < FIT_LIVE_PAD; i++) fa.idx.raw[i] = i < FIT_LIVE ? live_idx[i] : 0;
  fa.partials = partials; fa.granules = (double2*)out_granules; fa.ticket = ticket; fa.seq = seq;
  fa.spread = fused_spread(n);
  launch_knn5_L<2>(st, G, scan_sorted, n, P, mp.max_ring, nbr, wl, wl_count, cand, prev, 1, e0, e1, &fa, nullptr, 0, 0ull, nullptr, chain, wait_epoch, fa.ch.end_code, pipe);
}

size_t nbr_rec_size() { return sizeof(NbrRec); }
size_t wl_entry_size() { return 2 * sizeof(int4); }

void launch_knn(hipStream_t st, const GridView& G, const float* qxyz, int nq, int k, int max_ring, int32_t* idx,
                float* sqd, int32_t* cnt) {
  const int L = 4;
  const long long threads = (long long)nq * L;
  const int blocks = (int)((threads + 255) / 256);
  if (blocks == 0) return;
  const bool anywhere = max_ring > KNN_FAR_RING * 1024;
  hipLaunchKernelGGL((knn_kernel<4>), dim3(blocks), dim3(256), 0, st, G, qxyz, nq, k, anywhere ? KNN_FAR_RING : max_ring, idx, sqd, cnt);
  if (anywhere) hipLaunchKernelGGL(knn_far_kernel, dim3(std::min(4096, (nq + 3) / 4)), dim3(256), 0, st, G, qxyz, nq, k, idx, sqd, cnt);
}

void launch_cap(hipStream_t st, Rec16* recs, int n, int cap) {
  hipLaunchKernelGGL(cap_kernel, dim3(1), dim3(1024), 0, st, recs, n, cap);
}

void launch_capreduce(hipStream_t st, const Rec16* recs, int n, int cap, double* out256, int* wl_count, unsigned long long seq) {
  hipLaunchKernelGGL(capreduce_kernel, dim3(1), dim3(1024), 0, st, recs, n, cap, out256, wl_count, seq);
}

void launch_reduce(hipStream_t st, const Rec16* recs, int n, int nwaves, double* partials, double* out256) {
  hipLaunchKernelGGL(reduce_kernel, dim3(nwaves), dim3(64), 0, st, recs, n, partials);
  hipLaunchKernelGGL(reduce_final_kernel, dim3(1), dim3(1024), 0, st, partials, nwaves, out256);
}

void launch_word_probe(hipStream_t st, const unsigned int* src, void* out_granule, unsigned long long tag) {
  hipLaunchKernelGGL(word_probe_kernel, dim3(1), dim3(1), 0, st, src, (double2*)out_granule, tag);
}
void launch_mfma_layout(hipStream_t st, double* raw256) {
  hipLaunchKernelGGL(mfma_layout_kernel, dim3(1), dim3(64), 0, st, raw256);
}

void launch_deskew(hipStream_t st, const float4* in, const double* t, int n, const void* frames, int nf,
                   const float* mats32, float4* out_sorted, float4* out_orig, double t_offset) {
  const int blocks = (n + 255) / 256;
  if (blocks == 0) return;
  hipLaunchKernelGGL(deskew_kernel, dim3(blocks), dim3(256), 0, st, in, t, n, (const DevFrame*)frames, nf, mats32,
                     out_sorted, out_orig, t_offset);
}
// ... 19 lines not shown
```

include/flimo_dev.h:

```cpp
#ifndef FLIMO_DEV_H
#define FLIMO_DEV_H
#include "flimo_c.h"
#ifdef __cplusplus
extern "C" {
#endif

int flimo_set_timing(flimo_ctx* ctx, int level);
int flimo_set_timing_stride(flimo_ctx* ctx, int every);
int flimo_set_timing_deferred(flimo_ctx* ctx, int on);
unsigned long long flimo_pass_count(const flimo_ctx* ctx);
unsigned long long flimo_fused_pass_count(const flimo_ctx* ctx);
int flimo_tie_stats(flimo_ctx* ctx, unsigned long long out[2]);
int flimo_fine_stats(const flimo_ctx* ctx, unsigned long long out[4]);
int flimo_last_kernel_ms(const flimo_ctx* ctx, float* knn_ms, float* widen_ms, float* fit_ms);
int flimo_timing_totals(flimo_ctx* ctx, double* knn_ms, double* widen_ms, double* fit_ms, long long* passes,
                        long long* queries, int reset);
int flimo_timing_split(flimo_ctx* ctx, double out[6], int reset);
int flimo_set_path_switches(flimo_ctx* ctx, int tail, int fuse);
int flimo_last_widen_count(const flimo_ctx* ctx);
int flimo_last_stragglers(const flimo_ctx* ctx);
int flimo_stragglers_by_pass(const flimo_ctx* ctx, int out[4]);
double flimo_last_candidates_per_query(const flimo_ctx* ctx);

int flimo_map_grid_selfcheck(flimo_ctx* ctx, uint64_t* mismatches, uint64_t stats[2]);
int flimo_map_crop_stats(const flimo_ctx* ctx, uint64_t out[2]);
int flimo_map_carve_stats(const flimo_ctx* ctx, uint64_t out[2]);
int flimo_radius_candidates(flimo_ctx* ctx, const float* q_xyz, size_t nq, float radius, uint64_t* cand);
int flimo_knn_k_candidates(flimo_ctx* ctx, const float* q_xyz, size_t nq, int k, float max_dist, uint64_t* cand);
int flimo_set_normals_chunk(flimo_ctx* ctx, size_t n);
int flimo_set_outlier_chunk(flimo_ctx* ctx, size_t n);
int flimo_set_fpfh_chunk(flimo_ctx* ctx, size_t n);
int flimo_set_keypoints_chunk(flimo_ctx* ctx, size_t n);
int flimo_set_cluster_chunk(flimo_ctx* ctx, size_t n);
int flimo_set_plane_chunk(flimo_ctx* ctx, size_t n);
int flimo_set_voxel_plan(flimo_ctx* ctx, int plan);
int flimo_set_region_chunk(flimo_ctx* ctx, size_t n);
int flimo_set_corr_chunk(flimo_ctx* ctx, size_t n);
int flimo_set_desc_chunk(flimo_ctx* ctx, size_t queries_per_chunk, size_t refs_per_split);
float flimo_desc_last_ms(const flimo_ctx* ctx);
int flimo_set_fitness_chunk(flimo_ctx* ctx, size_t pairs);
int flimo_set_linearize_chunk(flimo_ctx* ctx, size_t pairs);

int flimo_chain_stats(flimo_ctx* ctx, double out[5], int reset);
int flimo_map_index_bytes(const flimo_ctx* ctx, uint64_t out[6]);
int flimo_map_index_layout(flimo_ctx* ctx, int level, double out[28]);
int flimo_pass_pipeline_stats(const flimo_ctx* ctx, unsigned long long out[4]);
int flimo_device_large_bar(int device, int* large_bar);

enum {
  FLIMO_IK_SO3_LOG = 0, FLIMO_IK_A_T = 1, FLIMO_IK_EXP_QUAT = 2, FLIMO_IK_COS_SINC_SQRT = 3, FLIMO_IK_S2_BX = 4,
  FLIMO_IK_S2_BOXMINUS = 5, FLIMO_IK_S2_J = 6, FLIMO_IK_GJ12_INVERSE = 7, FLIMO_IK_GJ12_SOLVE = 8, FLIMO_IK_PRE = 9
};
int flimo_ieskf_op_shape(int op, int* n_in, int* n_out);
int flimo_ieskf_eval(flimo_ctx* ctx, int op, const double* in, size_t n, double* out);
int flimo_ieskf_eval_host(int op, const double* in, size_t n, double* out, int* branch);
#define FLIMO_IK_ITER_N 591
#define FLIMO_IK_FINAL_N 158
int flimo_ieskf_run_fixed(flimo_ctx* ctx, const double x26[26], const double P[529], const double limits[23], double R, double D,
                          int max_iter, int n_sets, const double* partials, const double* extras, const int* tag_ok,
                          double* iter_out, double* final_out, int* n_iter);

void flimo_plane_fit5_host(const float xyz[15], float n_out[4]);
int  flimo_plane_eval5_host(const float n[4], const float xyz[15], float threshold);

int flimo_calculate_H_host(const double x26[26], const float* p_global, const float* n, const float* dist, size_t M,
                           int estimate_extrinsics, double* H, double* h);

int flimo_insert_rule_replay(float min_extent, int downsample, const float* xyz, const size_t* batch_sizes,
                             size_t n_batches, unsigned char* keep, size_t* stored);

#ifdef __cplusplus
}
#endif
#endif
```

Baseline: 7699 scans/s.

## Merge widen and fit2 into one kernel with per-block pending counters

```diff
diff --git a/fast_limo_amd/_abi.py b/fast_limo_amd/_abi.py
--- a/fast_limo_amd/_abi.py
+++ b/fast_limo_amd/_abi.py
@@ -254,7 +254,9 @@
     (i, "flimo_set_timing_deferred", [vp, i]),
     (i, "flimo_set_wait_timeout_ms", [vp, i]),
     (i, "flimo_set_debug_records", [vp, i]),
-    (i, "flimo_set_path_switches", [vp, i, i]),
+    (i, "flimo_set_path_switches", [vp, i, i, i]),
+    (i, "flimo_widen_fit_counts", [vp, P(ull), P(ull)]),
+    (i, "flimo_test_widen_fit_expire", [vp]),
     (ull, "flimo_pass_count", [vp]),
     (ull, "flimo_fused_pass_count", [vp]),
     (i, "flimo_tie_stats", [vp, P(ull)]),
diff --git a/fast_limo_amd/_lib.py b/fast_limo_amd/_lib.py
--- a/fast_limo_amd/_lib.py
+++ b/fast_limo_amd/_lib.py
@@ -769,8 +769,16 @@
         self._chk(self._L.flimo_timing_totals(self._h, C.byref(a), C.byref(b), C.byref(d), C.byref(n), C.byref(q), int(reset)))
         return dict(knn_ms=a.value, widen_ms=b.value, fit_ms=d.value, passes=n.value, queries=q.value)
 
-    def set_path_switches(self, tail=-1, fuse=-1):
-        self._chk(self._L.flimo_set_path_switches(self._h, int(tail), int(fuse)))
+    def set_path_switches(self, tail=-1, fuse=-1, widen_fit=-1):
+        self._chk(self._L.flimo_set_path_switches(self._h, int(tail), int(fuse), int(widen_fit)))
+
+    def widen_fit_counts(self):
+        a = C.c_ulonglong(0); b = C.c_ulonglong(0)
+        self._chk(self._L.flimo_widen_fit_counts(self._h, C.byref(a), C.byref(b)))
+        return int(a.value), int(b.value)
+
+    def test_widen_fit_expire(self):
+        self._chk(self._L.flimo_test_widen_fit_expire(self._h))
 
     def timing_split(self, reset=False):
         o = np.zeros(6)
diff --git a/fast_limo_amd/csrc/hip/flimo_capi.hip b/fast_limo_amd/csrc/hip/flimo_capi.hip
--- a/fast_limo_amd/csrc/hip/flimo_capi.hip
+++ b/fast_limo_amd/csrc/hip/flimo_capi.hip
@@ -252,6 +252,14 @@
   long long chain_alg_n = 0, chains_run = 0, chains_back = 0, chains_declined = 0;
   int fov_check = 0, fov_check_bad = 0;
   bool tail = true;
+  bool widen_fit = true;
+  int wf_blocks = 2048;
+  int* d_blk_pending = nullptr;
+  size_t blk_pending_cap = 0;
+  unsigned long long* h_wf_mail = nullptr;
+  unsigned long long* d_wf_mail = nullptr;
+  bool wf_test_expire = false;
+  unsigned long long wf_passes = 0, wf_fallbacks = 0;
 };
 
 constexpr size_t FRAMES_FG_SLOT = 8192;
@@ -328,6 +336,8 @@
   int v = 0;
   if (env_int("FLIMO_FUSE", v)) c->fuse = v != 0;
   if (env_int("FLIMO_TAIL", v)) c->tail = v != 0;
+  if (env_int("FLIMO_WIDEN_FIT", v)) c->widen_fit = v != 0;
+  if (env_int("FLIMO_WF_BLOCKS", v) && v >= 8 && v <= 2048) c->wf_blocks = v;
   if (env_int("FLIMO_PRUNE", v)) c->prune = v != 0;
   if (env_int("FLIMO_PROBE", v) && v >= 0) c->probe_min = (unsigned)v;
   if (env_int("FLIMO_TIES", v)) c->ties = v != 0;
@@ -408,8 +418,11 @@
             hipMalloc(&c->d_wl_count, sizeof(int)) == hipSuccess &&
             hipMemset(c->d_wl_count, 0, sizeof(int)) == hipSuccess &&
             hipHostMalloc((void**)&c->h_wl_count, sizeof(int), hipHostMallocDefault) == hipSuccess &&
+            hipHostMalloc((void**)&c->h_wf_mail, sizeof(unsigned long long), hipHostMallocMapped) == hipSuccess &&
+            hipHostGetDevicePointer((void**)&c->d_wf_mail, c->h_wf_mail, 0) == hipSuccess &&
             hipHostMalloc((void**)&c->h_cand, sizeof(unsigned long long), hipHostMallocDefault) == hipSuccess;
   if (!ok) { flimo_ctx_destroy(c); return FLIMO_ERR_HIP; }
+  *c->h_wf_mail = 0ull;
   memset(c->h_chain_res, 0, (size_t)CH_RES * 2 * sizeof(double));
   memset(c->h_chain_log, 0, (size_t)CH_MAX_PASSES * CH_LOGN * 2 * sizeof(double));
   memset(c->h_out256, 0, FIT_GROUPS * FIT_SLOT * sizeof(double));
@@ -508,6 +521,8 @@
   if (c->timeout_ev) (void)hipEventDestroy(c->timeout_ev);
   if (c->adopt_ev) (void)hipEventDestroy(c->adopt_ev);
   if (c->h_wl_count) (void)hipHostFree(c->h_wl_count);
+  if (c->h_wf_mail) (void)hipHostFree(c->h_wf_mail);
+  (void)hipFree(c->d_blk_pending);
   if (c->d_pipe_head) (void)hipFree(c->d_pipe_head);
   if (c->d_frames_fg) (void)hipFree(c->d_frames_fg);
   if (c->stream) (void)hipStreamDestroy(c->stream);
@@ -2216,6 +2231,14 @@
     (void)hipFree(c->d_fit2_partials);
     c->d_fit2_partials = f2; c->fit2_partials_cap = f2n;
   }
+  {
+    const size_t bpn = (size_t)fit2_blocks((int)cap) * WF_STRIDE;
+    int* bp = nullptr;
+    HIPCHK(c, hipMalloc(&bp, bpn * sizeof(int)));
+    HIPCHK(c, hipMemsetAsync(bp, 0, bpn * sizeof(int), c->stream));
+    (void)hipFree(c->d_blk_pending);
+    c->d_blk_pending = bp; c->blk_pending_cap = bpn;
+  }
   HIPCHK(c, hipMalloc(&so, cap * sizeof(float4)));
   HIPCHK(c, hipMalloc(&nb, cap * nbr_rec_size()));
   HIPCHK(c, hipMemsetAsync(nb, 0, cap * nbr_rec_size(), c->stream));
@@ -2722,10 +2745,22 @@
   if (reset) { c->tot_knn_ms = c->tot_widen_ms = c->tot_fit_ms = 0.0; c->tot_passes = 0; c->tot_queries = 0; }
   return FLIMO_OK;
 }
-extern "C" int flimo_set_path_switches(flimo_ctx* c, int tail, int fuse) {
+extern "C" int flimo_set_path_switches(flimo_ctx* c, int tail, int fuse, int widen_fit) {
   if (!c) return FLIMO_ERR_INVALID;
   if (tail >= 0) c->tail = tail != 0;
   if (fuse >= 0) c->fuse = fuse != 0;
+  if (widen_fit >= 0) c->widen_fit = widen_fit != 0;
+  return FLIMO_OK;
+}
+extern "C" int flimo_test_widen_fit_expire(flimo_ctx* c) {
+  if (!c) return FLIMO_ERR_INVALID;
+  c->wf_test_expire = true;
+  return FLIMO_OK;
+}
+extern "C" int flimo_widen_fit_counts(const flimo_ctx* c, unsigned long long* passes, unsigned long long* fallbacks) {
+  if (!c) return FLIMO_ERR_INVALID;
+  if (passes) *passes = c->wf_passes;
+  if (fallbacks) *fallbacks = c->wf_fallbacks;
   return FLIMO_OK;
 }
 extern "C" int flimo_timing_split(flimo_ctx* c, double out[6], int reset) {
@@ -2808,7 +2843,8 @@
   return true;
 }
 constexpr int FLIMO_PASS_LEFT = 1000;
-static int wait_tags(flimo_ctx* c, unsigned long long want, int left_ms = -1) {
+constexpr int FLIMO_WF_EXPIRED = 1001;
+static int wait_tags(flimo_ctx* c, unsigned long long want, int left_ms = -1, bool watch_mail = false) {
   const volatile unsigned long long* t0 = reinterpret_cast<const volatile unsigned long long*>(c->h_granules);
   unsigned long long spins = 0;
   double deadline = 0.0;
@@ -2819,6 +2855,7 @@
     if (t0[2 * (FIT_LIVE + 1) + 1] == want && tags_complete(c, want)) return FLIMO_OK;
     _mm_pause();
     if ((++spins & 0x3fffull) != 0) continue;
+    if (watch_mail && __atomic_load_n(c->h_wf_mail, __ATOMIC_ACQUIRE) == want) return FLIMO_WF_EXPIRED;
     if (left_ms >= 0 && c->d_pipe_head &&
         __atomic_load_n(&c->d_pipe_head->decision, __ATOMIC_ACQUIRE) == ((ch_epoch_of(want) & 0x3fffffffu) | 0x80000000u)) return FLIMO_PASS_LEFT;
     const double t = now_s();
@@ -2879,6 +2916,7 @@
   hipEvent_t* ev = nullptr;
   int tail_max = 0;
   bool tail = false, fused = false, after_fine = false, widen_timed = false;
+  bool widen_fit = false;
   unsigned long long seq = 0;
   bool ties_on = false, inline_ties = false;
   TieList tl{};
@@ -2979,6 +3017,8 @@
   pl.widen_timed = !pl.tail && pl.tlev == 1 && mp.max_ring >= 2;
   pl.fused_cap = pl.cap_binds && !c->debug_recs;
   pl.use_fit2 = !pl.want_recs;
+  pl.widen_fit = c->widen_fit && !pl.tail && !pl.fused && pl.use_fit2 && !pl.want_count && mp.max_ring >= 2 && mp.max_ring <= 3 &&
+                 c->d_blk_pending && (size_t)fit2_blocks(pl.n_all) * WF_STRIDE <= c->blk_pending_cap;
   return FLIMO_OK;
 }
 
@@ -3042,16 +3082,23 @@
   } else
   launch_knn5(c->stream, 2, c->grid, c->d_scan_sorted, n_all, P, mp.max_ring, c->d_nbr, c->d_wl,
               c->d_wl_count, c->debug_recs ? c->d_cand : nullptr, c->prev, pl.tail ? 1 : 0, tlev == 1 ? pl.ev[0] : nullptr,
-              tlev == 1 ? pl.ev[1] : nullptr, nullptr, &pl.tl, pl.after_fine ? 1 : 0, seq, pl.dkp);
+              tlev == 1 ? pl.ev[1] : nullptr, nullptr, &pl.tl, pl.after_fine ? 1 : 0, seq, pl.dkp, nullptr,
+              pl.widen_fit ? c->d_blk_pending : nullptr);
   c->prev_before = c->prev;
   if (c->prune) { memcpy(c->prev.RT, P.RT, sizeof(c->prev.RT)); c->prev.valid = 1; }
   pl.tpb = g_prof_pass ? now_us() : 0.0;
-  if (!pl.tail)
+  if (pl.widen_fit) {
+    launch_widen_fit(c->stream, c->grid, c->d_scan_sorted, n_all, c->d_nbr, P, mp, c->live_idx, c->d_fit2_partials, c->d_granules_host,
+                     c->d_ticket, c->d_wl, c->d_wl_count, seq, &pl.tl, pl.bookp, c->d_blk_pending, c->d_wf_mail, c->wf_blocks,
+                     c->wf_test_expire ? 1 : 0, pl.widen_timed ? pl.ev[4] : nullptr, pl.widen_timed ? pl.ev[5] : nullptr);
+    c->wf_test_expire = false;
+    c->wf_passes++;
+  } else if (!pl.tail)
     launch_widen(c->stream, c->grid, c->d_scan_sorted, P, mp.max_ring, c->d_nbr, c->d_wl, c->d_wl_count,
                  c->debug_recs ? c->d_cand : nullptr, pl.widen_timed ? pl.ev[4] : nullptr, pl.widen_timed ? pl.ev[5] : nullptr, &pl.tl);
   pl.tpc = g_prof_pass ? now_us() : 0.0;
   if (pl.want_count) HIPCHK(c, hipMemcpyAsync(c->h_wl_count, c->d_wl_count, sizeof(int), hipMemcpyDeviceToHost, c->stream));
-  if (pl.fused) {
+  if (pl.fused || pl.widen_fit) {
   } else if (pl.use_fit2)
     launch_fit2(c->stream, c->grid, c->d_scan_sorted, n_all, c->d_nbr, P, mp, c->live_idx, c->d_fit2_partials, c->d_granules_host,
                 c->d_ticket, c->d_wl_count, seq, tlev == 1 ? pl.ev[2] : nullptr, tlev == 1 ? pl.ev[3] : nullptr, &pl.tl, nullptr, nullptr, pl.bookp);
@@ -3098,7 +3145,7 @@
 }
 
 static int timing_read(flimo_ctx* c, hipEvent_t* ev, int kind) {
-  const bool fused = kind & 1, use_fit2 = kind & 2, widen_timed = kind & 4;
+  const bool fused = kind & 1, use_fit2 = kind & 2, widen_timed = kind & 4, widen_fit = kind & 8;
   if (hipEventElapsedTime(&c->last_knn_ms, ev[0], ev[1]) != hipSuccess) {
     HIPCHK(c, hipEventSynchronize(ev[1]));
     (void)hipEventElapsedTime(&c->last_knn_ms, ev[0], ev[1]);
@@ -3113,6 +3160,14 @@
       if (hipEventElapsedTime(&c->last_widen_ms, ev[4], ev[5]) != hipSuccess) c->last_widen_ms = 0.f;
       c->tot_widen_ms += c->last_widen_ms;
     }
+    if (widen_fit) {
+      c->last_fit_ms = 0.f;
+      if (widen_timed && c->last_widen_ms == 0.f) {
+        HIPCHK(c, hipEventSynchronize(ev[5]));
+        (void)hipEventElapsedTime(&c->last_widen_ms, ev[4], ev[5]);
+        c->tot_widen_ms += c->last_widen_ms;
+      }
+    } else
     if (hipEventElapsedTime(&c->last_fit_ms, ev[2], ev[3]) != hipSuccess) {
       HIPCHK(c, hipEventSynchronize(ev[3]));
       (void)hipEventElapsedTime(&c->last_fit_ms, ev[2], ev[3]);
@@ -3138,15 +3193,25 @@
   const int tlev = pl.tlev;
   double acc[256];
   if (pl.use_fit2) {
-    auto wait_granules = [&](unsigned long long want, int left_ms = -1) -> int {
-      const int rcw = wait_tags(c, want, left_ms);
+    auto wait_granules = [&](unsigned long long want, int left_ms = -1, bool watch_mail = false) -> int {
+      const int rcw = wait_tags(c, want, left_ms, watch_mail);
       if (rcw) return rcw;
       __atomic_thread_fence(__ATOMIC_ACQUIRE);
       return FLIMO_OK;
     };
     run_overlap(c);
     {
-      int rcw = wait_granules(seq, pl.was_pre ? CH_POLL_MS + 25 : -1);
+      int rcw = wait_granules(seq, pl.was_pre ? CH_POLL_MS + 25 : -1, pl.widen_fit);
+      if (rcw == FLIMO_WF_EXPIRED) {
+        cancel_prelaunch(c);
+        c->wf_fallbacks++;
+        HIPCHK(c, hipMemsetAsync(c->d_ticket, 0, (FIT_GROUPS + 2) * sizeof(unsigned int), c->stream));
+        HIPCHK(c, hipMemsetAsync(c->d_blk_pending, 0, c->blk_pending_cap * sizeof(int), c->stream));
+        launch_fit2(c->stream, c->grid, c->d_scan_sorted, n_all, c->d_nbr, P, mp, c->live_idx, c->d_fit2_partials, c->d_granules_host,
+                    c->d_ticket, c->d_wl_count, seq, nullptr, nullptr, &pl.tl, nullptr, nullptr, pl.bookp);
+        HIPCHK(c, hipGetLastError());
+        rcw = wait_granules(seq);
+      }
       if (rcw == FLIMO_PASS_LEFT) {
         cancel_prelaunch(c);
         c->pipe_left++;
@@ -3204,7 +3269,7 @@
     HIPCHK(c, hipStreamSynchronize(c->stream));
   }
   if (tlev) {
-    const int kind = (pl.fused ? 1 : 0) | (pl.use_fit2 ? 2 : 0) | (pl.widen_timed ? 4 : 0);
+    const int kind = (pl.fused ? 1 : 0) | (pl.use_fit2 ? 2 : 0) | (pl.widen_timed ? 4 : 0) | (pl.widen_fit ? 8 : 0);
     if (pl.ev != c->ev) {
       c->ev_kind[c->ev_pending++] = (unsigned char)kind;
       if (c->ev_pending == flimo_ctx::EV_RING) { const int rc = timing_drain(c); if (rc) return rc; }
diff --git a/fast_limo_amd/csrc/hip/flimo_kernels.h b/fast_limo_amd/csrc/hip/flimo_kernels.h
--- a/fast_limo_amd/csrc/hip/flimo_kernels.h
+++ b/fast_limo_amd/csrc/hip/flimo_kernels.h
@@ -19,7 +19,7 @@
                  const PoseMats& P, int max_ring, void* nbr, int* wl, int* wl_count, unsigned long long* cand,
                  const PrevPass& prev, int tail, hipEvent_t e0 = nullptr, hipEvent_t e1 = nullptr, const struct FuseArgs* fuse = nullptr,
                  const TieList* ties = nullptr, int after_fine = 0, unsigned long long seq = 0ull, const DeskewArgs* deskew = nullptr,
-                 const ChainHead* chain = nullptr);
+                 const ChainHead* chain = nullptr, int* blk_pending = nullptr);
 void launch_knn5_fine(hipStream_t st, const GridView& Gf, const float4* scan_sorted, int n, const PoseMats& P, void* nbr,
                       const PrevPass& prev, const int qlo[3], const int qhi[3], const TieList* ties, unsigned long long seq,
                       const ChainHead* chain = nullptr);
@@ -40,6 +40,11 @@
                  const MatchParams& mp, const unsigned char* live_idx, double* partials, void* out_granules, unsigned int* ticket,
                  int* wl_count, unsigned long long seq, hipEvent_t e0 = nullptr, hipEvent_t e1 = nullptr, const TieList* ties = nullptr,
                  const ChainHead* chain = nullptr, const ChainCtl* ctl = nullptr, const BookView* book = nullptr);
+constexpr int WF_STRIDE = 64;
+void launch_widen_fit(hipStream_t st, const GridView& G, const float4* scan_sorted, int n, void* nbr, const PoseMats& P,
+                      const MatchParams& mp, const unsigned char* live_idx, double* partials, void* out_granules, unsigned int* ticket,
+                      const int* wl, int* wl_count, unsigned long long seq, const TieList* ties, const BookView* book, int* blk_pending,
+                      unsigned long long* mail, int wblocks, int expire_now = 0, hipEvent_t e0 = nullptr, hipEvent_t e1 = nullptr);
 constexpr int FUSED_SPREAD_SLOTS = 32768;
 int fused_spread(int n);
 int fused_blocks(int n);
diff --git a/fast_limo_amd/csrc/hip/flimo_kernels.hip b/fast_limo_amd/csrc/hip/flimo_kernels.hip
--- a/fast_limo_amd/csrc/hip/flimo_kernels.hip
+++ b/fast_limo_amd/csrc/hip/flimo_kernels.hip
@@ -731,6 +731,7 @@
   BookView book;
   ChainCtl ch;
   int spread;
+  int* blk_pending;
 };
 template <int ROWS>
 __device__ __forceinline__ void fit_reduce_publish(const float (&v)[16], bool owns_row, int row, float* sr, double* sa0, double* sa1,
@@ -1186,6 +1187,12 @@
       e[1] = make_int4((int)(uint32_t)(best[4] >> 32), 2, __float_as_int(b2), 0);
     }
   }
+  if constexpr (!FUSE && !FINE) {
+    if (fa.blk_pending) {
+      const unsigned long long m = __ballot(in_range && sub == 0 && !pend_tail && flag >= 2);
+      if (m != 0ull && (threadIdx.x & 63) == 0) atomicAdd(&fa.blk_pending[(p >> 8) * WF_STRIDE], (int)__popcll(m));
+    }
+  }
   WaveLds& W = s_w[threadIdx.x >> 6];
   if (tail) knn5_tail(G, dir, max_ring, nbr, pend_tail && sub == 0, p, gx, gy, gz, (uint32_t)(best[4] >> 32), b2, W, wl_count, cand_total, FUSE, tl);
   TRACE(0, 5);
@@ -1307,14 +1314,17 @@
   knn5_pass<L, SLOTS, FUSE, FINE>(G, s_dir, nullptr, scan_sorted, n, Lh->pose, max_ring, nbr, wl, wl_count, cand_total, Lh->prev_RT, prev_valid, probe_min, tail, fa);
 }
 
+template <bool MERGED = false>
 __device__ __forceinline__ void widen_body(const GridView& G, int max_ring, NbrRec* __restrict__ nbr,
                                            const int* __restrict__ wl, const int* __restrict__ wl_count,
                                            unsigned long long* __restrict__ cand_total, int first_ring, const TieList& tl,
-                                           int blk, int nblk, uint32_t (*s_off)[65], uint32_t (*s_lo)[64]) {
+                                           int blk, int nblk, uint32_t (*s_off)[65], uint32_t (*s_lo)[64],
+                                           int* __restrict__ blk_pending = nullptr) {
   const int lane = threadIdx.x & 63, wave = threadIdx.x >> 6;
   const int maxdim = grid_maxdim(G);
   const float margin = 1.0e-3f + 4.0e-7f * (float)maxdim;
   int w = blk * 4 + wave;
+  int prev_blk = -1;
   const int4* entries = reinterpret_cast<const int4*>(wl);
   int4 e0 = entries[2 * (size_t)w], e1 = entries[2 * (size_t)w + 1];
   const int count = *wl_count;
@@ -1443,9 +1453,25 @@
       const bool tie = flag == 1 && key_has_tie(best, sixth);
       b.x = (int)(uint32_t)best[4]; b.y = flag; b.z = (int)(uint32_t)(best[4] >> 32); b.w = ((flag == 1) ? 1 : 0) | (tie ? 2 : 0);
       int4* o = reinterpret_cast<int4*>(&nbr[p]);
-      o[0] = a;
-      o[1] = b;
+      if constexpr (MERGED) {
+        typedef int v4i_t __attribute__((ext_vector_type(4)));
+        const v4i_t va = {a.x, a.y, a.z, a.w}, vb = {b.x, b.y, b.z, b.w};
+        asm volatile("s_waitcnt vmcnt(0)" ::: "memory");
+        if (prev_blk >= 0) __hip_atomic_fetch_add(&blk_pending[prev_blk], -1, __ATOMIC_RELAXED, __HIP_MEMORY_SCOPE_AGENT);
+        asm volatile("global_store_dwordx4 %0, %1, off sc1\n\tglobal_store_dwordx4 %0, %2, off offset:16 sc1\n\ts_nop 1"
+                     :: "v"(o), "v"(va), "v"(vb) : "memory");
+        prev_blk = (p >> 8) * WF_STRIDE;
+      } else {
+        o[0] = a;
+        o[1] = b;
+      }
       if (tie && tl.list) { const unsigned slot = atomicAdd(tl.count, 1u); if (slot < tl.cap) tl.list[slot] = p; }
+    }
+  }
+  if constexpr (MERGED) {
+    if (lane == 0 && prev_blk >= 0) {
+      asm volatile("s_waitcnt vmcnt(0)" ::: "memory");
+      __hip_atomic_fetch_add(&blk_pending[prev_blk], -1, __ATOMIC_RELAXED, __HIP_MEMORY_SCOPE_AGENT);
     }
   }
 }
@@ -1804,37 +1830,72 @@
   }
 }
 
-template <int PPW>
+struct WfCtl {
+  int* blk_pending;
+  unsigned long long* mail;
+  int wblocks;
+  int expire_now;
+};
+template <int PPW, bool MERGED = false>
 __device__ __forceinline__ void fit2_pass(const GridView& G, const float4* __restrict__ scan_sorted, int n,
                                           const NbrRec* __restrict__ nbr, const PoseMats& P, const MatchParams& mp, const FitIdx& idx,
                                           double* __restrict__ partials, double2* __restrict__ out_granules,
                                           unsigned int* __restrict__ ticket, int* __restrict__ wl_count,
-                                          unsigned long long seq, const TieList& tl, const ChainCtl& ch, const BookView& book) {
+                                          unsigned long long seq, const TieList& tl, const ChainCtl& ch, const BookView& book,
+                                          int blk, int nblk, const WfCtl& wf) {
   __shared__ __align__(16) float s_rec[4][16 * 65];
   __shared__ double s_acc[4][256];
   __shared__ unsigned int s_last;
   static_assert(sizeof(float) * 4 * 16 * 65 >= (size_t)IESKF_LDS_BYTES, "the filter's algebra runs in this workgroup's shared memory");
-  int nb = (int)gridDim.x;
+  int nb = nblk;
   if (ch.S) {
     nb -= 1;
-    if ((int)blockIdx.x == nb) {
+    if (blk == nb) {
       double* big = reinterpret_cast<double*>(&s_rec[0][0]);
       ik_extra_block(ch, big, (int)threadIdx.x);
       return;
     }
   }
   const int lane = threadIdx.x & 63, wave = threadIdx.x >> 6;
-  const int chunk = xcd_chunk(blockIdx.x, nb);
+  const int chunk = xcd_chunk(blk, nb);
   const int p = (chunk * 4 + wave) * PPW + lane;
   float v[16];
 #pragma unroll
   for (int i = 0; i < 16; i++) v[i] = 0.f;
   TRACE(1, 0);
+  if constexpr (MERGED) {
+    if (threadIdx.x == 0) {
+      unsigned int ok = wf.expire_now ? 0u : 1u;
+      if (ok && __hip_atomic_load(&wf.blk_pending[chunk * WF_STRIDE], __ATOMIC_RELAXED, __HIP_MEMORY_SCOPE_AGENT) != 0) {
+        const unsigned long long t0 = wall_clock64();
+        for (;;) {
+          __builtin_amdgcn_s_sleep(32);
+          if (__hip_atomic_load(&wf.blk_pending[chunk * WF_STRIDE], __ATOMIC_RELAXED, __HIP_MEMORY_SCOPE_AGENT) == 0) break;
+          if (wall_clock64() - t0 > (unsigned long long)CH_POLL_MS * 100000ull) { ok = 0u; break; }
+        }
+      }
+      if (!ok) __hip_atomic_store(wf.mail, seq, __ATOMIC_RELAXED, __HIP_MEMORY_SCOPE_SYSTEM);
+      s_last = ok;
+    }
+    __syncthreads();
+    const unsigned int go = s_last;
+    __syncthreads();
+    if (!go) return;
+  }
   {
     const bool mine = lane < PPW && p < n;
     const float4 sp = scan_sorted[mine ? p : 0];
     const int4* nb = reinterpret_cast<const int4*>(&nbr[mine ? p : 0]);
-    const int4 a = nb[0], b = nb[1];
+    int4 a, b;
+    if constexpr (MERGED) {
+      typedef int v4i_t __attribute__((ext_vector_type(4)));
+      v4i_t va, vb;
+      asm volatile("global_load_dwordx4 %0, %2, off sc1\n\tglobal_load_dwordx4 %1, %2, off offset:16 sc1\n\ts_waitcnt vmcnt(0)"
+                   : "=&v"(va), "=&v"(vb) : "v"(nb) : "memory");
+      a = make_int4(va.x, va.y, va.z, va.w); b = make_int4(vb.x, vb.y, vb.z, vb.w);
+    } else {
+      a = nb[0]; b = nb[1];
+    }
     float gx, gy, gz;
     xform4(P.RT, sp.x, sp.y, sp.z, gx, gy, gz);
     int ids[5] = {a.x, a.y, a.z, a.w, b.x};
@@ -1846,7 +1907,7 @@
   }
   TRACE(1, 3);
   fit_reduce_publish<PPW>(v, lane < PPW, lane, s_rec[wave], s_acc[0], s_acc[1], s_acc[2], s_acc[3], &s_last, idx, partials,
-                          out_granules, ticket, wl_count, seq, tl, (int)blockIdx.x, nb);
+                          out_granules, ticket, wl_count, seq, tl, blk, nb);
 }
 
 template <int PPW>
@@ -1855,7 +1916,8 @@
                                                    double* __restrict__ partials, double2* __restrict__ out_granules,
                                                    unsigned int* __restrict__ ticket, int* __restrict__ wl_count,
                                                    unsigned long long seq, TieList tl, ChainCtl ch, BookView book) {
-  fit2_pass<PPW>(G, scan_sorted, n, nbr, P, mp, idx, partials, out_granules, ticket, wl_count, seq, tl, ch, book);
+  fit2_pass<PPW>(G, scan_sorted, n, nbr, P, mp, idx, partials, out_granules, ticket, wl_count, seq, tl, ch, book, (int)blockIdx.x,
+                 (int)gridDim.x, WfCtl{});
 }
 template <int PPW>
 __global__ __launch_bounds__(256) void fit2_chain_kernel(GridView G, const float4* __restrict__ scan_sorted, int n,
@@ -1864,7 +1926,24 @@
                                                    unsigned int* __restrict__ ticket, int* __restrict__ wl_count,
                                                    unsigned long long seq, TieList tl, ChainCtl ch, BookView book) {
   if (H->status != 0) return;
-  fit2_pass<PPW>(G, scan_sorted, n, nbr, H->pose, mp, idx, partials, out_granules, ticket, wl_count, seq, tl, ch, book);
+  fit2_pass<PPW>(G, scan_sorted, n, nbr, H->pose, mp, idx, partials, out_granules, ticket, wl_count, seq, tl, ch, book, (int)blockIdx.x,
+                 (int)gridDim.x, WfCtl{});
+}
+
+template <int PPW>
+__global__ __attribute__((amdgpu_waves_per_eu(4,4))) __launch_bounds__(256) void widen_fit_kernel(GridView G, const float4* __restrict__ scan_sorted, int n, NbrRec* nbr,
+                                                        PoseMats P, MatchParams mp, FitIdx idx, double* __restrict__ partials,
+                                                        double2* __restrict__ out_granules, unsigned int* __restrict__ ticket,
+                                                        const int* __restrict__ wl, int* wl_count, unsigned long long seq, TieList tl,
+                                                        BookView book, WfCtl wf) {
+  if ((int)blockIdx.x < wf.wblocks) {
+    __shared__ uint32_t s_off[4][65];
+    __shared__ uint32_t s_lo[4][64];
+    widen_body<true>(G, mp.max_ring, nbr, wl, wl_count, nullptr, mp.max_ring, tl, (int)blockIdx.x, wf.wblocks, s_off, s_lo, wf.blk_pending);
+    return;
+  }
+  fit2_pass<PPW, true>(G, scan_sorted, n, nbr, P, mp, idx, partials, out_granules, ticket, wl_count, seq, tl, ChainCtl{}, book,
+                       (int)blockIdx.x - wf.wblocks, (int)gridDim.x - wf.wblocks, wf);
 }
 
 __constant__ unsigned char c_ordered_indices[8][7] = {
@@ -2523,7 +2602,8 @@
                           int max_ring, void* nbr, int* wl, int* wl_count, unsigned long long* cand, const PrevPass& prev,
                           int tail, hipEvent_t e0, hipEvent_t e1, const FuseArgs* fuse, const TieList* tlp, int after_fine = 0,
                           unsigned long long seq = 0ull, const DeskewArgs* dk = nullptr, const ChainHead* chain = nullptr,
-                          unsigned int wait_epoch = 0u, unsigned int end_code = 0u, const PipeHead* pipe = nullptr) {
+                          unsigned int wait_epoch = 0u, unsigned int end_code = 0u, const PipeHead* pipe = nullptr,
+                          int* blk_pending = nullptr) {
   const int qpb = 256 / L;
   PrevRT prt;
   for (int i = 0; i < 16; i++) prt.v[i] = prev.RT[i];
@@ -2545,6 +2625,7 @@
   nofuse.seq = seq;
   if (dk) nofuse.dk = *dk;
   nofuse.ch.end_code = end_code;
+  nofuse.blk_pending = blk_pending;
   if constexpr (L == 2) {
     if (chain || pipe) {
       hipExtLaunchKernelGGL((knn5_chain_kernel<2, 8, false>), dim3(blocks), dim3(256), 0, st, e0, e1, 0, G, scan_sorted, n, chain, max_ring, (NbrRec*)nbr, wl, wl_count, cand, prev.valid, prev.probe_min, tail, nofuse, wait_epoch, pipe, prt);
@@ -2557,12 +2638,13 @@
 void launch_knn5(hipStream_t st, int lanes_per_query, const GridView& G, const float4* scan_sorted, int n,
                  const PoseMats& P, int max_ring, void* nbr, int* wl, int* wl_count, unsigned long long* cand,
                  const PrevPass& prev, int tail, hipEvent_t e0, hipEvent_t e1, const FuseArgs* fuse, const TieList* tlp, int after_fine,
-                 unsigned long long seq, const DeskewArgs* dk, const ChainHead* chain) {
+                 unsigned long long seq, const DeskewArgs* dk, const ChainHead* chain, int* blk_pending) {
   if (n <= 0) return;
   if (max_ring < 2 || max_ring > TAIL_MAX_RING) tail = 0;
   if (chain) { launch_knn5_L<2>(st, G, scan_sorted, n, P, max_ring, nbr, wl, wl_count, cand, prev, tail, e0, e1, fuse, tlp, after_fine, seq, dk, chain); return; }
   (void)lanes_per_query;
-  launch_knn5_L<2>(st, G, scan_sorted, n, P, max_ring, nbr, wl, wl_count, cand, prev, tail, e0, e1, fuse, tlp, after_fine, seq, dk);
+  launch_knn5_L<2>(st, G, scan_sorted, n, P, max_ring, nbr, wl, wl_count, cand, prev, tail, e0, e1, fuse, tlp, after_fine, seq, dk, nullptr,
+                   0u, 0u, nullptr, blk_pending);
 }
 
 void launch_widen(hipStream_t st, const GridView& G, const float4* scan_sorted, const PoseMats& P, int max_ring, void* nbr,
@@ -2610,6 +2692,23 @@
     return;
   }
   hipExtLaunchKernelGGL((fit2_kernel<64>), dim3(grid), dim3(256), 0, st, e0, e1, 0, G, scan_sorted, n, (const NbrRec*)nbr, P, mp, idx, partials, (double2*)out_granules, ticket, wl_count, seq, tl, ch, book);
+}
+
+void launch_widen_fit(hipStream_t st, const GridView& G, const float4* scan_sorted, int n, void* nbr, const PoseMats& P,
+                      const MatchParams& mp, const unsigned char* live_idx, double* partials, void* out_granules, unsigned int* ticket,
+                      const int* wl, int* wl_count, unsigned long long seq, const TieList* tlp, const BookView* bookp, int* blk_pending,
+                      unsigned long long* mail, int wblocks, int expire_now, hipEvent_t e0, hipEvent_t e1) {
+  if (n <= 0) return;
+  BookView book{};
+  if (bookp) book = *bookp;
+  TieList tl{};
+  if (tlp) tl = *tlp;
+  FitIdx idx;
+  for (int i = 0; i < FIT_LIVE_PAD; i++) idx.raw[i] = i < FIT_LIVE ? live_idx[i] : 0;
+  WfCtl wf{blk_pending, mail, round_up8(std::max(wblocks, 8)), expire_now};
+  const int grid = wf.wblocks + fit2_blocks(n);
+  hipExtLaunchKernelGGL((widen_fit_kernel<64>), dim3(grid), dim3(256), 0, st, e0, e1, 0, G, scan_sorted, n, (NbrRec*)nbr, P, mp, idx, partials,
+                        (double2*)out_granules, ticket, wl, wl_count, seq, tl, book, wf);
 }
 
 int fused_spread(int n) { int sh = 0; while (sh < 3 && ((long long)n << (sh + 1)) <= FUSED_SPREAD_SLOTS) sh++; return sh; }
diff --git a/include/flimo_dev.h b/include/flimo_dev.h
--- a/include/flimo_dev.h
+++ b/include/flimo_dev.h
@@ -16,7 +16,9 @@
 int flimo_timing_totals(flimo_ctx* ctx, double* knn_ms, double* widen_ms, double* fit_ms, long long* passes,
                         long long* queries, int reset);
 int flimo_timing_split(flimo_ctx* ctx, double out[6], int reset);
-int flimo_set_path_switches(flimo_ctx* ctx, int tail, int fuse);
+int flimo_set_path_switches(flimo_ctx* ctx, int tail, int fuse, int widen_fit);
+int flimo_widen_fit_counts(const flimo_ctx* ctx, unsigned long long* passes, unsigned long long* fallbacks);
+int flimo_test_widen_fit_expire(flimo_ctx* ctx);
 int flimo_last_widen_count(const flimo_ctx* ctx);
 int flimo_last_stragglers(const flimo_ctx* ctx);
 int flimo_stragglers_by_pass(const flimo_ctx* ctx, int out[4]);
```

Result: slower. 7616 scans/s (-1.1%).
